# StefanHeng/Symbolic-Music-Generation

Hardware: AMD Instinct MI355X
Metric: train tokens/sec (TransfoXL seq2048 bf16), whole job (higher is better)
Workload: dtype bf16; 1 GPU; TransfoXL 12L/768d H12 dh64 F3072 T=2048 M=2048 V=1190 cutoffs=[] (SURVEY C3, mode R: fresh zero mems); per_gpu_batch=64, global_batch=64, seq_len=2048, mem_len=2048, parallelism=dp1

## Files before the change

include/musicxl.h:

```cpp
#ifndef MUSICXL_H
#define MUSICXL_H

#ifdef __cplusplus
extern "C" {
#endif

#define MXL_ABI_VERSION 2

int mxl_abi_version(void);
const char* mxl_error_string(int code);

#define MXL_GEMM_OUT_F32        0x01
#define MXL_GEMM_OUT_F32_ATOMIC 0x02
#define MXL_GEMM_BIAS           0x04
#define MXL_GEMM_RELU           0x08
#define MXL_GEMM_DROPOUT        0x10
#define MXL_GEMM_RELU_BWD       0x20
#define MXL_GEMM_ADD_AUX        0x40
int mxl_set_reserved_cus(int k);
int mxl_gemm_last_nt_kernel(void);

#define MXL_GEMM_SAVE_RELU_MASK 0x100
#define MXL_GEMM_RELU_BWD_BITS  0x200
size_t mxl_gemm_relu_mask_bytes(int M, int N);
int mxl_gemm_bf16(const void* A, const void* B, void* C, int M, int N, int K, int lda, int ldb, int ldc,
                  int transA, int transB, int flags, float alpha, const float* bias,
                  const void* aux, int ldaux, int ksplits,
                  float drop_p, unsigned long long seed, unsigned site, void* stream);

int mxl_gemm_bf16_colsum(const void* A, const void* B, void* C, int M, int N, int K, int lda, int ldb, int ldc,
                         int transA, int transB, int flags, float alpha, const float* bias, const void* aux, int ldaux,
                         float drop_p, unsigned long long seed, unsigned site, float* colsum, void* stream);

int mxl_gemm_bf16_headdot(const void* A, const void* B, void* C, int M, int N, int K, int lda, int ldb, int ldc, const void* O, int ldo,
                          int T, float* delta, void* stream);

int mxl_gemm_bf16_batched(const void* A, const void* B, void* C, int M, int N, int K, int lda, int ldb, int ldc,
                          int transA, int transB, int flags, float alpha, int ksplits, int batch, int bdiv,
                          long long sA1, long long sA2, long long sB1, long long sB2, long long sC1, long long sC2,
                          void* stream);

int mxl_gemm_skinny_bf16(const void* A, const void* W, void* C, int M, int N, int K, int lda, int ldw, int ldc, int flags,
                         const float* bias, void* stream);
int mxl_gemm_skinny_partial(const void* A, const void* W, float* slabs, int M, int N, int K, int lda, int ldw, int KS,
                            void* stream);
int mxl_ln_residual_fwd_partial(const float* slabs, int KS, long long slab_stride, const float* bias, const void* res,
                                const float* gamma, const float* beta, void* y, int N, int d, float eps, void* stream);
int mxl_decode_qkv(const void* x, const void* Wqkv, void* qkv, void* kcache, void* vcache, const int* t_dev,
                   const float* r_r_bias, void* qr_out, int B, int d, int dh, int Mring, void* stream);

int mxl_relattn_fwd(const void* q, const void* k, const void* v, const void* rd, const float* r_w_bias,
                    const float* r_r_bias, void* out, float* lse, int B, int T, int H, int dh, int M, int Kc,
                    long long q_bs, int q_rs, long long kv_bs, int kv_rs, int rd_rs, long long o_bs, int o_rs,
                    float scale, void* stream);

int mxl_relattn_bwd(const void* q, const void* k, const void* v, const void* rd, const float* r_w_bias,
                    const float* r_r_bias, const void* out, const void* dout, const float* lse, float* delta,
                    void* dq, void* dk, void* dv, void* dg, float* d_r_w_bias, float* d_r_r_bias , int B, int T,
                    int H, int dh, int M, int Kc, long long q_bs, int q_rs, long long kv_bs, int kv_rs, int rd_rs,
                    long long o_bs, int o_rs, long long dq_bs, int dq_rs, long long dkv_bs, int dkv_rs,
                    float scale, void* stream);

int mxl_relattn_drd(const void* dg, const void* qr, float* d_rd, int B, int T, int H, int dh, int M, long long qr_bs,
                    int qr_rs, int drd_ld, const void* rd, int rd_rs, float* d_r_r_bias, float* d_r_w_bias_fix, void* stream);

int mxl_relattn_bwd_sparse_dg(const void* q, const void* k, const void* v, const void* rd, const float* r_w_bias,
                              const float* r_r_bias, const void* out, const void* dout, const float* lse, float* delta, void* dq,
                              void* dk, void* dv, void* dg, float* d_r_w_bias, int B, int T, int H, int dh, int M, int Kc,
                              long long q_bs, int q_rs, long long kv_bs, int kv_rs, int rd_rs, long long o_bs, int o_rs,
                              long long dq_bs, int dq_rs, long long dkv_bs, int dkv_rs, float scale, void* stream);
int mxl_relattn_fwd_phantom(const void* q, const void* k, const void* v, const void* rd, const float* r_w_bias,
                            const float* r_r_bias, void* out, float* lse, void* oph, float* mph, int B, int T, int H,
                            int dh, int M, int Kc, long long q_bs, int q_rs, long long kv_bs, int kv_rs, int rd_rs,
                            long long o_bs, int o_rs, float scale, void* stream);
int mxl_relattn_bwd_sparse_dg_oph(const void* q, const void* k, const void* v, const void* rd, const float* r_w_bias,
                                  const float* r_r_bias, const void* out, const void* dout, const float* lse,
                                  float* delta, void* dq, void* dk, void* dv, void* dg, float* d_r_w_bias,
                                  const void* oph, const float* mph, int B, int T, int H, int dh, int M, int Kc,
                                  long long q_bs, int q_rs, long long kv_bs, int kv_rs, int rd_rs, long long o_bs, int o_rs,
                                  long long dq_bs, int dq_rs, long long dkv_bs, int dkv_rs, float scale, void* stream);
int mxl_relattn_drd_recompute(const void* dg, const void* qr, float* d_rd, int B, int T, int H, int dh, int M, long long qr_bs,
                              int qr_rs, int drd_ld, const void* rd, int rd_rs, float* d_r_r_bias, float* d_r_w_bias_fix,
                              const float* lse, const float* delta, float scale, int Kc, void* stream);

size_t mxl_relattn_bwd_fused_ws_bytes(int B, int T, int H, int dh, int M);
int mxl_relattn_bwd_fused(const void* q, const void* k, const void* v, const void* rd, const float* r_w_bias,
                          const float* r_r_bias, const void* out, const void* dout, const float* lse, float* delta,
                          void* dq, void* dk, void* dv, float* d_rd, int drd_ld, float* d_r_w_bias, float* d_r_r_bias,
                          const void* oph, const float* mph, void* ws, int B, int T, int H, int dh, int M, int Kc,
                          long long q_bs, int q_rs, long long kv_bs, int kv_rs, int rd_rs, long long o_bs, int o_rs,
                          long long dq_bs, int dq_rs, long long dkv_bs, int dkv_rs, float scale, int defer_finish, void* stream);
int mxl_relattn_dq_finish(const void* ws, const void* oph, const float* mph, const float* lse, const float* delta, void* dq,
                          float* d_r_r_bias, int B, int T, int H, int dh, int M, int Kc, long long o_bs, int o_rs, long long dq_bs,
                          int dq_rs, float scale, void* stream);
int mxl_relattn_fwd_phantom2(const void* q, const void* k, const void* v, const void* rd, const float* r_w_bias,
                             const float* r_r_bias, void* out, float* lse, void* oph, float* mph, int oph_all, void* ph_ws, int B,
                             int T, int H, int dh, int M, int Kc, long long q_bs, int q_rs, long long kv_bs, int kv_rs, int rd_rs,
                             long long o_bs, int o_rs, float scale, void* stream);
size_t mxl_relattn_drd_phantom_ws_bytes(int B, int T, int H);
int mxl_relattn_drd_phantom_prep(const void* q, long long q_bs, int q_rs, const float* r_r_bias, const float* lse, void* ws, int B, int T,
                                 int H, int dh, float scale, void* stream);
int mxl_relattn_drd_phantom(const void* ws, const float* delta, float* d_rd, int B, int T, int H, int dh, int M, int drd_ld,
                            const void* rd, int rd_rs, int Kc, void* stream);

int mxl_sinusoid_table(void* out, int M, int d, int clamp_len, float drop_p, unsigned long long seed, unsigned site,
                       void* stream);
int mxl_embed_fwd(const void* ids, const void* E, void* out, int N, int d, int V, float scale, float drop_p,
                  unsigned long long seed, unsigned site, void* stream);
int mxl_embed_bwd(const void* ids, const void* dout, const void* dout2, float* dE, int N, int d, int V, float scale,
                  float drop_p, unsigned long long seed, unsigned site, void* stream);
int mxl_dropout_bf16(const void* x, void* y, long long n, float drop_p, unsigned long long seed, unsigned site,
                     void* stream);
int mxl_ln_residual_fwd(const void* x, const void* res, const float* gamma, const float* beta, void* y, void* z,
                        float* mean, float* rstd, int N, int d, float eps, float drop_p, unsigned long long seed,
                        unsigned site, void* stream);
int mxl_ln_residual_bwd(const void* dy, const void* dy2, const void* z, const float* mean, const float* rstd,
                        const float* gamma, void* dres, void* dx, float* dgamma, float* dbeta, int N, int d,
                        float drop_p, unsigned long long seed, unsigned site, void* stream);
int mxl_ln_residual_bwd_colsum(const void* dy, const void* dy2, const void* z, const float* mean, const float* rstd,
                               const float* gamma, void* dres, void* dx, float* dgamma, float* dbeta, float* dxsum, int N,
                               int d, float drop_p, unsigned long long seed, unsigned site, void* stream);
int mxl_ln_residual_bwd_add(const void* dy, const void* dy2, const void* z, const float* mean, const float* rstd,
                            const float* gamma, const void* dadd, void* dres, float* dgamma, float* dbeta, int N, int d,
                            void* stream);
int mxl_ln_residual_bwd_add_drop(const void* dy, const void* dy2, const void* z, const float* mean, const float* rstd,
                                 const float* gamma, const void* dadd, void* dres, void* dx, float* dxsum, float* dgamma,
                                 float* dbeta, int N, int d, float drop_p, unsigned long long seed, unsigned site, void* stream);
int mxl_add_rowbias_bf16(const void* x, long long x_bs, int x_rs, const float* bias, void* out, int B, int T, int n,
                         void* stream);
int mxl_colsum_bf16(const void* X, float* out, int M, int N, int ld, void* stream);
int mxl_dropout_colsum_bf16(const void* X, void* Y, float* out, int M, int N, float drop_p, unsigned long long seed,
                            unsigned site, void* stream);
int mxl_center_columns_bf16(const void* X, void* Y, int M, int N, void* stream);
int mxl_mem_update(const void* mem, const void* hid, void* out, int B, int M, int T, int d, void* stream);

int mxl_label_guard(void* labels_row0, int T, long long eos, void* stream);
int mxl_adaptive_nll_fwd(const float* logits, int ldl, const void* labels, float* nll, float* lse, float* acc2, int B,
                         int T, int V, int ncl, const int* cutoffs_host, void* stream);
int mxl_adaptive_nll_bwd(const float* logits, int ldl, const void* labels, const float* nll, const float* lse,
                         const float* acc2, void* dlogits, int ldd, int B, int T, int V, int ncl,
                         const int* cutoffs_host, float grad_scale, void* stream);
int mxl_adaptive_nll_bwd_split(const float* logits, int ldl, const void* labels, const float* nll, const float* lse,
                               const float* acc2, void* dlogits_hi, void* dlogits_lo, int ldd, int B, int T, int V, int ncl,
                               const int* cutoffs_host, float grad_scale, void* stream);
int mxl_adaptive_logprob(const float* logits, int ldl, float* out, int ldo, int N, int V, int ncl,
                         const int* cutoffs_host, void* stream);

int mxl_cluster_bucket(const void* labels, int B, int T, int V, int ncl, const int* cutoffs_host, int* perm, int* counts,
                       int* tgt_head, int* tgt_tail, void* stream);
int mxl_gather_rows_bf16(const void* src, int ld_src, const int* idx, void* dst, int n, int d, void* stream);
int mxl_scatter_add_rows_bf16(const void* src, const int* idx, void* dst, int ld_dst, int n, int d, void* stream);
int mxl_rows_lse_pick(const float* logits, long long ld, int ncols, int n_rows, const int* rows_idx, int row0, const int* tgt,
                      float* lse_out, float* pick_out, void* stream);
int mxl_bucket_nll_finish(const float* head_lse, const float* head_pick, const float* tail_lse, const float* tail_pick,
                          const int* tgt_head, const int* tgt_tail, float* nll, float* nll_tok, float* acc2, int B, int T,
                          void* stream);
int mxl_rows_softmax_grad(const float* logits, long long ld, int ncols, int n_rows, const int* rows_idx, int row0, const int* tgt,
                          const float* lse, const float* nll_tok, const float* acc2, float grad_scale, void* out_hi, void* out_lo,
                          int ldo, void* stream);

int mxl_sumsq_f32(const float* x, long long n, float* out_accum, void* stream);
int mxl_adamw_step(float* p, const float* g, float* m, float* v, void* w16, long long n, long long n_decay, float lr,
                   float beta1, float beta2, float eps, float weight_decay, int step, const float* sumsq,
                   float max_norm, float grad_scale, void* stream);
int mxl_cast_f32_bf16(const float* x, void* y, long long n, void* stream);
int mxl_cast_bf16_f32(const void* x, float* y, long long n, void* stream);
int mxl_transpose_bf16(const void* src, void* dst, int rows, int cols, int ld_src, int ld_dst, int batch,
                       long long src_bstride, long long dst_bstride, void* stream);

int mxl_decode_embed(const void* ids, int ld_ids, const int* t_dev, const void* E, void* out, int B, int d, int V,
                     float scale, void* stream);
int mxl_kv_append(const void* qkv, void* kcache, void* vcache, const int* t_dev, int B, int M, int d, int dh,
                  const float* r_r_bias, void* qr_out, void* stream);
int mxl_kv_fill(const void* qkv, void* kcache, void* vcache, int B, int T, int M, int d, int dh, void* stream);
int mxl_kv_zero_pad(void* qkv, const int* n_pad, int B, int T, int d, void* stream);
int mxl_decode_bd(const void* qr, const void* rd, float* bd, int B, int H, int dh, int M, int ld_qr, int ld_rd, void* stream);
int mxl_relattn_decode(const void* qkv, const void* kcache, const void* vcache, const float* bd, const float* r_w_bias,
                       void* out, const int* t_dev, int B, int H, int dh, int M, float scale, void* stream);
size_t mxl_relattn_decode_split_ws_bytes(int B, int H, int dh, int pieces);
int mxl_relattn_decode_split(const void* qkv, const void* kcache, const void* vcache, const float* bd, const float* r_w_bias,
                             void* out, const int* t_dev, int B, int H, int dh, int M, float scale, int pieces, float* ws,
// ... 239 lines not shown
```

symbolic_music_generation_amd/csrc/relattn_bwd_fused.hip:

```cpp
#include <cstdlib>
#include <type_traits>
#include "common.h"
#include "musicxl_internal.h"

namespace {

typedef __attribute__((ext_vector_type(8))) __bf16 mfma_bf16x8;
typedef __attribute__((address_space(3))) bf16x4 lds_bf16x4;
typedef _Float16 f16x4 __attribute__((ext_vector_type(4)));
typedef float f32x4v __attribute__((ext_vector_type(4)));

#ifndef FUSED_PF
#define FUSED_PF 3
#endif
#ifndef FUSED_VF_RELOAD
#define FUSED_VF_RELOAD 0
#endif
#ifndef FUSED_PARK
#define FUSED_PARK 0
#endif
#ifndef FUSED_SB
#define FUSED_SB 1
#endif
#define UNIT_FENCE() do { if (FUSED_SB) __builtin_amdgcn_sched_barrier(0); } while (0)
#ifndef FUSED_DVDK_LATE
#define FUSED_DVDK_LATE 1
#endif
#ifndef FUSED_PRIO
#define FUSED_PRIO 3
#endif
#define PRIO_UP() do { if (FUSED_PRIO & 1) __builtin_amdgcn_s_setprio(1); } while (0)
#define PRIO_DOWN() do { if (FUSED_PRIO & 1) __builtin_amdgcn_s_setprio(0); } while (0)
#define PRIO_UP_B(bit_) do { if (FUSED_PRIO & (bit_)) __builtin_amdgcn_s_setprio(1); } while (0)
#define PRIO_DOWN_B(bit_) do { if (FUSED_PRIO & (bit_)) __builtin_amdgcn_s_setprio(0); } while (0)
#ifndef FUSED_OWNER_LD_EARLY
#define FUSED_OWNER_LD_EARLY 1
#endif
#ifndef FUSED_TRF_EARLY
#define FUSED_TRF_EARLY 1
#endif
constexpr float LOG2E = 1.4426950408889634f;
constexpr int KBLK = 256;
constexpr int QT = 32;
constexpr int ROWB = 128;
constexpr int K_BYTES = KBLK * ROWB;
constexpr int RING_BLKS = 10;
constexpr int RBLK_BYTES = 32 * ROWB;
constexpr int RING_BYTES = RING_BLKS * RBLK_BYTES;
constexpr int QIMG = QT * ROWB;
constexpr int QSET = 3 * QIMG + 3 * QT * 4;
constexpr int GP = 584;
constexpr int G_BYTES = QT * GP;
constexpr int X_BYTES = KBLK * 64;
constexpr int YP = 608;
constexpr int Y_BYTES = QT * YP;
constexpr int BIAS_BYTES = 2 * 64 * 4;
constexpr int PARK_BYTES = FUSED_PARK ? 32 * 64 * 4 : 0;
constexpr int SMEM = K_BYTES + RING_BYTES + 2 * QSET + G_BYTES + X_BYTES + Y_BYTES + BIAS_BYTES + PARK_BYTES;
constexpr int RING_OFF = 10240;

#ifdef MXL_STAMP
__device__ unsigned long long g_fused_stamps[16];
#define STAMP_DECL unsigned long long st_last, st_acc[16] = {0ull, 0ull, 0ull, 0ull, 0ull, 0ull, 0ull, 0ull, 0ull, 0ull, 0ull, 0ull, 0ull, 0ull, 0ull, 0ull}; \
    { __builtin_amdgcn_sched_barrier(0); asm volatile("s_memtime %0\n\ts_waitcnt lgkmcnt(0)" : "=s"(st_last) :: "memory"); __builtin_amdgcn_sched_barrier(0); }
#define STAMP(i) { unsigned long long t_; __builtin_amdgcn_sched_barrier(0); asm volatile("s_memtime %0\n\ts_waitcnt lgkmcnt(0)" : "=s"(t_) :: "memory"); \
    __builtin_amdgcn_sched_barrier(0); st_acc[i] += t_ - st_last; st_last = t_; }
#define STAMP_FLUSH if ((threadIdx.x & 63) == 0) { for (int i_ = 0; i_ < 16; i_++) atomicAdd(&g_fused_stamps[i_], st_acc[i_]); }
#else
#define STAMP_DECL
#define STAMP(i)
#define STAMP_FLUSH
#endif

#ifndef MXL_SLAB_BF16
#define MXL_SLAB_BF16 1
#endif
#if MXL_SLAB_BF16
typedef bf16_t slab_t;
#else
typedef float slab_t;
#endif

struct FusedP {
    const bf16_t *q, *k, *v, *rd, *dout;
    const float *rwb, *rrb, *lse, *delta;
    bf16_t *dk, *dv;
    slab_t* slab;
    bf16_t* dq;
    const bf16_t* oph;
    const float* mph;
    long long dq_bs;
    int dq_rs;
    float* drd;
    float *d_rwb, *d_rrb;
    int B, T, H, M, Kc;
    long long q_bs, kv_bs, o_bs, dkv_bs, slab_stride;
    int q_rs, kv_rs, rd_rs, o_rs, dkv_rs, drd_ld;
    float scale, scale_log2e;
};

__device__ __forceinline__ int qswz(int row) { return (((row >> 1) & 1) << 2) | (((row >> 2) & 1) << 1) | ((row >> 3) & 1); }
__device__ __forceinline__ int qoff(int row, int ch) { return row * ROWB + ((ch ^ qswz(row)) << 4); }
__device__ __forceinline__ int qeoff(int row, int e) { return qoff(row, e >> 3) + ((e & 7) << 1); }
__device__ __forceinline__ int sswz(int row) { return (((row >> 3) & 1) << 2) | (((row >> 1) & 1) << 1) | ((row >> 2) & 1); }
__device__ __forceinline__ int soff(int row, int ch) { return row * ROWB + ((ch ^ sswz(row)) << 4); }

__device__ __forceinline__ void lds_barrier() {
    asm volatile("s_waitcnt lgkmcnt(0)" ::: "memory");
    __builtin_amdgcn_s_barrier();
    asm volatile("" ::: "memory");
}

__device__ __forceinline__ uint32_t lds_addr(const void* p) {
    return (uint32_t)(uintptr_t)(__attribute__((address_space(3))) const char*)(const char*)p;
}

__device__ __forceinline__ void gskew_wait() { asm volatile("s_waitcnt lgkmcnt(0)" ::: "memory"); }
__device__ __forceinline__ void gskew_read16(uint32_t base, uint32_t (&u)[16]) {
    static_assert(GP == 584, "offsets below are pat(j) * (GP + 2)");
    asm volatile(
        "ds_read_u16 %0, %16\n\t"               "ds_read_u16 %1, %16 offset:586\n\t"    "ds_read_u16 %2, %16 offset:1172\n\t"
        "ds_read_u16 %3, %16 offset:1758\n\t"   "ds_read_u16 %4, %16 offset:4688\n\t"   "ds_read_u16 %5, %16 offset:5274\n\t"
        "ds_read_u16 %6, %16 offset:5860\n\t"   "ds_read_u16 %7, %16 offset:6446\n\t"   "ds_read_u16 %8, %16 offset:9376\n\t"
        "ds_read_u16 %9, %16 offset:9962\n\t"   "ds_read_u16 %10, %16 offset:10548\n\t" "ds_read_u16 %11, %16 offset:11134\n\t"
        "ds_read_u16 %12, %16 offset:14064\n\t" "ds_read_u16 %13, %16 offset:14650\n\t" "ds_read_u16 %14, %16 offset:15236\n\t"
        "ds_read_u16 %15, %16 offset:15822"
        : "=&v"(u[0]), "=&v"(u[1]), "=&v"(u[2]), "=&v"(u[3]), "=&v"(u[4]), "=&v"(u[5]), "=&v"(u[6]), "=&v"(u[7]),
          "=&v"(u[8]), "=&v"(u[9]), "=&v"(u[10]), "=&v"(u[11]), "=&v"(u[12]), "=&v"(u[13]), "=&v"(u[14]), "=&v"(u[15])
        : "v"(base)
        : "memory");
}
__device__ __forceinline__ void yskew_write16(uint32_t base, const uint32_t (&w)[8]) {
    static_assert(YP == 608, "offsets below are pat(j) * (YP + 2)");
    asm volatile(
        "ds_write_b16 %8, %0\n\t"               "ds_write_b16_d16_hi %8, %0 offset:610\n\t"
        "ds_write_b16 %8, %1 offset:1220\n\t"   "ds_write_b16_d16_hi %8, %1 offset:1830\n\t"
        "ds_write_b16 %8, %2 offset:4880\n\t"   "ds_write_b16_d16_hi %8, %2 offset:5490\n\t"
        "ds_write_b16 %8, %3 offset:6100\n\t"   "ds_write_b16_d16_hi %8, %3 offset:6710\n\t"
        "ds_write_b16 %8, %4 offset:9760\n\t"   "ds_write_b16_d16_hi %8, %4 offset:10370\n\t"
        "ds_write_b16 %8, %5 offset:10980\n\t"   "ds_write_b16_d16_hi %8, %5 offset:11590\n\t"
        "ds_write_b16 %8, %6 offset:14640\n\t"   "ds_write_b16_d16_hi %8, %6 offset:15250\n\t"
        "ds_write_b16 %8, %7 offset:15860\n\t"   "ds_write_b16_d16_hi %8, %7 offset:16470"
        :
        : "v"(w[0]), "v"(w[1]), "v"(w[2]), "v"(w[3]), "v"(w[4]), "v"(w[5]), "v"(w[6]), "v"(w[7]), "v"(base)
        : "memory");
}
__device__ __forceinline__ float add_f16(float s, uint32_t h16) {
    float r;
    asm("v_fma_mix_f32 %0, %1, 1.0, %2 op_sel_hi:[0,0,1]" : "=v"(r) : "v"(s), "v"(h16));
    return r;
}
__device__ __forceinline__ bf16x8 tr_pair(const char* lo_p, const char* hi_p) {
    const bf16x4 lo = __builtin_amdgcn_ds_read_tr16_b64_v4i16((lds_bf16x4*)lo_p);
    const bf16x4 hi = __builtin_amdgcn_ds_read_tr16_b64_v4i16((lds_bf16x4*)hi_p);
    return bf16x8{lo[0], lo[1], lo[2], lo[3], hi[0], hi[1], hi[2], hi[3]};
}
__device__ __forceinline__ f32x16 mfma32(bf16x8 a, bf16x8 b, f32x16 c) {
    return __builtin_amdgcn_mfma_f32_32x32x16_bf16(__builtin_bit_cast(mfma_bf16x8, a), __builtin_bit_cast(mfma_bf16x8, b), c, 0, 0, 0);
}
__device__ __forceinline__ f32x4 mfma16(bf16x8 a, bf16x8 b, f32x4 c) {
    return __builtin_amdgcn_mfma_f32_16x16x32_bf16(__builtin_bit_cast(mfma_bf16x8, a), __builtin_bit_cast(mfma_bf16x8, b), c, 0, 0, 0);
}

constexpr int VM_PER_TILE_BLOCK = 6;
constexpr int VM_PER_TILE_OWNER = 10;

__global__ __launch_bounds__(256) void fused_delta_kernel(const bf16_t* o, const bf16_t* dout, float* delta, int B, int T, int H,
                                                          long long o_bs, int o_rs) {
    const int row = blockIdx.x * 4 + (threadIdx.x >> 6);
    if (row >= B * T) return;
    const int lane = threadIdx.x & 63;
    const int b = row / T, i = row % T;
    const bf16_t* op = o + (size_t)b * o_bs + (size_t)i * o_rs;
    const bf16_t* dp = dout + (size_t)b * o_bs + (size_t)i * o_rs;
    const int chunks = H * 8;
    for (int c0 = 0; c0 < chunks; c0 += 64) {
        const int c = c0 + lane;
        float s = 0.f;
        if (c < chunks) {
            const bf16x8 a = *reinterpret_cast<const bf16x8*>(op + c * 8);
            const bf16x8 d = *reinterpret_cast<const bf16x8*>(dp + c * 8);
#pragma unroll
            for (int j = 0; j < 8; j++) s += bf2f((bf16_t)a[j]) * bf2f((bf16_t)d[j]);
        }
        s += __shfl_xor(s, 1, 64); s += __shfl_xor(s, 2, 64); s += __shfl_xor(s, 4, 64);
        if (c < chunks && (lane & 7) == 0) delta[((size_t)b * H + (c >> 3)) * T + i] = s;
    }
}

template <bool OWNER>
__global__ __launch_bounds__(512, 1) void relattn_bwd_fused_kernel(FusedP p) {
    constexpr int NT = 512;
    constexpr int VM_PER_TILE = OWNER ? VM_PER_TILE_OWNER : VM_PER_TILE_BLOCK;
    extern __shared__ __attribute__((aligned(16))) char smem[];
    char* sK = smem;
    char* sR = sK + K_BYTES;
    char* sQ = sR + RING_BYTES;
    char* sG = sQ + 2 * QSET;
    char* sX = sG + G_BYTES;
    char* sY = sX + X_BYTES;
    float* sBias = reinterpret_cast<float*>(sY + Y_BYTES);
    float* sPark = sBias + BIAS_BYTES / 4;

    STAMP_DECL
    const int tid = threadIdx.x;
    const int w = __builtin_amdgcn_readfirstlane(tid >> 6);
    const int l = tid & 63, r = l & 31, hh = l >> 5;
    int bx_, h, b;
    xcd_block(bx_, h, b);
    const int h64 = __builtin_amdgcn_readfirstlane(h * 64);
    const int T = p.T, M = p.M;
    const int p0 = T - p.Kc;
    const int nkb = (p.Kc + KBLK - 1) / KBLK;
    const int kloc0 = 32 * w + r;
    const int MB = M >> 5;

    const bf16_t* qbase = p.q + (size_t)b * p.q_bs + (size_t)h * 64;
    const bf16_t* dobase = p.dout + (size_t)b * p.o_bs + (size_t)h * 64;
    const bf16_t* rbase = p.rd + (size_t)h * 64;
    const bf16_t* kbase = p.k + (size_t)b * p.kv_bs + (size_t)h * 64;
    const bf16_t* vbase = p.v + (size_t)b * p.kv_bs + (size_t)h * 64;

    const int eq = w >> 1, ih0 = w & 1;
    const int g16 = l >> 4;
    int rowq, rows, tkb, xw, yt0, qb0, xa0, xa1, ka0, ka1, yq0, krow;
    uint32_t gRb, yWb;
    auto lane_consts = [&](const int l) {
    const int r = l & 31, hh = l >> 5, kloc0 = 32 * w + r;
    const int gq = l >> 4, q4 = (l & 15) >> 2, pp = l & 3;
    rowq = qoff(r, hh);
    rows = r * ROWB + ((hh ^ sswz(r)) << 4);
    tkb = qeoff(4 * hh + q4, 16 * (gq & 1) + 4 * pp);
    gRb = lds_addr(sG) + 4 * hh * (GP + 2) + (256 - kloc0) * 2;
    yWb = lds_addr(sY) + 4 * hh * (YP + 2) + (256 - kloc0) * 2;
    const int xf = (kloc0 >> 1) & 7;
    xw = kloc0 * 64 + ((((hh ^ (xf & 1)) | (xf & 6))) << 3);
    yt0 = (4 * (l >> 4) + ((l & 15) >> 2)) * YP + (16 * (w & 1) + 4 * pp) * 2;
    qb0 = qeoff(4 * (l >> 4) + ((l & 15) >> 2), 16 * (w >> 1) + 4 * pp);
    const int g16 = l >> 4, q16 = (l & 15) >> 2;
    xa0 = ((8 * g16 + q16) * 64 + ((pp ^ ((4 * g16 + (q16 >> 1)) & 7)) << 3)) ^ (ih0 << 5);
    xa1 = ((8 * g16 + q16 + 4) * 64 + ((pp ^ ((4 * g16 + 2 + (q16 >> 1)) & 7)) << 3)) ^ (ih0 << 5);
    const int kch = 2 * eq + (pp >> 1);
    const int ksw = ((g16 & 1) << 2) | (((q16 >> 1) & 1) << 1);
    ka0 = (8 * g16 + q16) * ROWB + ((kch ^ ksw) << 4) + ((pp & 1) << 3);
    ka1 = (8 * g16 + q16 + 4) * ROWB + ((kch ^ (ksw | 1)) << 4) + ((pp & 1) << 3);
    yq0 = (16 * ih0 + (l & 15)) * YP + 16 * g16;
    krow = kloc0 * ROWB + ((hh ^ sswz(kloc0)) << 4);
    };
    if (!OWNER) lane_consts(l);

    if (tid < 128) sBias[tid] = (tid < 64) ? p.rwb[h64 + tid] : p.rrb[h64 + tid - 64];

    const bool st_q = w < 4;
    const __amdgpu_buffer_rsrc_t rs_q = __builtin_amdgcn_make_buffer_rsrc((void*)qbase, 0, -1, 0x00020000);
    const __amdgpu_buffer_rsrc_t rs_2 = __builtin_amdgcn_make_buffer_rsrc((void*)(st_q ? rbase : dobase), 0, -1, 0x00020000);
    const __amdgpu_buffer_rsrc_t rs_lse = __builtin_amdgcn_make_buffer_rsrc((void*)(p.lse + ((size_t)b * p.H + h) * T), 0, -1, 0x00020000);
    const __amdgpu_buffer_rsrc_t rs_dl = __builtin_amdgcn_make_buffer_rsrc((void*)(p.delta + ((size_t)b * p.H + h) * T), 0, -1, 0x00020000);
    const bool has_ph = OWNER && p.oph != nullptr;
    const __amdgpu_buffer_rsrc_t rs_mph = __builtin_amdgcn_make_buffer_rsrc(
        (void*)(has_ph ? p.mph + ((size_t)b * p.H + h) * T : p.lse), 0, has_ph ? T * 4 : 0, 0x00020000);
    u32x4 tq = {0u, 0u, 0u, 0u}, t2 = {0u, 0u, 0u, 0u};
    float tl = 0.f, tdl = 0.f, tm = 0.f;
#define STG_IDS int tid_o = tid; asm volatile("" : "+v"(tid_o)); const int srow_ = (tid_o & 255) >> 3, sch_ = tid_o & 7;
    auto load_stage = [&](int it, int nblk) {
        STG_IDS
        const int I = it * QT;
        tq = __builtin_bit_cast(u32x4, __builtin_amdgcn_raw_buffer_load_b128(rs_q, (srow_ * p.q_rs + sch_ * 8) * 2, I * p.q_rs * 2, 0));
        int d = 32 * nblk + srow_;
        d = d < 0 ? 0 : (d > M - 1 ? M - 1 : d);
        const int vo2 = st_q ? (d * p.rd_rs + sch_ * 8) * 2 : (srow_ * p.o_rs + sch_ * 8) * 2;
        const int so2 = st_q ? 0 : I * p.o_rs * 2;
        t2 = __builtin_bit_cast(u32x4, __builtin_amdgcn_raw_buffer_load_b128(rs_2, vo2, so2, 0));
        tl = __builtin_bit_cast(float, __builtin_amdgcn_raw_buffer_load_b32(rs_lse, (tid & 31) * 4, I * 4, 0));
        tdl = __builtin_bit_cast(float, __builtin_amdgcn_raw_buffer_load_b32(rs_dl, (tid & 31) * 4, I * 4, 0));
        if (OWNER) tm = __builtin_bit_cast(float, __builtin_amdgcn_raw_buffer_load_b32(rs_mph, (tid & 31) * 4, I * 4, 0));
    };
    auto store_stage = [&](int buf, int slot) {
        STG_IDS
        char* sQw = sQ + buf * QSET;
        char* sQr = sQw + QIMG;
        char* sDO = sQr + QIMG;
        float* sLse = reinterpret_cast<float*>(sDO + QIMG);
        {
            const bf16_t* src = reinterpret_cast<const bf16_t*>(&tq);
            const float* bb = sBias + (st_q ? 0 : 64) + sch_ * 8;
            const f32x4 b0 = *reinterpret_cast<const f32x4*>(bb), b1 = *reinterpret_cast<const f32x4*>(bb + 4);
            u32x4 wq;
            bf16_t* dq_ = reinterpret_cast<bf16_t*>(&wq);
#pragma unroll
            for (int j = 0; j < 8; j++) dq_[j] = f2bf((bf2f(src[j]) + (j < 4 ? b0[j & 3] : b1[j & 3])) * p.scale_log2e);
            *reinterpret_cast<u32x4*>((st_q ? sQw : sQr) + qoff(srow_, sch_)) = wq;
        }
        if (st_q) {
            *reinterpret_cast<u32x4*>(sR + slot * RBLK_BYTES + soff(srow_, sch_)) = t2;
        } else {
            const bf16_t* src = reinterpret_cast<const bf16_t*>(&t2);
            u32x4 wd;
            bf16_t* dd = reinterpret_cast<bf16_t*>(&wd);
#pragma unroll
            for (int j = 0; j < 8; j++) dd[j] = f2bf(bf2f(src[j]) * p.scale);
            *reinterpret_cast<u32x4*>(sDO + qoff(srow_, sch_)) = wd;
        }
        if (tid < 32) {
            sLse[tid] = -tl * LOG2E; sLse[QT + tid] = -p.scale * tdl;
            if (OWNER) sLse[2 * QT + tid] = tm;
        }
    };
    auto slot_add = [&](int s, int k) { const int x = s + k; return x >= RING_BLKS ? x - RING_BLKS : x; };
    auto gblock = [&](int j, int s0, const bf16x8 (&bq)[4]) {
        f32x16 g;
#pragma unroll
        for (int t = 0; t < 16; t++) g[t] = 0.f;
        const char* rb = sR + slot_add(s0, j) * RBLK_BYTES;
        bf16x8 a[4];
#pragma unroll
        for (int ks = 0; ks < 4; ks++) a[ks] = *reinterpret_cast<const bf16x8*>(rb + (rows ^ (ks << 5)));
#pragma unroll
        for (int ks = 0; ks < 4; ks++) g = mfma32(a[ks], bq[ks], g);
        char* gw = sG + r * GP + (32 * j + 4 * hh) * 2;
#pragma unroll
        for (int grp = 0; grp < 4; grp++) {
            const f32x4v v4 = {g[4 * grp], g[4 * grp + 1], g[4 * grp + 2], g[4 * grp + 3]};
            *reinterpret_cast<f16x4*>(gw + 16 * grp) = __builtin_convertvector(v4, f16x4);
        }
    };

    f32x16 ak[2], av[2];
    f32x4 racc[9];
    float cw = 0.f, cr = 0.f;

    const int ld4 = p.drd_ld * 4;
    const __amdgpu_buffer_rsrc_t rs_drd = __builtin_amdgcn_make_buffer_rsrc((void*)(p.drd + h64), 0, (int)((32 * MB - 1) * ld4 + 256), 0x00020000);
    constexpr int DRD_OOB = 0x7ffff000;
    auto drd_park = [&](const f32x4& leave) {
#pragma unroll
        for (int t = 0; t < 4; t++) sPark[(16 * (w & 1) + 4 * (l >> 4) + t) * 64 + 16 * (w >> 1) + (l & 15)] = leave[t];
    };
    auto drd_add = [&](const f32x4& leave, int nL) {
        const bool ok = nL >= 0 && nL < MB;
        const float f = 1.f / p.scale_log2e;
        const int so = (ok ? 32 * nL : 0) + 16 * (w & 1);
        const int vo = ok ? 4 * (l >> 4) * ld4 + (16 * (w >> 1) + (l & 15)) * 4 : DRD_OOB;
#pragma unroll
        for (int t = 0; t < 4; t++)
#ifndef MXL_ABL_NO_ATOMICS
            __builtin_amdgcn_raw_ptr_buffer_atomic_fadd_f32(leave[t] * f, rs_drd, vo, (so + t) * ld4, 0);
#else
            asm volatile("" :: "v"(leave[t]));
#endif
    };
    float pk[4];
    auto park_read = [&]() {
#pragma unroll
        for (int i = 0; i < 4; i++) pk[i] = sPark[(4 * w + i) * 64 + l];
    };
    auto park_add = [&](int nL) {
        const bool ok = nL >= 0 && nL < MB;
        const int so = ok ? 32 * nL * ld4 : 0;
        const float f = 1.f / p.scale_log2e;
#pragma unroll
        for (int i = 0; i < 4; i++)
#ifndef MXL_ABL_NO_ATOMICS
            __builtin_amdgcn_raw_ptr_buffer_atomic_fadd_f32(pk[i] * f, rs_drd, ok ? l * 4 : DRD_OOB, so + (4 * w + i) * ld4, 0);
#else
            asm volatile("" :: "v"(pk[i]));
#endif
    };
    auto drd_flush_direct = [&](int nfirst, const int l) {
#ifndef MXL_ABL_NO_ATOMICS
        const float f = 1.f / p.scale_log2e;
        const int vo = 4 * (l >> 4) * ld4 + (16 * (w >> 1) + (l & 15)) * 4;
#pragma unroll
        for (int v = 0; v < 8; v++) {
            const int nb = nfirst + v;
            if (nb >= 0 && nb < MB) {
#pragma unroll
                for (int t = 0; t < 4; t++)
                    __builtin_amdgcn_raw_ptr_buffer_atomic_fadd_f32(racc[v][t] * f, rs_drd, vo, (32 * nb + 16 * (w & 1) + t) * ld4, 0);
            }
        }
#endif
    };
    const __amdgpu_buffer_rsrc_t rs_sc = __builtin_amdgcn_make_buffer_rsrc(
        (void*)((char*)p.slab + (OWNER ? ((size_t)b * p.H + h) * (size_t)(T >> 5) * 8192 : 0)), 0, OWNER ? (T >> 5) * 8192 : 0, 0x00020000);
    const __amdgpu_buffer_rsrc_t rs_dq = __builtin_amdgcn_make_buffer_rsrc(
        (void*)(OWNER ? p.dq + (size_t)b * p.dq_bs + (size_t)h * 64 + 16 * eq : (bf16_t*)p.slab), 0, OWNER ? T * p.dq_rs * 2 : 0, 0x00020000);
    const __amdgpu_buffer_rsrc_t rs_oph = __builtin_amdgcn_make_buffer_rsrc(
        (void*)(has_ph ? p.oph + (size_t)b * p.o_bs + (size_t)h * 64 + 16 * eq : p.q), 0, has_ph ? T * p.o_rs * 2 : 0, 0x00020000);
    auto owner_loads = [&](int it, bool first, bool last, f32x4& part, uint32_t (&ophw)[2]) {
        part = __builtin_bit_cast(f32x4, __builtin_amdgcn_raw_buffer_load_b128(rs_sc, first ? DRD_OOB : l * 16, it * 8192 + w * 1024, 0));
        const int vo = last ? (4 * g16 + ((l & 1) ? 2 : 0)) * p.o_rs * 2 + ((l & 15) >> 1) * 4 : DRD_OOB;
#pragma unroll
        for (int u = 0; u < 2; u++)
            ophw[u] = (uint32_t)__builtin_amdgcn_raw_buffer_load_b32(rs_oph, vo, (it * QT + 16 * ih0 + u) * p.o_rs * 2, 0);
    };

#pragma unroll 1
    do {
    const int P0 = p0 + KBLK * bx_;
    const int Pw = P0 + 32 * w;
    __syncthreads();
    int tp = tid;
    if (OWNER) asm volatile("" : "+v"(tp));
#pragma unroll
    for (int n = 0; n < 2048 / NT; n++) {
        const int c = tp + n * NT;
        const int row = c >> 3, ch = c & 7;
        const int srow = KBLK * bx_ + row;
        u32x4 val = {0u, 0u, 0u, 0u};
        if (srow < p.Kc) val = *reinterpret_cast<const u32x4*>(kbase + (size_t)srow * p.kv_rs + ch * 8);
        *reinterpret_cast<u32x4*>(sK + soff(row, ch)) = val;
    }
    for (int i = tp; i < Y_BYTES / 16; i += NT) reinterpret_cast<u32x4*>(sY)[i] = u32x4{0u, 0u, 0u, 0u};
    bf16x8 vf[4];
    const bool kok = Pw + r < T;
    {
        const size_t srow = (size_t)(kok ? Pw + r - p0 : 0);
        const bf16_t* vp = vbase + srow * p.kv_rs;
#pragma unroll
        for (int ks = 0; ks < 4; ks++) {
            const bf16x8 vv = *reinterpret_cast<const bf16x8*>(vp + 16 * ks + 8 * hh);
#pragma unroll
            for (int j = 0; j < 8; j++) vf[ks][j] = kok ? vv[j] : (short)0;
        }
    }

    const int i_lo = max(P0, 0), i_hi = min(P0 + KBLK - 1 + M - 1, T - 1);
    const int it_lo = i_lo >> 5, it_hi = i_hi >> 5;

    int rs0;
    {
        const int n0 = (it_lo * QT - P0 - KBLK) >> 5;
        rs0 = (n0 + RING_OFF) % RING_BLKS;
        load_stage(it_lo, n0 + 8);
        store_stage(0, slot_add(rs0, 8));
        constexpr int NPR = (9 * 256 + NT - 1) / NT;
        u32x4 pr_[NPR];
#pragma unroll
        for (int n = 0; n < NPR; n++) {
            const int c = tp + n * NT;
            int d = 32 * n0 + (c >> 3);
            d = d < 0 ? 0 : (d > M - 1 ? M - 1 : d);
            pr_[n] = (c < 9 * 256) ? *reinterpret_cast<const u32x4*>(rbase + (size_t)d * p.rd_rs + (c & 7) * 8) : u32x4{0u, 0u, 0u, 0u};
        }
#pragma unroll
        for (int n = 0; n < NPR; n++) {
            const int c = tp + n * NT;
            if (c < 9 * 256) {
                const int slot = slot_add(rs0, c >> 8);
                *reinterpret_cast<u32x4*>(sR + slot * RBLK_BYTES + soff((c >> 3) & 31, c & 7)) = pr_[n];
            }
        }
    }
    __syncthreads();
    if (OWNER) {
        int l_ = l;
        asm volatile("" : "+v"(l_));
        lane_consts(l_);
    }
    {
        bf16x8 bq[4];
#pragma unroll
        for (int ks = 0; ks < 4; ks++) bq[ks] = *reinterpret_cast<const bf16x8*>(sQ + QIMG + (rowq ^ (ks << 5)));
        gblock(w, rs0, bq);
        if (w == 0) gblock(8, rs0, bq);
    }
    load_stage(min(it_lo + 1, it_hi), ((it_lo * QT - P0 - KBLK) >> 5) + 9);
    __syncthreads();

#pragma unroll
    for (int e = 0; e < 2; e++)
#pragma unroll
        for (int j = 0; j < 16; j++) { ak[e][j] = 0.f; av[e][j] = 0.f; }
#pragma unroll
    for (int v = 0; v < 9; v++) racc[v] = f32x4{0.f, 0.f, 0.f, 0.f};

    if (FUSED_PARK) {
        for (int i = tid; i < PARK_BYTES / 4; i += NT) sPark[i] = 0.f;
        __syncthreads();
    }
#pragma unroll
    for (int i = 0; i < VM_PER_TILE; i++)
        __builtin_amdgcn_raw_ptr_buffer_atomic_fadd_f32(0.f, rs_drd, DRD_OOB, i * ld4, 0);

    int cur = 0;
    STAMP(15)
#pragma unroll 1
    for (int it = it_lo; it <= it_hi; it++) {
        const int I = it * QT;
        const bool more = it < it_hi;
        asm volatile("" : "+v"(rowq), "+v"(rows), "+v"(tkb), "+v"(xw), "+v"(yt0), "+v"(qb0), "+v"(xa0), "+v"(xa1), "+v"(ka0), "+v"(ka1), "+v"(yq0), "+v"(krow));
        const char* sQw = sQ + cur * QSET;
        const char* sQr = sQw + QIMG;
        const char* sDO = sQr + QIMG;
        const float* sLse = reinterpret_cast<const float*>(sDO + QIMG);
        const int n0 = (I - P0 - KBLK) >> 5;
#ifndef MXL_ABL_NO_STAGING
#ifdef MXL_STAMP
        asm volatile("s_waitcnt vmcnt(6)" ::: "memory");
        STAMP(14)
#endif
        store_stage(cur ^ 1, slot_add(rs0, 9));
#ifdef MXL_ABL_HOT_LOADS
        load_stage(it_lo, n0 + 10);
#else
        load_stage(min(it + 2, it_hi), n0 + 10);
#endif
#endif
        if (FUSED_PARK) park_read();
        STAMP(0)

        const int dmin_w = I - Pw - 31, dmax_w = I + 31 - Pw;
        const bool active = (dmax_w >= 0) && (dmin_w <= M - 1) && (Pw < T);
        const bool full = (dmin_w >= 0) && (dmax_w <= M - 1) && (Pw + 31 < T);
        uint32_t dsw[8], prw[8];
        bf16x8 tdo_[2][2], tqw_[2][2];
        auto dvdk = [&]() {
#ifndef MXL_ABL_NO_DVDK
#pragma unroll
            for (int st = 0; st < 2; st++) {
                const u32x4 pw = {prw[4 * st], prw[4 * st + 1], prw[4 * st + 2], prw[4 * st + 3]};
                const u32x4 dw = {dsw[4 * st], dsw[4 * st + 1], dsw[4 * st + 2], dsw[4 * st + 3]};
#pragma unroll
                for (int e = 0; e < 2; e++) {
                    av[e] = mfma32(tdo_[st][e], __builtin_bit_cast(bf16x8, pw), av[e]);
                    ak[e] = mfma32(tqw_[st][e], __builtin_bit_cast(bf16x8, dw), ak[e]);
                }
            }
#endif
        };
        auto tr_frags = [&]() {
#pragma unroll
            for (int st = 0; st < 2; st++)
#pragma unroll
                for (int e = 0; e < 2; e++) {
                    const int lo = 2048 * st + (tkb ^ (e << 6)), hi = 2048 * st + 1024 + (tkb ^ 16 ^ (e << 6));
                    tdo_[st][e] = tr_pair(sDO + lo, sDO + hi);
                    tqw_[st][e] = tr_pair(sQw + lo, sQw + hi);
                }
        };
        if (active) {
            bf16x8 aq[4], ad[4], kfl[4];
            f32x16 s, dp;
#pragma unroll
            for (int grp = 0; grp < 4; grp++) {
                const f32x4 cl = *reinterpret_cast<const f32x4*>(sLse + 8 * grp + 4 * hh);
#pragma unroll
                for (int t = 0; t < 4; t++) s[4 * grp + t] = cl[t];
            }
#pragma unroll
            for (int ks = 0; ks < 4; ks++) {
                aq[ks] = *reinterpret_cast<const bf16x8*>(sQw + (rowq ^ (ks << 5)));
                kfl[ks] = *reinterpret_cast<const bf16x8*>(sK + (krow ^ (ks << 5)));
            }
            __builtin_amdgcn_sched_barrier(0);
#pragma unroll
            for (int grp = 0; grp < 4; grp++) {
                const f32x4 cd = *reinterpret_cast<const f32x4*>(sLse + QT + 8 * grp + 4 * hh);
#pragma unroll
                for (int t = 0; t < 4; t++) dp[4 * grp + t] = cd[t];
            }
#pragma unroll
            for (int ks = 0; ks < 4; ks++) ad[ks] = *reinterpret_cast<const bf16x8*>(sDO + (rowq ^ (ks << 5)));
            PRIO_UP();
#pragma unroll
            for (int ks = 0; ks < 4; ks++) s = mfma32(aq[ks], kfl[ks], s);
            __builtin_amdgcn_sched_barrier(0);
#if FUSED_VF_RELOAD
            bf16x8 vfl[4];
            {
                const bf16_t* vp = vbase + (size_t)(kok ? Pw + r - p0 : 0) * p.kv_rs;
#pragma unroll
                for (int ks = 0; ks < 4; ks++) vfl[ks] = *reinterpret_cast<const bf16x8*>(vp + 16 * ks + 8 * hh);
            }
#pragma unroll
            for (int ks = 0; ks < 4; ks++) dp = mfma32(ad[ks], vfl[ks], dp);
#else
#pragma unroll
            for (int ks = 0; ks < 4; ks++) dp = mfma32(ad[ks], vf[ks], dp);
#endif
            PRIO_DOWN();
            uint32_t bdu[16];
            gskew_read16(gRb, bdu);
            STAMP(1)
            gskew_wait();
            STAMP(2)
            f32x16 pr;
            const bool fl = __builtin_amdgcn_readfirstlane((int)full) != 0;
            if (fl) {
#pragma unroll
                for (int j = 0; j < 16; j++) {
                    const float pv = __builtin_amdgcn_exp2f(add_f16(s[j], bdu[j]));
                    pr[j] = pv;
                    s[j] = pv * dp[j];
                }
            } else {
                const int pk = Pw + r;
#pragma unroll
                for (int j = 0; j < 16; j++) {
                    const int ii = (j & 3) + 8 * (j >> 2) + 4 * hh;
                    const int d = I + ii - pk;
                    const bool valid = (d >= 0) && (d <= M - 1) && kok;
                    const float x = add_f16(s[j], bdu[j]);
                    const float pv = __builtin_amdgcn_exp2f(valid ? x : -1.0e30f);
                    pr[j] = pv;
                    s[j] = pv * (valid ? dp[j] : 0.f);
                }
            }
#pragma unroll
            for (int m = 0; m < 8; m++) { dsw[m] = pack2bf(s[2 * m], s[2 * m + 1]); prw[m] = pack2bf(pr[2 * m], pr[2 * m + 1]); }
            if (FUSED_TRF_EARLY || !FUSED_DVDK_LATE) tr_frags();
#pragma unroll
            for (int grp = 0; grp < 4; grp++)
                *reinterpret_cast<u32x2*>(sX + (xw ^ (grp << 4))) = u32x2{dsw[2 * grp], dsw[2 * grp + 1]};
            yskew_write16(yWb, dsw);
            if (!FUSED_DVDK_LATE) dvdk();
        } else {
            const uint32_t z[8] = {0u, 0u, 0u, 0u, 0u, 0u, 0u, 0u};
#pragma unroll
            for (int grp = 0; grp < 4; grp++) *reinterpret_cast<u32x2*>(sX + (xw ^ (grp << 4))) = u32x2{0u, 0u};
            yskew_write16(yWb, z);
            if (FUSED_DVDK_LATE) {
#pragma unroll
                for (int m = 0; m < 8; m++) asm volatile("" : "=v"(dsw[m]), "=v"(prw[m]));
#pragma unroll
                for (int st = 0; st < 2; st++)
#pragma unroll
                    for (int e = 0; e < 2; e++) asm volatile("" : "=v"(tdo_[st][e]), "=v"(tqw_[st][e]));
            }
        }
        if (FUSED_PARK) park_add(n0 - 1);
        bool v_first = false, v_last = false;
        f32x4 part = {0.f, 0.f, 0.f, 0.f};
        uint32_t ophw[2] = {0u, 0u};
        if (OWNER) {
            const int x = I - M - 254 - p0;
            const int kb_lo = x <= 0 ? 0 : (x + 255) >> 8;
            const int kb_hi = min(nkb - 1, (I + 31 - p0) >> 8);
            v_first = bx_ == kb_lo;
            v_last = bx_ == kb_hi;
#if FUSED_OWNER_LD_EARLY
            owner_loads(it, v_first, v_last, part, ophw);
#endif
        }
        STAMP(3)
        lds_barrier();
        STAMP(4)

        {
            bf16x8 ua[26], ub[17], qrb;
            int sl = rs0;
            auto rd_unit = [&](int n) {
                if (n < 8) {
                    ub[n] = tr_pair(sK + n * 4096 + ka0, sK + n * 4096 + ka1);
                    ua[n] = tr_pair(sX + n * 2048 + xa0, sX + n * 2048 + xa1);
                } else if (n < 17) {
                    const char* rb = sR + sl * RBLK_BYTES;
                    ub[n] = tr_pair(rb + ka0, rb + ka1);
                    ua[n] = *reinterpret_cast<const bf16x8*>(sY + yq0 + (n - 8) * 64);
                    sl = (sl == RING_BLKS - 1) ? 0 : sl + 1;
                } else {
                    if (n == 17) qrb = tr_pair(sQr + qb0, sQr + qb0 + 2048);
                    ua[n] = tr_pair(sY + yt0 + (n - 17) * 64, sY + yt0 + 16 * YP + (n - 17) * 64);
                }
            };
            if (FUSED_DVDK_LATE && !FUSED_TRF_EARLY && active) tr_frags();
#pragma unroll
            for (int n = 0; n < FUSED_PF; n++) rd_unit(n);
            UNIT_FENCE();
            PRIO_UP();
            if (FUSED_DVDK_LATE && active) dvdk();
            PRIO_DOWN();
#if !FUSED_OWNER_LD_EARLY
            if (OWNER) owner_loads(it, v_first, v_last, part, ophw);
#endif
            UNIT_FENCE();
            STAMP(5)
            f32x4 aw4[2], ar4[2];
#pragma unroll
            for (int c = 0; c < 2; c++) { aw4[c] = f32x4{0.f, 0.f, 0.f, 0.f}; ar4[c] = f32x4{0.f, 0.f, 0.f, 0.f}; }
            f32x4 leave;
            PRIO_UP_B(2);
#pragma unroll
            for (int n = 0; n < 26; n++) {
                if (n < 8) aw4[n & 1] = mfma16(ua[n], ub[n], aw4[n & 1]);
                else if (n < 17) ar4[n & 1] = mfma16(ua[n], ub[n], ar4[n & 1]);
                else if (n == 17) leave = mfma16(ua[n], qrb, racc[0]);
                else racc[n - 18] = mfma16(ua[n], qrb, racc[n - 17]);
                if (n + FUSED_PF < 26) rd_unit(n + FUSED_PF);
                UNIT_FENCE();
            }
            PRIO_DOWN_B(2);
            racc[8] = f32x4{0.f, 0.f, 0.f, 0.f};
            STAMP(6)
            const char* sQrN = sQ + (cur ^ 1) * QSET + QIMG;
            const int rs1 = slot_add(rs0, 1);
            bf16x8 gq_[4], ga[4];
            {
                const char* rb = sR + slot_add(rs1, w) * RBLK_BYTES;
#pragma unroll
                for (int ks = 0; ks < 4; ks++) {
                    gq_[ks] = *reinterpret_cast<const bf16x8*>(sQrN + (rowq ^ (ks << 5)));
                    ga[ks] = *reinterpret_cast<const bf16x8*>(rb + (rows ^ (ks << 5)));
                }
            }
            UNIT_FENCE();
            if (OWNER) {
#pragma unroll
                for (int t = 0; t < 4; t++) { aw4[0][t] += aw4[1][t]; ar4[0][t] += ar4[1][t]; }
                const bool odd = (l & 1) != 0;
                float v[4], nb[4];
#pragma unroll
                for (int t = 0; t < 4; t++) v[t] = (aw4[0][t] + ar4[0][t]) + part[t];
                __builtin_amdgcn_raw_buffer_store_b128(u32x4{__builtin_bit_cast(uint32_t, v[0]), __builtin_bit_cast(uint32_t, v[1]),
                                                             __builtin_bit_cast(uint32_t, v[2]), __builtin_bit_cast(uint32_t, v[3])},
                                                       rs_sc, v_last ? DRD_OOB : l * 16, it * 8192 + w * 1024, 0);
#pragma unroll
                for (int t = 0; t < 4; t++)
                    nb[t] = __builtin_bit_cast(float, __builtin_amdgcn_mov_dpp(__builtin_bit_cast(int, v[t]), 0xB1, 0xf, 0xf, true));
                const int rowl = 16 * ih0 + 4 * g16 + (odd ? 2 : 0);
                const int vo = v_last ? (4 * g16 + (odd ? 2 : 0)) * p.dq_rs * 2 + ((l & 15) >> 1) * 4 : DRD_OOB;
                float slo = 0.f, shi = 0.f;
#pragma unroll
                for (int u = 0; u < 2; u++) {
                    float lo = odd ? nb[2 + u] : v[u], hi = odd ? v[2 + u] : nb[u];
                    const float f = sLse[QT + rowl + u] * __builtin_amdgcn_exp2f(fminf(sLse[2 * QT + rowl + u] + sLse[rowl + u], 126.f));
                    const float plo = f * __builtin_bit_cast(float, ophw[u] << 16), phi = f * __builtin_bit_cast(float, ophw[u] & 0xffff0000u);
                    if (has_ph) { lo += plo; hi += phi; slo += plo; shi += phi; }
                    __builtin_amdgcn_raw_buffer_store_b32((int)pack2bf(lo, hi), rs_dq, vo, (I + 16 * ih0 + u) * p.dq_rs * 2, 0);
                }
                cw += (aw4[0][0] + aw4[0][1]) + (aw4[0][2] + aw4[0][3]);
                cr += (ar4[0][0] + ar4[0][1]) + (ar4[0][2] + ar4[0][3]);
                const float want = odd ? slo : shi;
                const float got = __builtin_bit_cast(float, __builtin_amdgcn_mov_dpp(__builtin_bit_cast(int, want), 0xB1, 0xf, 0xf, true));
                if (has_ph && v_last) cr += (odd ? shi : slo) + got;
            } else {
#pragma unroll
                for (int t = 0; t < 4; t++) { aw4[0][t] += aw4[1][t]; ar4[0][t] += ar4[1][t]; }
                const int x = I - M - 254 - p0;
                const int kb_lo = x <= 0 ? 0 : (x + 255) >> 8;
                const int rowb = p.H * 64 * (int)sizeof(slab_t);
                slab_t* tile = p.slab + (size_t)(bx_ - kb_lo) * p.slab_stride + ((size_t)b * T + I + 16 * ih0) * (size_t)(p.H * 64) + h * 64 + 16 * eq;
                const __amdgpu_buffer_rsrc_t rs_sl = __builtin_amdgcn_make_buffer_rsrc((void*)tile, 0, -1, 0x00020000);
#if MXL_SLAB_BF16
                const bool odd = (l & 1) != 0;
                const int vo = (4 * g16 + (odd ? 2 : 0)) * rowb + ((l & 15) >> 1) * 4;
                float v[4], nb[4];
#pragma unroll
                for (int t = 0; t < 4; t++) {
                    v[t] = aw4[0][t] + ar4[0][t];
                    nb[t] = __builtin_bit_cast(float, __builtin_amdgcn_mov_dpp(__builtin_bit_cast(int, v[t]), 0xB1, 0xf, 0xf, true));
                }
#pragma unroll
                for (int u = 0; u < 2; u++) {
                    const float lo = odd ? nb[2 + u] : v[u], hi = odd ? v[2 + u] : nb[u];
                    __builtin_amdgcn_raw_buffer_store_b32((int)pack2bf(lo, hi), rs_sl, vo, u * rowb, 0);
                }
#else
                const int vo = 4 * g16 * rowb + (l & 15) * 4;
#pragma unroll
                for (int t = 0; t < 4; t++)
                    __builtin_amdgcn_raw_buffer_store_b32(__builtin_bit_cast(int, aw4[0][t] + ar4[0][t]), rs_sl, vo, t * rowb, 0);
#endif
                cw += (aw4[0][0] + aw4[0][1]) + (aw4[0][2] + aw4[0][3]);
                cr += (ar4[0][0] + ar4[0][1]) + (ar4[0][2] + ar4[0][3]);
            }
            STAMP(7)
            if (FUSED_PARK) drd_park(leave); else drd_add(leave, n0);
            STAMP(8)
            if (more) {
                f32x16 g;
#pragma unroll
                for (int t = 0; t < 16; t++) g[t] = 0.f;
                PRIO_UP_B(4);
#pragma unroll
                for (int ks = 0; ks < 4; ks++) g = mfma32(ga[ks], gq_[ks], g);
                PRIO_DOWN_B(4);
                char* gw = sG + r * GP + (32 * w + 4 * hh) * 2;
#pragma unroll
                for (int grp = 0; grp < 4; grp++) {
                    const f32x4v v4 = {g[4 * grp], g[4 * grp + 1], g[4 * grp + 2], g[4 * grp + 3]};
                    *reinterpret_cast<f16x4*>(gw + 16 * grp) = __builtin_convertvector(v4, f16x4);
                }
                if (w == ((n0 + 4) & 7)) {
                    const char* rb = sR + slot_add(rs1, 8) * RBLK_BYTES;
#pragma unroll
                    for (int ks = 0; ks < 4; ks++) ga[ks] = *reinterpret_cast<const bf16x8*>(rb + (rows ^ (ks << 5)));
                    UNIT_FENCE();
                    f32x16 g8;
#pragma unroll
                    for (int t = 0; t < 16; t++) g8[t] = 0.f;
#pragma unroll
                    for (int ks = 0; ks < 4; ks++) g8 = mfma32(ga[ks], gq_[ks], g8);
                    char* gw8 = sG + r * GP + (32 * 8 + 4 * hh) * 2;
#pragma unroll
                    for (int grp = 0; grp < 4; grp++) {
                        const f32x4v v4 = {g8[4 * grp], g8[4 * grp + 1], g8[4 * grp + 2], g8[4 * grp + 3]};
                        *reinterpret_cast<f16x4*>(gw8 + 16 * grp) = __builtin_convertvector(v4, f16x4);
                    }
                }
            }
            STAMP(9)
            STAMP(10)
        }
        lds_barrier();
        STAMP(12)
        cur ^= 1;
        rs0 = (rs0 == RING_BLKS - 1) ? 0 : rs0 + 1;
    }
    {
        const int n0_end = ((it_hi + 1) * QT - P0 - KBLK) >> 5;
        if (FUSED_PARK && it_lo <= it_hi) { park_read(); park_add(n0_end - 1); }
    }
    int le = l;
    if (OWNER) asm volatile("" : "+v"(le));
    drd_flush_direct(((it_hi + 1) * QT - P0 - KBLK) >> 5, le);
    STAMP(13)

    if (kok) {
        const int r = le & 31, hh = le >> 5;
        const float fk = 1.f / p.scale_log2e, fv = 1.f / p.scale;
        const size_t srow = (size_t)(Pw + r - p0);
        bf16_t* dkp = p.dk + (size_t)b * p.dkv_bs + srow * p.dkv_rs + (size_t)h * 64;
        bf16_t* dvp = p.dv + (size_t)b * p.dkv_bs + srow * p.dkv_rs + (size_t)h * 64;
#pragma unroll
        for (int e = 0; e < 2; e++) {
#pragma unroll
            for (int grp = 0; grp < 4; grp++) {
                const int e0 = 32 * e + 8 * grp + 4 * hh;
                const u32x2 wk = {pack2bf(ak[e][4 * grp] * fk, ak[e][4 * grp + 1] * fk), pack2bf(ak[e][4 * grp + 2] * fk, ak[e][4 * grp + 3] * fk)};
                const u32x2 wv = {pack2bf(av[e][4 * grp] * fv, av[e][4 * grp + 1] * fv), pack2bf(av[e][4 * grp + 2] * fv, av[e][4 * grp + 3] * fv)};
                *reinterpret_cast<u32x2*>(dkp + e0) = wk;
                *reinterpret_cast<u32x2*>(dvp + e0) = wv;
            }
        }
    }
    } while (OWNER && ++bx_ < nkb);
    STAMP_FLUSH

    {
        float a = cw, c = cr;
        a += __shfl_xor(a, 16, 64); a += __shfl_xor(a, 32, 64);
        c += __shfl_xor(c, 16, 64); c += __shfl_xor(c, 32, 64);
        if (l < 16) {
            atomicAdd(p.d_rwb + h * 64 + 16 * eq + l, a);
            atomicAdd(p.d_rrb + h * 64 + 16 * eq + l, c);
        }
    }
}

struct FinP {
    const slab_t* slab; const bf16_t* oph; const float *mph, *lse, *delta;
    bf16_t* dq; float* d_rrb;
    int B, T, H, M, Kc;
    long long slab_stride, o_bs, dq_bs; int o_rs, dq_rs;
    float scale;
};
#ifndef FIN_K_
#define FIN_K_ 1
#endif
constexpr int FIN_K = FIN_K_;
constexpr int FIN_ROWS = 16;
__global__ __launch_bounds__(256) void relattn_dq_finish_kernel(FinP p) {
    __shared__ float s_red[256 * 8];
    const int d = p.H * 64, nch = d >> 3;
    const int per_b = p.T / FIN_ROWS;
    const int p0 = p.T - p.Kc;
    const int nkb = (p.Kc + KBLK - 1) / KBLK;
    const bool colsum = p.oph != nullptr && p.d_rrb != nullptr;
    const slab_t* __restrict__ slab = p.slab;
    const int t = threadIdx.x;
    for (int cb = 0; cb < nch; cb += 256) {
        const int cw = min(256, nch - cb), kr = 256 / cw;
        const int c = cb + t % cw, rsub = t / cw;
        const bool act = rsub < kr;
        float cs[8];
#pragma unroll
        for (int j = 0; j < 8; j++) cs[j] = 0.f;
        for (int rg = blockIdx.x; rg < p.B * per_b; rg += gridDim.x) {
            const int b = rg / per_b, i0 = (rg % per_b) * FIN_ROWS;
            const int I = i0 & ~31;
            const int x = I - p.M - 254 - p0;
            const int kb_lo = x <= 0 ? 0 : (x + 255) >> 8;
            const int kb_hi = min(nkb - 1, (I + 31 - p0) >> 8);
            const int nsl = kb_hi - kb_lo + 1;
            for (int rbase = 0; rbase < FIN_ROWS; rbase += FIN_K * kr) {
                float acc[FIN_K][8];
                int i_[FIN_K];
                bool ok[FIN_K];
#pragma unroll
                for (int k = 0; k < FIN_K; k++) {
// ... 9 lines not shown
                    bf16x8 a[FIN_K];
#pragma unroll
                    for (int k = 0; k < FIN_K; k++)
                        a[k] = *reinterpret_cast<const bf16x8*>(slab + (size_t)s * p.slab_stride + ((size_t)b * p.T + i_[k]) * (size_t)d + c * 8);
#pragma unroll
                    for (int k = 0; k < FIN_K; k++)
#pragma unroll
                        for (int j = 0; j < 8; j++) acc[k][j] += bf2f((bf16_t)a[k][j]);
#else
                    f32x4 a[FIN_K][2];
#pragma unroll
                    for (int k = 0; k < FIN_K; k++) {
                        const float* sp = slab + (size_t)s * p.slab_stride + ((size_t)b * p.T + i_[k]) * (size_t)d + c * 8;
                        a[k][0] = *reinterpret_cast<const f32x4*>(sp); a[k][1] = *reinterpret_cast<const f32x4*>(sp + 4);
                    }
#pragma unroll
                    for (int k = 0; k < FIN_K; k++)
#pragma unroll
                        for (int j = 0; j < 4; j++) { acc[k][j] += a[k][0][j]; acc[k][4 + j] += a[k][1][j]; }
#endif
                }
#pragma unroll
                for (int k = 0; k < FIN_K; k++) {
                    if (!ok[k]) continue;
                    const int i = i_[k];
                    if (p.oph) {
                        const size_t sidx = ((size_t)b * p.H + (c >> 3)) * p.T + i;
                        const float f = -p.scale * p.delta[sidx] * __builtin_amdgcn_exp2f(fminf(p.mph[sidx] - p.lse[sidx] * LOG2E, 126.f));
                        const bf16x8 o = *reinterpret_cast<const bf16x8*>(p.oph + (size_t)b * p.o_bs + (size_t)i * p.o_rs + c * 8);
#pragma unroll
                        for (int j = 0; j < 8; j++) {
                            const float v = f * bf2f((bf16_t)o[j]);
                            acc[k][j] += v;
                            cs[j] += v;
                        }
                    }
                    const u32x4 wq = {pack2bf(acc[k][0], acc[k][1]), pack2bf(acc[k][2], acc[k][3]), pack2bf(acc[k][4], acc[k][5]),
                                      pack2bf(acc[k][6], acc[k][7])};
                    *reinterpret_cast<u32x4*>(p.dq + (size_t)b * p.dq_bs + (size_t)i * p.dq_rs + c * 8) = wq;
                }
            }
        }
        if (colsum) {
            __syncthreads();
            if (act) {
#pragma unroll
                for (int j = 0; j < 8; j++) s_red[(rsub * 8 + j) * cw + (c - cb)] = cs[j];
            }
            __syncthreads();
            for (int a = t; a < cw * 8; a += blockDim.x) {
                float v = 0.f;
                for (int q = 0; q < kr; q++) v += s_red[(q * 8 + (a & 7)) * cw + (a >> 3)];
                atomicAdd(p.d_rrb + cb * 8 + a, v);
            }
        }
    }
}

}

#ifdef MXL_STAMP
extern "C" int mxl_debug_fused_stamps(unsigned long long* host_out16) {
    hipError_t e = hipMemcpyFromSymbol(host_out16, HIP_SYMBOL(g_fused_stamps), sizeof(unsigned long long) * 16);
    if (e != hipSuccess) return (int)e;
    unsigned long long z[16] = {0};
    e = hipMemcpyToSymbol(HIP_SYMBOL(g_fused_stamps), z, sizeof(z));
    return (int)e;
}
#endif

#ifndef FUSED_OWNER_MIN_FILL
#define FUSED_OWNER_MIN_FILL 0.9
#endif
static bool fused_owner_fills(int B, int H, int cus) {
    const long long wgs = (long long)B * H, rounds = (wgs + cus - 1) / cus;
    return (double)wgs >= FUSED_OWNER_MIN_FILL * (double)(rounds * cus);
}

extern "C" size_t mxl_relattn_bwd_fused_ws_bytes(int B, int T, int H, int dh, int M) {
    if (B <= 0 || T <= 0 || H <= 0 || dh != 64 || M <= 0) return 0;
    return (size_t)((M + KBLK - 1) / KBLK + 1) * (size_t)B * T * H * 64 * sizeof(slab_t);
}

extern "C" int mxl_relattn_bwd_fused(const void* q, const void* k, const void* v, const void* rd, const float* r_w_bias,
                                     const float* r_r_bias, const void* out, const void* dout, const float* lse, float* delta,
                                     void* dq, void* dk, void* dv, float* d_rd, int drd_ld, float* d_r_w_bias, float* d_r_r_bias,
                                     const void* oph, const float* mph, void* ws, int B, int T, int H, int dh, int M, int Kc,
                                     long long q_bs, int q_rs, long long kv_bs, int kv_rs, int rd_rs, long long o_bs, int o_rs,
                                     long long dq_bs, int dq_rs, long long dkv_bs, int dkv_rs, float scale, int defer_finish,
                                     void* stream) {
    MXL_CHECK_ARG(q && k && v && rd && r_w_bias && r_r_bias && out && dout && lse && delta && dq && dk && dv && d_rd && d_r_w_bias &&
                  d_r_r_bias && ws);
    if (dh != 64) return MXL_EUNSUPPORTED;
    MXL_CHECK_ARG(B > 0 && T > 0 && H > 0 && M > 0 && Kc >= T && Kc <= M + T && drd_ld >= H * 64);
    if ((T % 32) != 0 || (M % 32) != 0 || (Kc % 32) != 0) return MXL_EUNSUPPORTED;
    MXL_CHECK_ARG(Kc == M + T || (oph && mph));
    MXL_CHECK_ARG((q_rs % 8) == 0 && (kv_rs % 8) == 0 && (rd_rs % 8) == 0 && (o_rs % 8) == 0 && (dq_rs % 8) == 0 && (dkv_rs % 4) == 0);
    MXL_CHECK_ARG((q_bs % 8) == 0 && (kv_bs % 8) == 0 && (o_bs % 8) == 0 && (dq_bs % 8) == 0 && (dkv_bs % 4) == 0);
    MXL_CHECK_ARG(((uintptr_t)q % 16) == 0 && ((uintptr_t)k % 16) == 0 && ((uintptr_t)v % 16) == 0 && ((uintptr_t)rd % 16) == 0 &&
                  ((uintptr_t)out % 16) == 0 && ((uintptr_t)dout % 16) == 0 && ((uintptr_t)dq % 16) == 0 && ((uintptr_t)ws % 16) == 0 &&
                  (oph == nullptr || ((uintptr_t)oph % 16) == 0));
    hipStream_t s = (hipStream_t)stream;
    static bool attr_set = false;
    if (!attr_set) {
        hipError_t e = hipFuncSetAttribute(reinterpret_cast<const void*>(&relattn_bwd_fused_kernel<false>), hipFuncAttributeMaxDynamicSharedMemorySize, SMEM);
        if (e == hipSuccess)
            e = hipFuncSetAttribute(reinterpret_cast<const void*>(&relattn_bwd_fused_kernel<true>), hipFuncAttributeMaxDynamicSharedMemorySize, SMEM);
        if (e != hipSuccess) return (int)e;
        attr_set = true;
    }
    const bool delta_ready = (defer_finish & 2) != 0;
    MXL_CHECK_ARG((defer_finish & 12) != 12);
    const bool owner = (defer_finish & 1) ? false : (defer_finish & 4) ? true : (defer_finish & 8) ? false
                                                                               : fused_owner_fills(B, H, mxl_usable_cus());
    defer_finish &= 1;
    if (!delta_ready) {
        mxl_kt::Scope kt(MXL_KT_RELATTN_DELTA, s);
        hipLaunchKernelGGL(fused_delta_kernel, dim3((B * T + 3) / 4), dim3(256), 0, s, (const bf16_t*)out, (const bf16_t*)dout, delta, B, T,
                           H, o_bs, o_rs);
    }
    FusedP p;
    p.q = (const bf16_t*)q; p.k = (const bf16_t*)k; p.v = (const bf16_t*)v; p.rd = (const bf16_t*)rd; p.dout = (const bf16_t*)dout;
    p.rwb = r_w_bias; p.rrb = r_r_bias; p.lse = lse; p.delta = delta;
    p.dk = (bf16_t*)dk; p.dv = (bf16_t*)dv; p.slab = (slab_t*)ws; p.drd = d_rd; p.d_rwb = d_r_w_bias; p.d_rrb = d_r_r_bias;
    p.B = B; p.T = T; p.H = H; p.M = M; p.Kc = Kc;
    p.q_bs = q_bs; p.kv_bs = kv_bs; p.o_bs = o_bs; p.dkv_bs = dkv_bs; p.slab_stride = (long long)B * T * H * 64;
    p.q_rs = q_rs; p.kv_rs = kv_rs; p.rd_rs = rd_rs; p.o_rs = o_rs; p.dkv_rs = dkv_rs; p.drd_ld = drd_ld;
    p.scale = scale; p.scale_log2e = scale * LOG2E;
    p.dq = (bf16_t*)dq; p.dq_bs = dq_bs; p.dq_rs = dq_rs;
    p.oph = (Kc < M + T) ? (const bf16_t*)oph : nullptr; p.mph = mph;
    {
        mxl_kt::Scope kt(MXL_KT_RELATTN_FUSED, s);
        if (owner) hipLaunchKernelGGL(relattn_bwd_fused_kernel<true>, dim3(1, H, B), dim3(512), SMEM, s, p);
        else hipLaunchKernelGGL(relattn_bwd_fused_kernel<false>, dim3((Kc + KBLK - 1) / KBLK, H, B), dim3(512), SMEM, s, p);
    }
    MXL_LAUNCH_CHECK();
    if (defer_finish || owner) return MXL_OK;
    return mxl_relattn_dq_finish(ws, oph, mph, lse, delta, dq, d_r_r_bias, B, T, H, dh, M, Kc, o_bs, o_rs, dq_bs, dq_rs, scale, stream);
}

extern "C" int mxl_relattn_dq_finish(const void* ws, const void* oph, const float* mph, const float* lse, const float* delta, void* dq,
                                     float* d_r_r_bias, int B, int T, int H, int dh, int M, int Kc, long long o_bs, int o_rs,
                                     long long dq_bs, int dq_rs, float scale, void* stream) {
    MXL_CHECK_ARG(ws && lse && delta && dq && B > 0 && T > 0 && H > 0 && M > 0 && Kc >= T && Kc <= M + T);
    if (dh != 64 || (T % 32) != 0 || (M % 32) != 0 || (Kc % 32) != 0) return MXL_EUNSUPPORTED;
    MXL_CHECK_ARG(Kc == M + T || (oph && mph));
    MXL_CHECK_ARG((o_rs % 8) == 0 && (o_bs % 8) == 0 && (dq_rs % 8) == 0 && (dq_bs % 8) == 0 && ((uintptr_t)dq % 16) == 0 &&
                  ((uintptr_t)ws % 16) == 0 && (oph == nullptr || ((uintptr_t)oph % 16) == 0));
    hipStream_t s = (hipStream_t)stream;
    FinP f;
    f.slab = (const slab_t*)ws; f.oph = (Kc < M + T) ? (const bf16_t*)oph : nullptr; f.mph = mph; f.lse = lse; f.delta = delta;
    f.dq = (bf16_t*)dq; f.d_rrb = d_r_r_bias;
    f.B = B; f.T = T; f.H = H; f.M = M; f.Kc = Kc;
    f.slab_stride = (long long)B * T * H * 64; f.o_bs = o_bs; f.dq_bs = dq_bs; f.o_rs = o_rs; f.dq_rs = dq_rs; f.scale = scale;
    {
        mxl_kt::Scope kt(MXL_KT_RELATTN_DQFIN, s);
        const long long rgs = (long long)B * (T / FIN_ROWS);
        const int nch = H * 8, cw = nch < 256 ? nch : 256, busy = (256 / cw) * cw, nthr = (busy + 63) / 64 * 64;
        static const int per_cu = getenv("MXL_DQFIN_WG_PER_CU") ? atoi(getenv("MXL_DQFIN_WG_PER_CU")) : 2048 / nthr;
        const long long want = 256ll * per_cu;
        hipLaunchKernelGGL(relattn_dq_finish_kernel, dim3((unsigned)(rgs < want ? rgs : want)), dim3(nthr), 0, s, f);
    }
    MXL_LAUNCH_CHECK();
    return MXL_OK;
}
```

symbolic_music_generation_amd/csrc/relattn_fwd.hip:

```cpp
#include <type_traits>
#include "common.h"
#include "musicxl_internal.h"

namespace {

typedef __attribute__((ext_vector_type(8))) __bf16 mfma_bf16x8;
typedef __attribute__((address_space(3))) bf16x4 lds_bf16x4;

struct RelAttnP {
    const bf16_t *q, *k, *v, *rd;
    const float *rwb, *rrb;
    bf16_t* out;
    float* lse;
    int B, T, H, M, Kc;
    long long q_bs, kv_bs, o_bs;
    int q_rs, kv_rs, rd_rs, o_rs;
    float scale_log2e;
    bf16_t* oph;
    float* mph;
    int oph_all;
    char* ph_rec;
};

constexpr int QB = 128;
constexpr int KT = 64;
constexpr int GS = 100;
constexpr float NEG_BIG = -1.0e30f;

__device__ __forceinline__ int floordiv(int a, int b) { return (a >= 0) ? a / b : -((-a + b - 1) / b); }

template <int DH> struct Geo {
    static constexpr int KS = DH / 16;
    static constexpr int EB = (DH + 31) / 32;
    static constexpr int VW = EB * 32;
    static constexpr int ROWB = DH * 2;
    static constexpr int VROWB = VW * 2;
    static constexpr int CH = DH / 8;
    static constexpr int VCH = VW / 8;
    static constexpr int K_BYTES = KT * ROWB;
    static constexpr int V_BYTES = KT * VROWB;
    static constexpr int R_BYTES = 256 * ROWB;
    static constexpr int G_BYTES = 4 * 32 * GS * 2;
    static constexpr int SMEM = K_BYTES + V_BYTES + R_BYTES + G_BYTES;
    static constexpr int NLD_K = (KT * CH + 255) / 256;
    static constexpr int NLD_V = (KT * CH + 255) / 256;
    __device__ static __forceinline__ int koff(int row, int ch) {
        if (DH == 64) return row * ROWB + ((ch ^ ((row >> 1) & 7)) << 4);
        return row * ROWB + (ch << 4);
    }
    __device__ static __forceinline__ int eoff(int row, int e) { return koff(row, e >> 3) + ((e & 7) << 1); }
    __device__ static __forceinline__ int voff(int row, int byte) {
        if (DH == 64) return row * VROWB + (byte ^ (((row >> 1) & 1) << 6));
        return row * VROWB + byte;
    }
};

typedef _Float16 f16x4 __attribute__((ext_vector_type(4)));
typedef float f32x4v __attribute__((ext_vector_type(4)));


#define MXL_SKEW_READS                                                                                                        \
        "ds_read_u16 %0, %16 offset:54\n\t"  "ds_read_u16 %1, %16 offset:52\n\t"  "ds_read_u16 %2, %16 offset:50\n\t"           \
        "ds_read_u16 %3, %16 offset:48\n\t"  "ds_read_u16 %4, %16 offset:38\n\t"  "ds_read_u16 %5, %16 offset:36\n\t"           \
        "ds_read_u16 %6, %16 offset:34\n\t"  "ds_read_u16 %7, %16 offset:32\n\t"  "ds_read_u16 %8, %16 offset:22\n\t"           \
        "ds_read_u16 %9, %16 offset:20\n\t"  "ds_read_u16 %10, %16 offset:18\n\t" "ds_read_u16 %11, %16 offset:16\n\t"          \
        "ds_read_u16 %12, %16 offset:6\n\t"  "ds_read_u16 %13, %16 offset:4\n\t"  "ds_read_u16 %14, %16 offset:2\n\t"           \
        "ds_read_u16 %15, %16\n\t"
#define MXL_SKEW_OPERANDS                                                                                                     \
        : "=&v"(u[0]), "=&v"(u[1]), "=&v"(u[2]), "=&v"(u[3]), "=&v"(u[4]), "=&v"(u[5]), "=&v"(u[6]), "=&v"(u[7]),               \
          "=&v"(u[8]), "=&v"(u[9]), "=&v"(u[10]), "=&v"(u[11]), "=&v"(u[12]), "=&v"(u[13]), "=&v"(u[14]), "=&v"(u[15])          \
        : "v"(base)                                                                                                           \
        : "memory"
__device__ __forceinline__ void skew_issue16(uint32_t base, uint32_t (&u)[16]) {
    asm volatile(MXL_SKEW_READS "s_nop 0" MXL_SKEW_OPERANDS);
}
__device__ __forceinline__ void skew_issue16_w15(uint32_t base, uint32_t (&u)[16]) {
    asm volatile(MXL_SKEW_READS "s_waitcnt lgkmcnt(15)" MXL_SKEW_OPERANDS);
}
__device__ __forceinline__ void lgkm_wait0() { asm volatile("s_waitcnt lgkmcnt(0)" ::: "memory"); }

__device__ __forceinline__ float add_f16v(float s, uint32_t h16) {
    float r;
    asm volatile("v_fma_mix_f32 %0, %1, 1.0, %2 op_sel_hi:[0,0,1]" : "=v"(r) : "v"(s), "v"(h16));
    return r;
}

__device__ __forceinline__ float max3(float a, float b, float c) {
    float r;
    asm("v_max3_f32 %0, %1, %2, %3" : "=v"(r) : "v"(a), "v"(b), "v"(c));
    return r;
}

#ifdef MXL_STAMP
__device__ unsigned long long g_fwd_stamps[16];
#define STAMP_DECL unsigned long long st_last, st_acc[16] = {0ull, 0ull, 0ull, 0ull, 0ull, 0ull, 0ull, 0ull, 0ull, 0ull, 0ull, 0ull, 0ull, 0ull, 0ull, 0ull}; \
    { __builtin_amdgcn_sched_barrier(0); asm volatile("s_memtime %0\n\ts_waitcnt lgkmcnt(0)" : "=s"(st_last) :: "memory"); __builtin_amdgcn_sched_barrier(0); }
#define STAMP(i) { unsigned long long t_; __builtin_amdgcn_sched_barrier(0); asm volatile("s_memtime %0\n\ts_waitcnt lgkmcnt(0)" : "=s"(t_) :: "memory"); \
    __builtin_amdgcn_sched_barrier(0); st_acc[i] += t_ - st_last; st_last = t_; }
#define STAMP_FLUSH if ((threadIdx.x & 63) == 0) { for (int i_ = 0; i_ < 16; i_++) atomicAdd(&g_fwd_stamps[i_], st_acc[i_]); }
#else
#define STAMP_DECL
#define STAMP(i)
#define STAMP_FLUSH
#endif

#ifndef FWD_PRIO
#define FWD_PRIO 6
#endif
#define FPRIO_UP(bit_) do { if (FWD_PRIO & (bit_)) __builtin_amdgcn_s_setprio(1); } while (0)
#define FPRIO_DOWN(bit_) do { if (FWD_PRIO & (bit_)) __builtin_amdgcn_s_setprio(0); } while (0)
constexpr float RESCALE_THRESH = 8.0f;
constexpr float FAST_SUM_MAX = 8192.0f;

template <int DH>
__global__ __launch_bounds__(256, 2) void relattn_fwd_kernel(RelAttnP p) {
    using G = Geo<DH>;
    constexpr int KS = G::KS, EB = G::EB;
    extern __shared__ __attribute__((aligned(16))) char smem[];
    char* sK = smem;
    char* sV = sK + G::K_BYTES;
    char* sR = sV + G::V_BYTES;
    _Float16* sG = reinterpret_cast<_Float16*>(sR + G::R_BYTES);

    STAMP_DECL
    const int tid = threadIdx.x;
    const int wid = __builtin_amdgcn_readfirstlane(tid >> 6);
    const int l = tid & 63, r = l & 31, hh = l >> 5;
    int bx_, h, b;
    xcd_block(bx_, h, b);
    const int i0 = (gridDim.x - 1 - bx_) * QB;
    const int iw0 = i0 + 32 * wid;
    const int T = p.T, M = p.M;
    const int p0 = T - p.Kc;
    _Float16* gW = sG + wid * 32 * GS + r * GS + 4 * hh;
    const _Float16* gR = sG + wid * 32 * GS + r * GS + r + 64 - 4 * hh;
    const uint32_t gRb = (uint32_t)(uintptr_t)(__attribute__((address_space(3))) const char*)(const char*)(gR - 27);
    f16x4 carry[4];
    int rfr[KS];
#pragma unroll
    for (int ks = 0; ks < KS; ks++)
        rfr[ks] = r * G::ROWB + ((DH == 64) ? (((2 * ks + hh) ^ ((r >> 1) & 7)) << 4) : ((2 * ks + hh) << 4));

    const bf16_t* kbase = p.k + (size_t)b * p.kv_bs + (size_t)h * DH;
    const bf16_t* vbase = p.v + (size_t)b * p.kv_bs + (size_t)h * DH;
    const bf16_t* rbase = p.rd + (size_t)h * DH;

    bf16x8 qw[KS], qr[KS];
    {
        const int i = iw0 + r;
        const bool ok = i < T;
        const bf16_t* qp = p.q + (size_t)b * p.q_bs + (size_t)(ok ? i : 0) * p.q_rs + (size_t)h * DH;
#pragma unroll
        for (int ks = 0; ks < KS; ks++) {
            const int e0 = 16 * ks + 8 * hh;
            bf16x8 qv = *reinterpret_cast<const bf16x8*>(qp + e0);
#pragma unroll
            for (int j = 0; j < 8; j++) {
                const float qf = ok ? bf2f((bf16_t)qv[j]) : 0.f;
                qw[ks][j] = (short)f2bf((qf + p.rwb[h * DH + e0 + j]) * p.scale_log2e);
                qr[ks][j] = (short)f2bf((qf + p.rrb[h * DH + e0 + j]) * p.scale_log2e);
            }
        }
    }

    if (p.ph_rec && iw0 < T) {
        char* rec = p.ph_rec + (((size_t)b * p.H + h) * (size_t)(T >> 5) + (iw0 >> 5)) * 4352;
        const int sw = (((r >> 1) & 1) << 2) | (((r >> 2) & 1) << 1) | ((r >> 3) & 1);
#pragma unroll
        for (int ks = 0; ks < KS; ks++) *reinterpret_cast<bf16x8*>(rec + r * 128 + (((2 * ks + hh) ^ sw) << 4)) = qr[ks];
    }

    const int p_lo = i0 - M + 1;
    const int p_hi = min(i0 + QB - 1, T - 1);
    const int kt_lo = floordiv(p_lo, KT), kt_hi = floordiv(p_hi, KT);

    typedef u32x4 stage_t[G::NLD_K];
    stage_t rk, rv, rr[2];
    const unsigned kv_bytes = (unsigned)(((long long)(p.Kc - 1) * p.kv_rs + DH) * 2);
    const unsigned rd_bytes = (unsigned)(((long long)(M - 1) * p.rd_rs + DH) * 2);
    const __amdgpu_buffer_rsrc_t rs_k = __builtin_amdgcn_make_buffer_rsrc((void*)kbase, 0, (int)kv_bytes, 0x00020000);
    const __amdgpu_buffer_rsrc_t rs_v = __builtin_amdgcn_make_buffer_rsrc((void*)vbase, 0, (int)kv_bytes, 0x00020000);
    const __amdgpu_buffer_rsrc_t rs_r = __builtin_amdgcn_make_buffer_rsrc((void*)rbase, 0, (int)rd_bytes, 0x00020000);
    constexpr bool STG_ALL = (KT * G::CH) % 256 == 0;
    int kvo[G::NLD_K], rdo[G::NLD_K], kst[G::NLD_K], vst[G::NLD_K];
#pragma unroll
    for (int n = 0; n < G::NLD_K; n++) {
        const int c = tid + n * 256;
        const int row = c / G::CH, ch = c % G::CH;
        kvo[n] = ((row - p0) * p.kv_rs + ch * 8) * 2;
        rdo[n] = (row * p.rd_rs + ch * 8) * 2;
        kst[n] = G::koff(row & (KT - 1), ch);
        vst[n] = G::voff(row & (KT - 1), ch * 16);
    }
    auto load_kv = [&](stage_t& dk, stage_t& dv, int P) __attribute__((always_inline)) {
        const int so = P * p.kv_rs * 2;
#pragma unroll
        for (int n = 0; n < G::NLD_K; n++) {
// ... 166 lines not shown
                    const int dblk = db + 32 * gb;
                    if (p.oph && on[gb] && (p.oph_all || (dblk & ~255) > iw0 + 31 - pz)) {
                        const int gq = l >> 4, li = l & 15, q4 = li >> 2, pp = li & 3;
                        const char* rbb = rb + gb * 32 * G::ROWB;
#pragma unroll
                        for (int st = 0; st < 2; st++) {
                            const u32x4 pw = {pack2bf(g[gb][8 * st], g[gb][8 * st + 1]), pack2bf(g[gb][8 * st + 2], g[gb][8 * st + 3]),
                                              pack2bf(g[gb][8 * st + 4], g[gb][8 * st + 5]), pack2bf(g[gb][8 * st + 6], g[gb][8 * st + 7])};
                            const bf16x8 pf = __builtin_bit_cast(bf16x8, pw);
#pragma unroll
                            for (int e = 0; e < EB; e++) {
                                const int dist = dblk + 16 * st + 4 * hh + q4;
                                const int ecol = 32 * e + 16 * (gq & 1) + 4 * pp;
                                bf16x8 a = {0, 0, 0, 0, 0, 0, 0, 0};
                                if (DH == 64) {
                                    const char* a0 = rbb + tk0 + 16 * st * G::ROWB;
                                    const bf16x4 lo = __builtin_amdgcn_ds_read_tr16_b64_v4i16((lds_bf16x4*)(a0 + 64 * e));
                                    const bf16x4 hi = __builtin_amdgcn_ds_read_tr16_b64_v4i16((lds_bf16x4*)(a0 + 8 * G::ROWB + 64 * (1 - e)));
                                    a = bf16x8{lo[0], lo[1], lo[2], lo[3], hi[0], hi[1], hi[2], hi[3]};
                                } else if (ecol < DH) {
                                    const bf16x4 lo = __builtin_amdgcn_ds_read_tr16_b64_v4i16((lds_bf16x4*)(sR + G::eoff(dist & 255, ecol)));
                                    const bf16x4 hi = __builtin_amdgcn_ds_read_tr16_b64_v4i16((lds_bf16x4*)(sR + G::eoff((dist + 8) & 255, ecol)));
                                    a = bf16x8{lo[0], lo[1], lo[2], lo[3], hi[0], hi[1], hi[2], hi[3]};
                                }
                                o[e] = __builtin_amdgcn_mfma_f32_32x32x16_bf16(__builtin_bit_cast(mfma_bf16x8, a),
                                                                               __builtin_bit_cast(mfma_bf16x8, pf), o[e], 0, 0, 0);
                            }
                        }
                    }
                }
                FPRIO_DOWN(4);
            }
            STAMP(13)
            __syncthreads();
            STAMP(14)
        };
#pragma unroll 1
        for (int db = db0; db <= M - 1; db += 128) {
            chunk(std::integral_constant<int, 0>{}, db);
            if (db + 64 > M - 1) break;
            chunk(std::integral_constant<int, 1>{}, db + 64);
        }
    }

    if (p.oph) {
        const int qi = iw0 + r;
        if (qi < T) {
            bf16_t* op = p.oph + (size_t)b * p.o_bs + (size_t)qi * p.o_rs + (size_t)h * DH;
#pragma unroll
            for (int e = 0; e < EB; e++) {
#pragma unroll
                for (int grp = 0; grp < 4; grp++) {
                    const int e0 = 32 * e + 8 * grp + 4 * hh;
                    if (e0 < DH) {
                        u32x2 w = {pack2bf(o[e][4 * grp], o[e][4 * grp + 1]), pack2bf(o[e][4 * grp + 2], o[e][4 * grp + 3])};
                        *reinterpret_cast<u32x2*>(op + e0) = w;
                    }
                }
            }
            if (hh == 0) p.mph[((size_t)b * p.H + h) * T + qi] = (m_run == NEG_BIG) ? 0.f : m_run;
        }
#pragma unroll
        for (int e = 0; e < EB; e++)
#pragma unroll
            for (int j = 0; j < 16; j++) o[e][j] = 0.f;
    }

    {
        const int P0 = kt_start * KT;
        const int dbase = i0 - P0 - 64;
        stage_t w2;
        load_kv(rk, rv, P0);
        load_r(rr[0], dbase);
        load_r(rr[1], dbase + 64);
        load_r(w2, dbase + 128);
        store_kv(rk, rv);
        store_r(rr[0], dbase);
        store_r(rr[1], dbase + 64);
        store_r(w2, dbase + 128);
    }
    __syncthreads();

    bool have_ring = false;
    auto rescale_o = [&](float alpha) __attribute__((always_inline)) {
#pragma unroll
        for (int e = 0; e < EB; e++)
#pragma unroll
            for (int j = 0; j < 16; j++) o[e][j] *= alpha;
    };

#pragma unroll 1
    for (int kt = kt_start; kt <= kt_hi; kt++) {
        const int P = kt * KT;
        STAMP(15)
        load_kv(rk, rv, P + KT);
        load_r(rr[0], i0 - (P + KT) - 64);
        STAMP(0)
        const int dmin_w = iw0 - P - (KT - 1), dmax_w = iw0 + 31 - P;
        const bool active = (dmax_w >= 0) && (dmin_w <= M - 1) && (iw0 < T);
        if (active) {
            const char* cK = sK;
            const char* cV = sV;
            const int dlo = iw0 - P - 64;
            auto gblock = [&](int gb, f16x4 (&dst)[4]) __attribute__((always_inline)) {
                f32x16 g;
#pragma unroll
                for (int j = 0; j < 16; j++) g[j] = 0.f;
                const char* rb = sR + ((dlo + 32 * gb) & 255) * G::ROWB;
#pragma unroll
                for (int ks = 0; ks < KS; ks++) {
                    const bf16x8 a = *reinterpret_cast<const bf16x8*>(rb + rfr[ks]);
                    g = __builtin_amdgcn_mfma_f32_32x32x16_bf16(__builtin_bit_cast(mfma_bf16x8, a),
                                                                __builtin_bit_cast(mfma_bf16x8, qr[ks]), g, 0, 0, 0);
                }
#pragma unroll
                for (int grp = 0; grp < 4; grp++) {
                    const f32x4v v4 = {g[4 * grp], g[4 * grp + 1], g[4 * grp + 2], g[4 * grp + 3]};
                    dst[grp] = __builtin_convertvector(v4, f16x4);
                }
            };
            f16x4 b0[4], b1[4];
            if (!have_ring) gblock(2, carry);
            {
                bf16x8 ra[2][KS];
#pragma unroll
                for (int gb = 0; gb < 2; gb++) {
                    const char* rb = sR + ((dlo + 32 * gb) & 255) * G::ROWB;
#pragma unroll
                    for (int ks = 0; ks < KS; ks++) ra[gb][ks] = *reinterpret_cast<const bf16x8*>(rb + rfr[ks]);
                }
                __builtin_amdgcn_sched_barrier(0);
                f32x16 g0, g1;
#pragma unroll
                for (int j = 0; j < 16; j++) { g0[j] = 0.f; g1[j] = 0.f; }
                FPRIO_UP(1);
#pragma unroll
                for (int ks = 0; ks < KS; ks++) {
                    g0 = __builtin_amdgcn_mfma_f32_32x32x16_bf16(__builtin_bit_cast(mfma_bf16x8, ra[0][ks]),
                                                                 __builtin_bit_cast(mfma_bf16x8, qr[ks]), g0, 0, 0, 0);
                    g1 = __builtin_amdgcn_mfma_f32_32x32x16_bf16(__builtin_bit_cast(mfma_bf16x8, ra[1][ks]),
                                                                 __builtin_bit_cast(mfma_bf16x8, qr[ks]), g1, 0, 0, 0);
                }
                FPRIO_DOWN(1);
                STAMP(1)
#pragma unroll
                for (int grp = 0; grp < 4; grp++) {
                    const f32x4v v0 = {g0[4 * grp], g0[4 * grp + 1], g0[4 * grp + 2], g0[4 * grp + 3]};
                    const f32x4v v1 = {g1[4 * grp], g1[4 * grp + 1], g1[4 * grp + 2], g1[4 * grp + 3]};
                    b0[grp] = __builtin_convertvector(v0, f16x4);
                    b1[grp] = __builtin_convertvector(v1, f16x4);
                }
            }
#pragma unroll
            for (int grp = 0; grp < 4; grp++) {
                *reinterpret_cast<f16x4*>(gW + 8 * grp) = b0[grp];
                *reinterpret_cast<f16x4*>(gW + 32 + 8 * grp) = b1[grp];
                *reinterpret_cast<f16x4*>(gW + 64 + 8 * grp) = carry[grp];
                carry[grp] = b0[grp];
            }
            have_ring = true;
            STAMP(2)
            const bool full = (dmin_w >= 0) && (dmax_w <= M - 1) && (iw0 + 31 < T);
            const int qi = iw0 + r;
            f32x16 s[2];
            auto tile_scores = [&](auto masked) __attribute__((always_inline)) {
                constexpr bool MASKED = decltype(masked)::value;
                {
                    bf16x8 ka[2][KS];
#pragma unroll
                    for (int kb = 0; kb < 2; kb++)
#pragma unroll
                        for (int ks = 0; ks < KS; ks++)
                            ka[kb][ks] = *reinterpret_cast<const bf16x8*>(cK + G::koff(32 * kb + r, 2 * ks + hh));
                    __builtin_amdgcn_sched_barrier(0);
                    s[0] = cinit; s[1] = cinit;
                    FPRIO_UP(1);
#pragma unroll
                    for (int ks = 0; ks < KS; ks++) {
#pragma unroll
                        for (int kb = 0; kb < 2; kb++)
                            s[kb] = __builtin_amdgcn_mfma_f32_32x32x16_bf16(__builtin_bit_cast(mfma_bf16x8, ka[kb][ks]),
                                                                            __builtin_bit_cast(mfma_bf16x8, qw[ks]), s[kb], 0, 0, 0);
                    }
                    FPRIO_DOWN(1);
                    __builtin_amdgcn_sched_barrier(0);
                }
                STAMP(3)
                uint32_t u0[16], u1[16];
                skew_issue16(gRb, u0);
                skew_issue16_w15(gRb - 64, u1);
#pragma unroll
                for (int kb = 0; kb < 2; kb++) {
                    if (kb == 1) lgkm_wait0();
#pragma unroll
                    for (int j = 0; j < 16; j++) {
                        float val = add_f16v(s[kb][j], kb == 0 ? u0[j] : u1[j]);
                        if (MASKED) {
                            const int d = qi - P - (32 * kb + (j & 3) + 8 * (j >> 2) + 4 * hh);
                            const bool valid = (d >= 0) && (d <= M - 1) && (qi < T);
                            val = valid ? val : NEG_BIG;
                        }
                        s[kb][j] = val;
                    }
                }
            };
            auto scores = [&]() __attribute__((always_inline)) { if (full) tile_scores(std::false_type{}); else tile_scores(std::true_type{}); };
            const bool attempt = all_set;
            bool precise = !attempt, bad = false;
            float rs = 0.f;
            if (attempt) {
                scores();
                STAMP(4)
                rs = exp_sum(s);
                bad = !(rs <= FAST_SUM_MAX);
                precise = __any(bad);
            }
            if (precise) {
                scores();
                rebase(s, rescale_o, attempt, rs);
                rs = exp_sum(s);
            }
            l_run += rs;
            STAMP(5)
            FPRIO_UP(2);
#pragma unroll
            for (int kb = 0; kb < 2; kb++) {
#pragma unroll
                for (int st = 0; st < 2; st++) {
                    const u32x4 pw = {pack2bf(s[kb][8 * st], s[kb][8 * st + 1]), pack2bf(s[kb][8 * st + 2], s[kb][8 * st + 3]),
                                      pack2bf(s[kb][8 * st + 4], s[kb][8 * st + 5]), pack2bf(s[kb][8 * st + 6], s[kb][8 * st + 7])};
                    const bf16x8 pf = __builtin_bit_cast(bf16x8, pw);
                    const int gq = l >> 4, li = l & 15, q4 = li >> 2, pp = li & 3;
#pragma unroll
                    for (int e = 0; e < EB; e++) {
                        const int key = 32 * kb + 16 * st + 4 * hh + q4;
                        const int byte = (32 * e + 16 * (gq & 1) + 4 * pp) * 2;
                        const lds_bf16x4* a0 = (const lds_bf16x4*)(cV + G::voff(key, byte));
                        const lds_bf16x4* a1 = (const lds_bf16x4*)(cV + G::voff(key + 8, byte));
                        const bf16x4 lo = __builtin_amdgcn_ds_read_tr16_b64_v4i16((lds_bf16x4*)a0);
                        const bf16x4 hi = __builtin_amdgcn_ds_read_tr16_b64_v4i16((lds_bf16x4*)a1);
                        const bf16x8 a = {lo[0], lo[1], lo[2], lo[3], hi[0], hi[1], hi[2], hi[3]};
                        o[e] = __builtin_amdgcn_mfma_f32_32x32x16_bf16(__builtin_bit_cast(mfma_bf16x8, a),
                                                                       __builtin_bit_cast(mfma_bf16x8, pf), o[e], 0, 0, 0);
                    }
                }
            }
            FPRIO_DOWN(2);
        }
        STAMP(6)
        __syncthreads();
        STAMP(7)
        store_kv(rk, rv);
        store_r(rr[0], i0 - (P + KT) - 64);
        STAMP(8)
        __syncthreads();
        STAMP(9)
    }
    STAMP(15)

    const float l_tot = l_run + __shfl_xor(l_run, 32, 64);
    const float inv = l_tot > 0.f ? 1.f / l_tot : 0.f;
    const int qi = iw0 + r;
    if (qi < T) {
        bf16_t* op = p.out + (size_t)b * p.o_bs + (size_t)qi * p.o_rs + (size_t)h * DH;
#pragma unroll
        for (int e = 0; e < EB; e++) {
#pragma unroll
            for (int grp = 0; grp < 4; grp++) {
                const int e0 = 32 * e + 8 * grp + 4 * hh;
                if (e0 < DH) {
                    u32x2 w = {pack2bf(o[e][4 * grp] * inv, o[e][4 * grp + 1] * inv),
                               pack2bf(o[e][4 * grp + 2] * inv, o[e][4 * grp + 3] * inv)};
                    *reinterpret_cast<u32x2*>(op + e0) = w;
                }
            }
        }
        const float lse2 = m_run + __builtin_amdgcn_logf(l_tot);
        if (hh == 0 && p.lse) p.lse[((size_t)b * p.H + h) * T + qi] = lse2 * 0.6931471805599453f;
        if (hh == 0 && p.ph_rec)
            reinterpret_cast<float*>(p.ph_rec + (((size_t)b * p.H + h) * (size_t)(T >> 5) + (iw0 >> 5)) * 4352 + 4096)[r] = -lse2;
    }
    STAMP(15)
    STAMP_FLUSH
}

template <int DH>
int launch_fwd(const RelAttnP& p, hipStream_t s) {
    using G = Geo<DH>;
    static bool attr_set = false;
    if (!attr_set) {
        hipError_t e = hipFuncSetAttribute(reinterpret_cast<const void*>(&relattn_fwd_kernel<DH>),
                                           hipFuncAttributeMaxDynamicSharedMemorySize, G::SMEM);
        if (e != hipSuccess) return (int)e;
        attr_set = true;
    }
    dim3 grid((p.T + QB - 1) / QB, p.H, p.B);
    {
        mxl_kt::Scope kt(MXL_KT_RELATTN_FWD, s);
        hipLaunchKernelGGL((relattn_fwd_kernel<DH>), grid, dim3(256), G::SMEM, s, p);
    }
    MXL_LAUNCH_CHECK();
    return MXL_OK;
}

}

#ifdef MXL_STAMP
extern "C" int mxl_debug_fwd_stamps(unsigned long long* host_out16) {
    hipError_t e = hipMemcpyFromSymbol(host_out16, HIP_SYMBOL(g_fwd_stamps), sizeof(unsigned long long) * 16);
    if (e != hipSuccess) return (int)e;
    unsigned long long z[16] = {0};
    e = hipMemcpyToSymbol(HIP_SYMBOL(g_fwd_stamps), z, sizeof(z));
    return (int)e;
}
#endif

static int relattn_fwd_launch(const void* q, const void* k, const void* v, const void* rd, const float* r_w_bias,
                              const float* r_r_bias, void* out, float* lse, int B, int T, int H, int dh, int M, int Kc,
                              long long q_bs, int q_rs, long long kv_bs, int kv_rs, int rd_rs, long long o_bs, int o_rs,
                              float scale, void* oph, float* mph, void* stream, int oph_all = 0, void* ph_ws = nullptr) {
    MXL_CHECK_ARG(q && k && v && rd && r_w_bias && r_r_bias && out);
    if (oph_all) MXL_CHECK_ARG(oph && ((T - Kc) % 64) == 0);
    if (ph_ws) MXL_CHECK_ARG(oph_all && dh == 64 && ((uintptr_t)ph_ws % 16) == 0);
    if (oph) MXL_CHECK_ARG(mph && (M % (oph_all ? 32 : 256)) == 0 && (T % 32) == 0 && ((uintptr_t)oph % 8) == 0);
    MXL_CHECK_ARG(B > 0 && T > 0 && H > 0 && M > 0 && Kc >= T && Kc <= M + T);
    MXL_CHECK_ARG((q_rs % 8) == 0 && (kv_rs % 8) == 0 && (rd_rs % 8) == 0 && (o_rs % 4) == 0);
    MXL_CHECK_ARG((q_bs % 8) == 0 && (kv_bs % 8) == 0 && (o_bs % 4) == 0);
    MXL_CHECK_ARG((long long)Kc * kv_rs * 2 < (1ll << 31) && (long long)M * rd_rs * 2 < (1ll << 31));
    MXL_CHECK_ARG(((uintptr_t)q % 16) == 0 && ((uintptr_t)k % 16) == 0 && ((uintptr_t)v % 16) == 0 &&
                  ((uintptr_t)rd % 16) == 0 && ((uintptr_t)out % 8) == 0);
    RelAttnP p;
    p.q = (const bf16_t*)q; p.k = (const bf16_t*)k; p.v = (const bf16_t*)v; p.rd = (const bf16_t*)rd;
    p.rwb = r_w_bias; p.rrb = r_r_bias; p.out = (bf16_t*)out; p.lse = lse;
    p.B = B; p.T = T; p.H = H; p.M = M; p.Kc = Kc;
    p.q_bs = q_bs; p.kv_bs = kv_bs; p.o_bs = o_bs; p.q_rs = q_rs; p.kv_rs = kv_rs; p.rd_rs = rd_rs; p.o_rs = o_rs;
    p.scale_log2e = scale * 1.4426950408889634f;
    p.oph = (bf16_t*)oph; p.mph = mph; p.oph_all = oph_all ? 1 : 0; p.ph_rec = (char*)ph_ws;
    hipStream_t s = (hipStream_t)stream;
    switch (dh) {
        case 16: return launch_fwd<16>(p, s);
        case 32: return launch_fwd<32>(p, s);
        case 64: return launch_fwd<64>(p, s);
        default: return MXL_EUNSUPPORTED;
    }
}

extern "C" int mxl_relattn_fwd(const void* q, const void* k, const void* v, const void* rd, const float* r_w_bias,
                               const float* r_r_bias, void* out, float* lse, int B, int T, int H, int dh, int M, int Kc,
                               long long q_bs, int q_rs, long long kv_bs, int kv_rs, int rd_rs, long long o_bs, int o_rs,
                               float scale, void* stream) {
    return relattn_fwd_launch(q, k, v, rd, r_w_bias, r_r_bias, out, lse, B, T, H, dh, M, Kc, q_bs, q_rs, kv_bs, kv_rs, rd_rs, o_bs,
                              o_rs, scale, nullptr, nullptr, stream);
}

extern "C" int mxl_relattn_fwd_phantom(const void* q, const void* k, const void* v, const void* rd, const float* r_w_bias,
                                       const float* r_r_bias, void* out, float* lse, void* oph, float* mph, int B, int T, int H,
                                       int dh, int M, int Kc, long long q_bs, int q_rs, long long kv_bs, int kv_rs, int rd_rs,
                                       long long o_bs, int o_rs, float scale, void* stream) {
    MXL_CHECK_ARG(oph && mph);
    return relattn_fwd_launch(q, k, v, rd, r_w_bias, r_r_bias, out, lse, B, T, H, dh, M, Kc, q_bs, q_rs, kv_bs, kv_rs, rd_rs, o_bs,
                              o_rs, scale, oph, mph, stream);
}

extern "C" int mxl_relattn_fwd_phantom2(const void* q, const void* k, const void* v, const void* rd, const float* r_w_bias,
                                        const float* r_r_bias, void* out, float* lse, void* oph, float* mph, int oph_all, void* ph_ws,
                                        int B, int T, int H, int dh, int M, int Kc, long long q_bs, int q_rs, long long kv_bs, int kv_rs,
                                        int rd_rs, long long o_bs, int o_rs, float scale, void* stream) {
    MXL_CHECK_ARG(oph && mph);
    return relattn_fwd_launch(q, k, v, rd, r_w_bias, r_r_bias, out, lse, B, T, H, dh, M, Kc, q_bs, q_rs, kv_bs, kv_rs, rd_rs, o_bs,
                              o_rs, scale, oph, mph, stream, oph_all, ph_ws);
}
```

symbolic_music_generation_amd/ops.py:

```python
import ctypes as C
import math
import os
from typing import Optional, Sequence

import torch

from ._lib import lib, check, MusicXLError

GEMM_OUT_F32 = 0x01
GEMM_OUT_F32_ATOMIC = 0x02
GEMM_BIAS = 0x04
GEMM_RELU = 0x08
GEMM_DROPOUT = 0x10
GEMM_RELU_BWD = 0x20
GEMM_ADD_AUX = 0x40
GEMM_SAVE_RELU_MASK = 0x100
GEMM_RELU_BWD_BITS = 0x200


def mix_seed(base_seed: int, step: int) -> int:
    import torch.distributed as dist
    rank = dist.get_rank() if (dist.is_available() and dist.is_initialized()) else 0
    x = (base_seed * 0x9E3779B97F4A7C15 + rank * 0xD1B54A32D192ED03 + step * 0x2545F4914F6CDD1D) & 0xFFFFFFFFFFFFFFFF
    x ^= x >> 32
# ... 544 lines not shown
        check(lib().mxl_ln_residual_bwd_colsum(_p(dy), _p(dy2), _p(z), _p(mean), _p(rstd), _p(gamma), _p(dres), _p(dx),
                                               _p(dgamma), _p(dbeta), _p(dxsum), N, d, float(drop_p), seed, site, _stream()),
              'mxl_ln_residual_bwd_colsum')
        return
    check(lib().mxl_ln_residual_bwd(_p(dy), _p(dy2), _p(z), _p(mean), _p(rstd), _p(gamma), _p(dres), _p(dx),
                                    _p(dgamma), _p(dbeta), N, d, float(drop_p), seed, site, _stream()),
          'mxl_ln_residual_bwd')
    if dxsum is not None:
        colsum(dx, dxsum, N, d)


def ln_bwd_add(dy, dy2, z, mean, rstd, gamma, dadd, dres, dgamma, dbeta):
    d = z.shape[-1]
    N = z.numel() // d
    check(lib().mxl_ln_residual_bwd_add(_p(dy), _p(dy2), _p(z), _p(mean), _p(rstd), _p(gamma), _p(dadd), _p(dres), _p(dgamma),
                                        _p(dbeta), N, d, _stream()), 'mxl_ln_residual_bwd_add')


def ln_bwd_add_drop(dy, dy2, z, mean, rstd, gamma, dadd, dres, dx, dxsum, dgamma, dbeta, p: float, seed: int, site: int):
    d = z.shape[-1]
    N = z.numel() // d
    check(lib().mxl_ln_residual_bwd_add_drop(_p(dy), _p(dy2), _p(z), _p(mean), _p(rstd), _p(gamma), _p(dadd), _p(dres), _p(dx),
                                             _p(dxsum), _p(dgamma), _p(dbeta), N, d, float(p), seed, site, _stream()),
          'mxl_ln_residual_bwd_add_drop')


def dropout_colsum(x: torch.Tensor, y: torch.Tensor, out: torch.Tensor, M: int, N: int, p: float, seed: int, site: int):
    check(lib().mxl_dropout_colsum_bf16(_p(x), _p(y), _p(out), M, N, float(p), seed, site, _stream()), 'mxl_dropout_colsum_bf16')


def colsum(x: torch.Tensor, out: torch.Tensor, M: int, N: int, ld: Optional[int] = None):
    check(lib().mxl_colsum_bf16(_p(x), _p(out), M, N, ld if ld is not None else x.stride(-2), _stream()), 'mxl_colsum_bf16')
    return out


def mem_update(mem, hid, out):
    B, M, d = mem.shape
    T = hid.shape[1]
    check(lib().mxl_mem_update(_p(mem), _p(hid), _p(out), B, M, T, d, _stream()), 'mxl_mem_update')
    return out


def phantom_sum_applies(*, T, dh, M, Kc) -> bool:
    return (dh == 64 and T % 32 == 0 and M % 256 == 0 and Kc < M + T and os.environ.get('MXL_NO_DQ8') != '1'
            and os.environ.get('MXL_DG_RECOMPUTE', '1') != '0' and os.environ.get('MXL_NO_OPH') != '1')


def set_reserved_cus(k: int) -> None:
    global _RESERVED_CUS
    check(lib().mxl_set_reserved_cus(int(k)), 'mxl_set_reserved_cus')
    _RESERVED_CUS = int(k)


_RESERVED_CUS = 0
_N_CUS = {}
FUSED_OWNER_MIN_FILL = 0.9


def fused_dq_owner_mode(B, H, cus, reserved=0, env=None) -> bool:
    ov = (env or {}).get('MXL_FUSED_OWNER')
    if ov in ('0', '1'):
        return ov == '1'
    usable = max(int(cus) - int(reserved), 8)
    wgs = int(B) * int(H)
    rounds = (wgs + usable - 1) // usable
    return wgs >= FUSED_OWNER_MIN_FILL * rounds * usable


def _n_cus(device) -> int:
    key = str(device)
    if key not in _N_CUS:
        _N_CUS[key] = int(torch.cuda.get_device_properties(device).multi_processor_count)
    return _N_CUS[key]


def fused_bwd_applies(*, T, dh, M, Kc, B=None, H=None) -> bool:
    ok = (dh == 64 and T % 32 == 0 and M % 32 == 0 and M <= 8192 and Kc % 32 == 0 and (T - Kc) % 64 == 0
          and os.environ.get('MXL_NO_FUSED_BWD') != '1')
    if ok and B is not None and H is not None and Kc < M + T:
        ok = H * (T // 32) * 4352 < 2 ** 31 and B * H * T * 4 < 2 ** 31
    return ok


def relattn_fwd(q, k, v, rd, r_w_bias, r_r_bias, out, lse, *, B, T, H, dh, M, Kc, q_bs, q_rs, kv_bs, kv_rs, rd_rs,
                o_bs, o_rs, scale=None, oph=None, mph=None, oph_all=False, ph_buf=None):
    scale = scale if scale is not None else 1.0 / math.sqrt(dh)
    if oph is not None and oph_all:
        check(lib().mxl_relattn_fwd_phantom2(_p(q), _p(k), _p(v), _p(rd), _p(r_w_bias), _p(r_r_bias), _p(out), _p(lse), _p(oph),
                                             _p(mph), 1, _p(ph_buf), B, T, H, dh, M, Kc, q_bs, q_rs, kv_bs, kv_rs, rd_rs, o_bs, o_rs,
                                             float(scale), _stream()), 'mxl_relattn_fwd_phantom2')
        return out
    if oph is not None:
        check(lib().mxl_relattn_fwd_phantom(_p(q), _p(k), _p(v), _p(rd), _p(r_w_bias), _p(r_r_bias), _p(out), _p(lse), _p(oph),
                                            _p(mph), B, T, H, dh, M, Kc, q_bs, q_rs, kv_bs, kv_rs, rd_rs, o_bs, o_rs, float(scale),
                                            _stream()), 'mxl_relattn_fwd_phantom')
        return out
    check(lib().mxl_relattn_fwd(_p(q), _p(k), _p(v), _p(rd), _p(r_w_bias), _p(r_r_bias), _p(out), _p(lse), B, T, H, dh,
                                M, Kc, q_bs, q_rs, kv_bs, kv_rs, rd_rs, o_bs, o_rs, float(scale), _stream()),
          'mxl_relattn_fwd')
    return out


def label_guard(labels: torch.Tensor, eos: int):
    _req(labels, torch.int64, 'labels')
    check(lib().mxl_label_guard(_p(labels), labels.shape[1], int(eos), _stream()), 'mxl_label_guard')


def adaptive_nll_fwd(logits, labels, nll, lse, acc2, B, T, V, cutoffs=()):
    n, arr = _cut(cutoffs)
    check(lib().mxl_adaptive_nll_fwd(_p(logits), logits.stride(0), _p(labels), _p(nll), _p(lse), _p(acc2), B, T, V, n,
                                     C.cast(arr, C.c_void_p) if arr is not None else None, _stream()),
          'mxl_adaptive_nll_fwd')


def adaptive_nll_bwd(logits, labels, nll, lse, acc2, dlogits, B, T, V, cutoffs=(), grad_scale=1.0, dlogits_lo=None):
    n, arr = _cut(cutoffs)
    if dlogits_lo is not None:
        assert dlogits_lo.shape == dlogits.shape and dlogits_lo.stride(0) == dlogits.stride(0)
        check(lib().mxl_adaptive_nll_bwd_split(_p(logits), logits.stride(0), _p(labels), _p(nll), _p(lse), _p(acc2), _p(dlogits),
                                               _p(dlogits_lo), dlogits.stride(0), B, T, V, n,
                                               C.cast(arr, C.c_void_p) if arr is not None else None, float(grad_scale),
                                               _stream()), 'mxl_adaptive_nll_bwd_split')
        return
    check(lib().mxl_adaptive_nll_bwd(_p(logits), logits.stride(0), _p(labels), _p(nll), _p(lse), _p(acc2), _p(dlogits),
                                     dlogits.stride(0), B, T, V, n,
                                     C.cast(arr, C.c_void_p) if arr is not None else None, float(grad_scale), _stream()),
          'mxl_adaptive_nll_bwd')


def adaptive_logprob(logits, out, N, V, cutoffs=()):
    n, arr = _cut(cutoffs)
    check(lib().mxl_adaptive_logprob(_p(logits), logits.stride(0), _p(out), out.stride(0), N, V, n,
                                     C.cast(arr, C.c_void_p) if arr is not None else None, _stream()),
          'mxl_adaptive_logprob')
    return out


def cluster_bucket(labels, V, cutoffs, perm, counts, tgt_head, tgt_tail):
    B, T = labels.shape
    n, arr = _cut(cutoffs)
    check(lib().mxl_cluster_bucket(_p(labels), B, T, V, n, C.cast(arr, C.c_void_p), _p(perm), _p(counts), _p(tgt_head),
                                   _p(tgt_tail), _stream()), 'mxl_cluster_bucket')


def gather_rows(src, idx, dst, n):
    check(lib().mxl_gather_rows_bf16(_p(src), src.stride(-2), _p(idx), _p(dst), n, src.shape[-1], _stream()), 'mxl_gather_rows_bf16')
    return dst


def scatter_add_rows(src, idx, dst, n):
    check(lib().mxl_scatter_add_rows_bf16(_p(src), _p(idx), _p(dst), dst.stride(-2), n, src.shape[-1], _stream()),
          'mxl_scatter_add_rows_bf16')


def rows_lse_pick(logits, ncols, n_rows, tgt, lse_out, pick_out, rows_idx=None, row0=0):
    check(lib().mxl_rows_lse_pick(_p(logits), logits.stride(0), ncols, n_rows, _p(rows_idx), row0, _p(tgt), _p(lse_out),
                                  _p(pick_out), _stream()), 'mxl_rows_lse_pick')


def bucket_nll_finish(hlse, hpick, tlse, tpick, tgt_head, tgt_tail, nll, nll_tok, acc2, B, T):
    check(lib().mxl_bucket_nll_finish(_p(hlse), _p(hpick), _p(tlse), _p(tpick), _p(tgt_head), _p(tgt_tail), _p(nll), _p(nll_tok),
                                      _p(acc2), B, T, _stream()), 'mxl_bucket_nll_finish')


def rows_softmax_grad(logits, ncols, n_rows, tgt, lse, nll_tok, acc2, grad_scale, out_hi, out_lo=None, rows_idx=None, row0=0):
    check(lib().mxl_rows_softmax_grad(_p(logits), logits.stride(0), ncols, n_rows, _p(rows_idx), row0, _p(tgt), _p(lse), _p(nll_tok),
                                      _p(acc2), float(grad_scale), _p(out_hi), _p(out_lo), out_hi.stride(0), _stream()),
          'mxl_rows_softmax_grad')

# ... 46 lines not shown
def add_rowbias(x, x_bs, x_rs, bias, out, B, T, n):
    check(lib().mxl_add_rowbias_bf16(_p(x), x_bs, x_rs, _p(bias), _p(out), B, T, n, _stream()), 'mxl_add_rowbias_bf16')
    return out


def relattn_bwd(q, k, v, rd, r_w_bias, r_r_bias, out, dout, lse, delta, dq, dk, dv, dg, d_rwb, d_rrb, *, B, T, H, dh, M,
                Kc, q_bs, q_rs, kv_bs, kv_rs, rd_rs, o_bs, o_rs, dq_bs, dq_rs, dkv_bs, dkv_rs, scale=None,
                d_rd: Optional[torch.Tensor] = None, qr_buf: Optional[torch.Tensor] = None, defer_drd: bool = False,
                oph: Optional[torch.Tensor] = None, mph: Optional[torch.Tensor] = None):
    scale = scale if scale is not None else 1.0 / math.sqrt(dh)
    fused_rrb = (d_rd is not None and dg is not None and dh == 64 and T % 32 == 0 and M % 8 == 0 and M >= 8
                 and os.environ.get('MXL_NO_DQ8') != '1')
    Bc = B if dg is None else min(B, dg.shape[0])
    sparse = fused_rrb and M % 256 == 0 and Kc < M + T and os.environ.get('MXL_DG_RECOMPUTE', '1') != '0'
    assert oph is None or sparse, 'oph / mph are for the shapes phantom_sum_applies() accepts, with d_rd / dg given'

    def launch(b0, n):
        sl = slice(b0, b0 + n)
        if sparse and oph is not None:
            check(lib().mxl_relattn_bwd_sparse_dg_oph(_p(q[sl]), _p(k[sl]), _p(v[sl]), _p(rd), _p(r_w_bias), _p(r_r_bias),
                                                      _p(out[sl]), _p(dout[sl]), _p(lse[sl]), _p(delta[sl]), _p(dq[sl]), _p(dk[sl]),
                                                      _p(dv[sl]), _p(dg), _p(d_rwb), _p(oph[sl]), _p(mph[sl]), n, T, H, dh, M, Kc,
                                                      q_bs, q_rs, kv_bs, kv_rs, rd_rs, o_bs, o_rs, dq_bs, dq_rs, dkv_bs, dkv_rs,
                                                      float(scale), _stream()), 'mxl_relattn_bwd_sparse_dg_oph')
            return
        if sparse:
            check(lib().mxl_relattn_bwd_sparse_dg(_p(q[sl]), _p(k[sl]), _p(v[sl]), _p(rd), _p(r_w_bias), _p(r_r_bias), _p(out[sl]),
                                                  _p(dout[sl]), _p(lse[sl]), _p(delta[sl]), _p(dq[sl]), _p(dk[sl]), _p(dv[sl]),
                                                  _p(dg), _p(d_rwb), n, T, H, dh, M, Kc, q_bs, q_rs, kv_bs, kv_rs, rd_rs, o_bs,
                                                  o_rs, dq_bs, dq_rs, dkv_bs, dkv_rs, float(scale), _stream()),
                  'mxl_relattn_bwd_sparse_dg')
            return
        check(lib().mxl_relattn_bwd(_p(q[sl]), _p(k[sl]), _p(v[sl]), _p(rd), _p(r_w_bias), _p(r_r_bias), _p(out[sl]), _p(dout[sl]),
                                    _p(lse[sl]), _p(delta[sl]), _p(dq[sl]), _p(dk[sl]), _p(dv[sl]), _p(dg), _p(d_rwb),
                                    None if fused_rrb else _p(d_rrb), n, T, H, dh, M, Kc, q_bs, q_rs, kv_bs, kv_rs, rd_rs, o_bs,
                                    o_rs, dq_bs, dq_rs, dkv_bs, dkv_rs, float(scale), _stream()), 'mxl_relattn_bwd')

    def drd(b0, n):
        if d_rd is not None:
            relattn_drd(q[b0:b0 + n], r_r_bias, dg, d_rd, qr_buf, B=n, T=T, H=H, dh=dh, M=M, q_bs=q_bs, q_rs=q_rs,
                        rd=rd if fused_rrb else None, rd_rs=rd_rs, d_rrb=d_rrb if fused_rrb else None,
                        d_rwb=d_rwb if fused_rrb else None,
                        recompute=dict(lse=lse[b0:b0 + n], delta=delta[b0:b0 + n], scale=scale, Kc=Kc) if sparse else None)

    if Bc >= B:
        launch(0, B)
        if defer_drd:
            return lambda: drd(0, B)
        drd(0, B)
        return None
    for b0 in range(0, B, Bc):
        n = min(Bc, B - b0)
        launch(b0, n)
        drd(b0, n)
    return (lambda: None) if defer_drd else None


def relattn_bwd_fused_ws_numel(B, T, H, dh, M) -> int:
    return int(lib().mxl_relattn_bwd_fused_ws_bytes(B, T, H, dh, M)) // 4


_PH_WS = {}


def _phantom_ws(B, T, H, device):
    key = (B, T, H, str(device))
    buf = _PH_WS.get(key)
    if buf is None:
        buf = torch.empty(int(lib().mxl_relattn_drd_phantom_ws_bytes(B, T, H)), device=device, dtype=torch.uint8)
        _PH_WS[key] = buf
    return buf


def gemm_headdot(a, b, c, M, N, K, o, T, delta, lda=None, ldb=None, ldc=None, ldo=None):
    rc = lib().mxl_gemm_bf16_headdot(_p(a), _p(b), _p(c), M, N, K, lda or K, ldb or K, ldc or N, _p(o), ldo or N, T, _p(delta), _stream())
    if rc == -2:
        return False
    check(rc, 'mxl_gemm_bf16_headdot')
    return True


def relattn_bwd_fused(q, k, v, rd, r_w_bias, r_r_bias, out, dout, lse, delta, dq, dk, dv, d_rd, d_rwb, d_rrb, ws, qr_buf, *,
                      B, T, H, dh, M, Kc, q_bs, q_rs, kv_bs, kv_rs, rd_rs, o_bs, o_rs, dq_bs, dq_rs, dkv_bs, dkv_rs,
                      scale=None, oph=None, mph=None, defer_drd=False, ph_buf=None, ph_ready=False, delta_ready=False, dq_mode=None):
    scale = scale if scale is not None else 1.0 / math.sqrt(dh)
    d = H * dh
    if dq_mode is None:
        owner = fused_dq_owner_mode(B, H, _n_cus(q.device), _RESERVED_CUS, os.environ)
    else:
        if dq_mode not in ('owner', 'slabs'):
            raise ValueError(f'dq_mode must be None, "owner" or "slabs", not {dq_mode!r}')
        owner = dq_mode == 'owner'
    mode_bits = (2 if delta_ready else 0) | (4 if owner else 8)
    check(lib().mxl_relattn_bwd_fused(_p(q), _p(k), _p(v), _p(rd), _p(r_w_bias), _p(r_r_bias), _p(out), _p(dout), _p(lse), _p(delta),
                                      _p(dq), _p(dk), _p(dv), _p(d_rd), d_rd.stride(0), _p(d_rwb), _p(d_rrb), _p(oph), _p(mph), _p(ws),
                                      B, T, H, dh, M, Kc, q_bs, q_rs, kv_bs, kv_rs, rd_rs, o_bs, o_rs, dq_bs, dq_rs, dkv_bs, dkv_rs,
                                      float(scale), mode_bits, _stream()), 'mxl_relattn_bwd_fused')

    def phantom():
        if Kc < M + T:
            ph = ph_buf if ph_buf is not None else _phantom_ws(B, T, H, q.device)
            if not (ph_ready and ph_buf is not None):
                check(lib().mxl_relattn_drd_phantom_prep(_p(q), q_bs, q_rs, _p(r_r_bias), _p(lse), _p(ph), B, T, H, dh, float(scale),
                                                         _stream()), 'mxl_relattn_drd_phantom_prep')
            check(lib().mxl_relattn_drd_phantom(_p(ph), _p(delta), _p(d_rd), B, T, H, dh, M, d_rd.stride(0), _p(rd), int(rd_rs), Kc,
                                                _stream()), 'mxl_relattn_drd_phantom')
    if defer_drd:
        return phantom
    phantom()
    return None


def relattn_drd(q, r_r_bias, dg, d_rd, qr_buf, *, B, T, H, dh, M, q_bs, q_rs, rd=None, rd_rs=0, d_rrb=None, d_rwb=None,
                recompute=None):
    d = H * dh
    add_rowbias(q, q_bs, q_rs, r_r_bias.reshape(-1), qr_buf, B, T, d)
    if recompute is not None:
        check(lib().mxl_relattn_drd_recompute(_p(dg), _p(qr_buf), _p(d_rd), B, T, H, dh, M, T * d, d, d, _p(rd), int(rd_rs),
                                              _p(d_rrb), _p(d_rwb), _p(recompute['lse']), _p(recompute['delta']),
                                              float(recompute['scale']), int(recompute['Kc']), _stream()),
              'mxl_relattn_drd_recompute')
        return
    rc = lib().mxl_relattn_drd(_p(dg), _p(qr_buf), _p(d_rd), B, T, H, dh, M, T * d, d, d, _p(rd), int(rd_rs), _p(d_rrb),
                               _p(d_rwb), _stream())
    if rc == -2:
        assert d_rrb is None
        gemm_batched(dg, qr_buf, d_rd, M, dh, T, lda=M, ldb=d, ldc=d, trans_a=True, trans_b=True,
                     flags=GEMM_OUT_F32_ATOMIC, batch=B * H, bdiv=H, sA=(H * T * M, T * M), sB=(T * d, dh), sC=(0, dh))
    else:
        check(rc, 'mxl_relattn_drd')


def decode_embed(ids, t_dev, E, out, scale):
    B, d = out.shape
    check(lib().mxl_decode_embed(_p(ids), ids.stride(0), _p(t_dev), _p(E), _p(out), B, d, E.shape[0], float(scale),
                                 _stream()), 'mxl_decode_embed')


def kv_append(qkv, kc, vc, t_dev, rrb=None, qr_out=None):
    B, H, M, dh = kc.shape
    check(lib().mxl_kv_append(_p(qkv), _p(kc), _p(vc), _p(t_dev), B, M, H * dh, dh, _p(rrb), _p(qr_out), _stream()),
          'mxl_kv_append')


def kv_fill(qkv, kc, vc, T):
    B, H, M, dh = kc.shape
    check(lib().mxl_kv_fill(_p(qkv), _p(kc), _p(vc), B, T, M, H * dh, dh, _stream()), 'mxl_kv_fill')


def _req_fp8_rings(kc8, ke, vc8, ve, what):
    for t, dt in ((kc8, torch.uint8), (vc8, torch.uint8), (ke, torch.int8), (ve, torch.int8)):
        _req(t, dt, what)
        if not t.is_contiguous():
            raise MusicXLError(f'{what}: fp8 rings and their exponents must be contiguous')
    if kc8.dim() != 4 or vc8.shape != kc8.shape or ke.shape != kc8.shape[:3] or ve.shape != kc8.shape[:3]:
        raise MusicXLError(f'{what}: expected (B, H, M, dh) byte rings with (B, H, M) exponents')


def kv_append_fp8(qkv, kc8, ke, vc8, ve, t_dev, rrb=None, qr_out=None):
    _req_fp8_rings(kc8, ke, vc8, ve, 'kv_append_fp8')
    B, H, M, dh = kc8.shape
    check(lib().mxl_kv_append_fp8(_p(qkv), _p(kc8), _p(ke), _p(vc8), _p(ve), _p(t_dev), B, M, H * dh, dh, _p(rrb), _p(qr_out),
                                  _stream()), 'mxl_kv_append_fp8')


def kv_fill_fp8(qkv, kc8, ke, vc8, ve, T):
    _req_fp8_rings(kc8, ke, vc8, ve, 'kv_fill_fp8')
    B, H, M, dh = kc8.shape
    check(lib().mxl_kv_fill_fp8(_p(qkv), _p(kc8), _p(ke), _p(vc8), _p(ve), B, T, M, H * dh, dh, _stream()), 'mxl_kv_fill_fp8')


def kv_zero_pad(qkv, n_pad, B, T, d):
    _req(qkv, torch.bfloat16, 'kv_zero_pad qkv')
    _req(n_pad, torch.int32, 'kv_zero_pad n_pad')
    if not qkv.is_contiguous() or qkv.numel() != B * T * 3 * d or n_pad.numel() != B or not n_pad.is_contiguous():
        raise MusicXLError(f'kv_zero_pad: expected a contiguous ({B}, {T}, {3 * d}) qkv buffer and ({B},) n_pad')
    check(lib().mxl_kv_zero_pad(_p(qkv), _p(n_pad), B, T, d, _stream()), 'mxl_kv_zero_pad')


def decode_ring_pieces(B: int, H: int, M: int) -> int:
# ... 391 lines not shown
```

symbolic_music_generation_amd/xl_engine.py:

```python
import math
import os
from collections import OrderedDict
from typing import Dict, List, Optional, Sequence, Tuple

import torch

from . import ops
from ._lib import MusicXLError

F = ops


def _r8(n: int) -> int:
    return (n + 7) // 8 * 8


class ParamLayout:

    def __init__(self, cfg):
        d, Fi, H, dh, V, L = cfg.d_model, cfg.d_inner, cfg.n_head, cfg.d_head, cfg.vocab_size, cfg.n_layer
        ncl = len(cfg.cutoffs)
        self.n_head_rows = V + ncl
        self.head_rows_padded = _r8(V + ncl)
        decay: List[Tuple[str, Tuple[int, ...]]] = [('transformer.word_emb.emb_layers.0.weight', (V, d))]
        if ncl:
            decay.append(('crit.cluster_weight', (ncl, d)))
        if self.head_rows_padded > V + ncl:
            decay.append(('_pad.head_rows', (self.head_rows_padded - V - ncl, d)))
        nodecay: List[Tuple[str, Tuple[int, ...]]] = [('crit.out_layers.0.bias', (V,))]
        if ncl:
            nodecay.append(('crit.cluster_bias', (ncl,)))
        for l in range(L):
            p = f'transformer.layers.{l}.'
            decay += [(p + 'dec_attn.qkv_net.weight', (3 * H * dh, d)), (p + 'dec_attn.r_net.weight', (H * dh, d)),
                      (p + 'dec_attn.o_net.weight', (d, H * dh)), (p + 'pos_ff.CoreNet.0.weight', (Fi, d)),
                      (p + 'pos_ff.CoreNet.3.weight', (d, Fi))]
            nodecay += [(p + 'dec_attn.r_r_bias', (H, dh)), (p + 'dec_attn.r_w_bias', (H, dh)),
                        (p + 'dec_attn.layer_norm.weight', (d,)), (p + 'dec_attn.layer_norm.bias', (d,)),
                        (p + 'pos_ff.CoreNet.0.bias', (Fi,)), (p + 'pos_ff.CoreNet.3.bias', (d,)),
                        (p + 'pos_ff.layer_norm.weight', (d,)), (p + 'pos_ff.layer_norm.bias', (d,))]
        self.entries: "OrderedDict[str, Tuple[int, Tuple[int, ...]]]" = OrderedDict()
        off = 0
        for name, shape in decay:
            self.entries[name] = (off, shape)
            n = math.prod(shape)
            contiguous_next = name in ('transformer.word_emb.emb_layers.0.weight', 'crit.cluster_weight')
            off = off + n if contiguous_next else _r8(off + n)
        off = _r8(off)
        self.n_decay = off
        for name, shape in nodecay:
            self.entries[name] = (off, shape)
            n = math.prod(shape)
            off = off + n if (name == 'crit.out_layers.0.bias' and ncl) else _r8(off + n)
        self.total = _r8(off)

    def view(self, buf: torch.Tensor, name: str) -> torch.Tensor:
        off, shape = self.entries[name]
        return buf[off:off + math.prod(shape)].view(*shape)

    def real_names(self):
        return [n for n in self.entries if not n.startswith('_pad.')]


class _WS:
    pass


class XLEngine:
    SITE_EMB, SITE_POS, SITE_FINAL = 0, 1, 2

    def __init__(self, cfg, device, seed: int = 77):
        if not torch.cuda.is_available():
            raise MusicXLError('XLEngine needs a GPU: the product path has no CPU fallback')
        self.cfg = cfg
        self.dev = torch.device(device)
        assert cfg.d_model % 8 == 0 and cfg.d_inner % 8 == 0 and cfg.n_head * cfg.d_head == cfg.d_model
        assert cfg.d_head in (16, 32, 64), 'HIP attention kernels cover d_head 16/32/64 (all reference presets)'
        assert cfg.mem_len % 8 == 0 and cfg.mem_len > 0
        assert cfg.same_length and cfg.div_val == 1 and cfg.d_embed == cfg.d_model
        self.layout = ParamLayout(cfg)
        n = self.layout.total
        self.P = torch.zeros(n, device=self.dev, dtype=torch.float32)
        self.W = torch.zeros(n, device=self.dev, dtype=torch.bfloat16)
        self.G: Optional[torch.Tensor] = None
        self.m: Optional[torch.Tensor] = None
        self.v: Optional[torch.Tensor] = None
        self.WT: Optional[Dict[str, torch.Tensor]] = None
        self.step_count = 0
        self.rng_step = 0
        self.base_seed = seed
        self._ws: Dict[Tuple, _WS] = {}
        self._sumsq = torch.zeros(1, device=self.dev)
        self.bucketed_head = len(cfg.cutoffs) > 0 and cfg.vocab_size >= 16384
# ... 67 lines not shown
        for name in self.layout.real_names():
            sd[name] = self.p32(name).detach().cpu().clone()
        sd['crit.out_layers.0.weight'] = sd['transformer.word_emb.emb_layers.0.weight']
        return sd

    def load_state_dict(self, sd: Dict[str, torch.Tensor], strict: bool = True):
        missing = []
        for name in self.layout.real_names():
            if name in sd:
                self.p32(name).copy_(sd[name].to(torch.float32).reshape(self.layout.entries[name][1]))
            else:
                missing.append(name)
        if strict and missing:
            raise KeyError(f'missing parameters: {missing[:4]}...')
        self.sync_weights()

    def num_parameters(self) -> int:
        return sum(math.prod(self.layout.entries[n][1]) for n in self.layout.real_names())

    def _workspace(self, B, T, Kc, train) -> _WS:
        key = (B, T, Kc, train)
        ws = self._ws.get(key)
        if ws is not None:
            self._ws[key] = self._ws.pop(key)
            return ws
        same = [k for k in self._ws if k[-1] == train]
        for k in same[:max(0, len(same) - 1)]:
            del self._ws[k]
        c, dev = self.cfg, self.dev
        d, Fi, H, L, M = c.d_model, c.d_inner, c.n_head, c.n_layer, c.mem_len
        N = B * T
        bf = dict(device=dev, dtype=torch.bfloat16)
        f32 = dict(device=dev, dtype=torch.float32)
        ws = _WS()
        keep = L if train else 1
        ws.phi = torch.empty(M, d, **bf)
        ws.h = [torch.empty(N, d, **bf) for _ in range(L + 1)] if train else [torch.empty(N, d, **bf) for _ in range(2)]
        ws.cat = [torch.empty(B, Kc, d, **bf) for _ in range(keep)] if Kc > T else None
        ws.qkv = [torch.empty(B, Kc, 3 * d, **bf) for _ in range(keep)]
        ws.rd = [torch.empty(M, d, **bf) for _ in range(keep)]
        ws.av = [torch.empty(N, d, **bf) for _ in range(keep)]
        ws.lse = [torch.empty(B, H, T, **f32) for _ in range(keep)]
        ws.fused_bwd = train and ops.fused_bwd_applies(T=T, dh=c.d_head, M=M, Kc=Kc, B=B, H=H)
        use_oph = train and ((ws.fused_bwd and Kc < M + T) or ops.phantom_sum_applies(T=T, dh=c.d_head, M=M, Kc=Kc))
        ws.oph = [torch.empty(N, d, **bf) for _ in range(keep)] if use_oph else None
        ws.mph = [torch.empty(B, H, T, **f32) for _ in range(keep)] if use_oph else None
        ws.ph = ([torch.empty(int(ops.lib().mxl_relattn_drd_phantom_ws_bytes(B, T, H)), device=self.dev, dtype=torch.uint8)
                  for _ in range(keep)] if (use_oph and ws.fused_bwd) else None)
        ws.tmp = torch.empty(N, d, **bf)
        ws.h1 = [torch.empty(N, d, **bf) for _ in range(keep)]
        ws.a = [torch.empty(N, Fi, **bf) for _ in range(keep)]
        mb = ops.gemm_relu_mask_bytes(N, Fi) if train else 0
        ws.rmask = [torch.empty(mb, device=self.dev, dtype=torch.uint8) for _ in range(keep)] if mb else None
        if train:
            ws.z1 = [torch.empty(N, d, **bf) for _ in range(L)]
            ws.z2 = [torch.empty(N, d, **bf) for _ in range(L)]
            ws.st1 = [torch.empty(2, N, **f32) for _ in range(L)]
            ws.st2 = [torch.empty(2, N, **f32) for _ in range(L)]
            ws.hid_d = torch.empty(N, d, **bf)
            ws.dA = torch.empty(N, d, **bf)
            ws.dB = torch.empty(N, d, **bf)
            ws.dC = torch.empty(N, d, **bf)
            ws.dD = torch.empty(N, d, **bf)
            ws.dF = torch.empty(N, Fi, **bf)
            ws.dqkv = torch.empty(B, Kc, 3 * d, **bf)
            ws.delta = torch.empty(B, H, T, **f32)
            if ws.fused_bwd:
                ws.dg = None
                ws.dq_slabs = torch.empty(ops.relattn_bwd_fused_ws_numel(B, T, H, c.d_head, M), **f32)
                ws.qr = None
            else:
                ws.dg = torch.empty(B, H, T, M, **bf)
                ws.qr = torch.empty(B, T, d, **bf)
            ws.d_rd = torch.empty(M, d, **f32)
            ws.d_rd16 = torch.empty(M, d, **bf)
            ws.phi_c = torch.empty(M, d, **bf)
            if not self.bucketed_head:
                ws.dlogits = torch.empty(N, self._head_kp(), **bf)
                ws.dlogits_lo = torch.empty(N, self._head_kp(), **bf)
        ws.logits = torch.empty(N, self.layout.head_rows_padded, **f32) if not self.bucketed_head else None
        ws.nll = torch.empty(B, max(T - 1, 1), **f32)
        ws.hlse = torch.empty(N, 2, **f32)
        ws.acc = torch.zeros(2, **f32)
        self._ws[key] = ws
        return ws

    def _site(self, l, k):
        return 8 + 8 * l + k

    def forward(self, input_ids: torch.Tensor, mems: Optional[Sequence[torch.Tensor]] = None,
                labels: Optional[torch.Tensor] = None, train: bool = False, want_logprobs: bool = True, kv_sink=None,
                n_pad: Optional[torch.Tensor] = None):
        c = self.cfg
        B, T = input_ids.shape
        if n_pad is not None and (train or mems is not None):
            raise MusicXLError('n_pad (left-padded prompts) is only supported for an eval forward from zero mems')
        d, H, dh, L, M, Fi = c.d_model, c.n_head, c.d_head, c.n_layer, c.mem_len, c.d_inner
        V, cut = c.vocab_size, tuple(c.cutoffs)
        N = B * T
        has_mem = mems is not None
        Kc = T + (M if has_mem else 0)
        ws = self._workspace(B, T, Kc, train)
        p = float(c.dropout) if train else 0.0
        seed = ops.mix_seed(self.base_seed, self.rng_step)
        ids = input_ids.contiguous()
        ws.ids, ws.B, ws.T, ws.Kc, ws.p, ws.seed, ws.has_mem = ids, B, T, Kc, p, seed, has_mem

        ops.sinusoid_table(M, d, c.clamp_len, self.dev, drop_p=p, seed=seed, site=self.SITE_POS, out=ws.phi)
        E = self.w16('transformer.word_emb.emb_layers.0.weight')
        ops.embed_fwd(ids, E, ws.h[0], math.sqrt(d), drop_p=p, seed=seed, site=self.SITE_EMB)
        new_mems = [] if not train else None
        st = dict(B=B, T=T, H=H, dh=dh, M=M, Kc=Kc, q_bs=Kc * 3 * d, q_rs=3 * d, kv_bs=Kc * 3 * d, kv_rs=3 * d, rd_rs=d,
                  o_bs=T * d, o_rs=d)
        for l in range(L):
            s = l if train else 0
            h_in = ws.h[l] if train else ws.h[l & 1]
            h_out = ws.h[l + 1] if train else ws.h[(l + 1) & 1]
            if has_mem:
                cat = ws.cat[s]
                cat[:, :M].copy_(mems[l])
                cat[:, M:].copy_(h_in.view(B, T, d))
                x_qkv = cat.view(B * Kc, d)
            else:
                x_qkv = h_in
            if new_mems is not None:
                if has_mem:
                    new_mems.append(cat[:, Kc - M:].clone())
                elif T >= M:
                    new_mems.append(h_in.view(B, T, d)[:, T - M:].clone())
                else:
                    nm = torch.zeros(B, M, d, device=self.dev, dtype=torch.bfloat16)
                    nm[:, M - T:].copy_(h_in.view(B, T, d))
                    new_mems.append(nm)
            qkv = ws.qkv[s]
            ops.gemm(x_qkv, self._lw(l, 'dec_attn.qkv_net.weight'), qkv.view(B * Kc, 3 * d), B * Kc, 3 * d, d)
            if n_pad is not None:
                ops.kv_zero_pad(qkv, n_pad, B, T, d)
            if kv_sink is not None:
                kv_sink(l, qkv)
            ops.gemm(ws.phi, self._lw(l, 'dec_attn.r_net.weight'), ws.rd[s], M, d, d)
            ops.relattn_fwd(qkv[:, Kc - T:, :d], qkv[:, :, d:2 * d], qkv[:, :, 2 * d:], ws.rd[s],
                            self._lw(l, 'dec_attn.r_w_bias', self.P), self._lw(l, 'dec_attn.r_r_bias', self.P),
                            ws.av[s], ws.lse[s], oph=ws.oph[s].view(B, T, d) if (train and ws.oph is not None) else None,
                            mph=ws.mph[s] if (train and ws.oph is not None) else None,
                            oph_all=bool(train and getattr(ws, 'fused_bwd', False)),
                            ph_buf=ws.ph[s] if (train and ws.ph is not None) else None, **st)
            ops.gemm(ws.av[s], self._lw(l, 'dec_attn.o_net.weight'), ws.tmp, N, d, d)
            ops.ln_residual_fwd(ws.tmp, h_in, self._lw(l, 'dec_attn.layer_norm.weight', self.P),
                                self._lw(l, 'dec_attn.layer_norm.bias', self.P), ws.h1[s],
                                ws.z1[l] if train else None, ws.st1[l][0] if train else None,
                                ws.st1[l][1] if train else None, eps=c.layer_norm_epsilon, drop_p=p, seed=seed,
                                site=self._site(l, 0))
            fl = F.GEMM_BIAS | F.GEMM_RELU | (F.GEMM_DROPOUT if p > 0 else 0)
            save_bits = train and ws.rmask is not None
            ops.gemm(ws.h1[s], self._lw(l, 'pos_ff.CoreNet.0.weight'), ws.a[s], N, Fi, d,
                     flags=fl | (F.GEMM_SAVE_RELU_MASK if save_bits else 0), aux=ws.rmask[s] if save_bits else None,
                     bias=self._lw(l, 'pos_ff.CoreNet.0.bias', self.P), drop_p=p, seed=seed, site=self._site(l, 1))
            ops.gemm(ws.a[s], self._lw(l, 'pos_ff.CoreNet.3.weight'), ws.tmp, N, d, Fi, flags=F.GEMM_BIAS,
                     bias=self._lw(l, 'pos_ff.CoreNet.3.bias', self.P))
            ops.ln_residual_fwd(ws.tmp, ws.h1[s], self._lw(l, 'pos_ff.layer_norm.weight', self.P),
                                self._lw(l, 'pos_ff.layer_norm.bias', self.P), h_out,
                                ws.z2[l] if train else None, ws.st2[l][0] if train else None,
                                ws.st2[l][1] if train else None, eps=c.layer_norm_epsilon, drop_p=p, seed=seed,
                                site=self._site(l, 2))
        hid = ws.h[L] if train else ws.h[L & 1]
        if p > 0:
            ops.dropout(hid, ws.hid_d, p, seed=seed, site=self.SITE_FINAL)
            hid = ws.hid_d
        ws.hid = hid
        nrow = self.layout.n_head_rows
        head_w = self.W[:self.layout.head_rows_padded * d].view(self.layout.head_rows_padded, d)
        boff = self.layout.entries['crit.out_layers.0.bias'][0]
        head_b = self.P[boff:boff + nrow]
        out = dict(loss=None, losses=None, logprobs=None, mems=new_mems)
        if self.bucketed_head:
            if labels is not None:
                lab = labels.contiguous().clone()
                ops.label_guard(lab, c.eos_token_id)
                ws.labels = lab
                ws.acc.zero_()
                self._bucketed_nll_fwd(ws, hid, lab, B, T)
                out['losses'] = ws.nll
                out['loss'] = ws.acc[0] / ws.acc[1]
            if want_logprobs and (labels is None or not train):
                out['logprobs'] = self._chunked_logprobs(hid, N, head_w, head_b).view(B, T, V)
            self._last = ws
            return out
        ops.gemm(hid, head_w, ws.logits, N, nrow, d, flags=F.GEMM_OUT_F32 | F.GEMM_BIAS, bias=head_b)
        if labels is not None:
            lab = labels.contiguous().clone()
            ops.label_guard(lab, c.eos_token_id)
            ws.labels = lab
            ws.acc.zero_()
            ops.adaptive_nll_fwd(ws.logits, lab, ws.nll, ws.hlse, ws.acc, B, T, V, cut)
            out['losses'] = ws.nll
            out['loss'] = ws.acc[0] / ws.acc[1]
        if want_logprobs and (labels is None or not train):
            lp = torch.empty(N, V, device=self.dev, dtype=torch.float32)
            ops.adaptive_logprob(ws.logits, lp, N, V, cut)
            out['logprobs'] = lp.view(B, T, V)
        self._last = ws
        return out

    HEAD_CHUNK_BYTES = 1 << 30

    def _hb_scratch(self, N):
        c, dev = self.cfg, self.dev
        hb = self._hb
        ncl, c1, d = len(c.cutoffs), c.cutoffs[0], c.d_model
        if hb is None or hb.N != N:
            hb = self._hb = _WS()
            hb.N = N
            i32 = dict(device=dev, dtype=torch.int32)
            f32 = dict(device=dev, dtype=torch.float32)
            hb.perm = torch.empty(ncl + 2, N, **i32)
            hb.counts = torch.zeros(ncl + 2, **i32)
            hb.tgt_head, hb.tgt_tail = torch.empty(N, **i32), torch.empty(N, **i32)
            hb.hlse, hb.hpick, hb.tlse, hb.tpick = (torch.zeros(N, **f32) for _ in range(4))
            hb.nll_tok = torch.empty(N, **f32)
            hb.ldh = _r8(c1 + ncl)
            hb.wp = torch.zeros(hb.ldh, d, device=dev, dtype=torch.bfloat16)
            hb.bp = torch.zeros(hb.ldh, **f32)
        return hb

    def _chunk_rows(self, n, cols):
        ch = max(256, (self.HEAD_CHUNK_BYTES // (4 * max(cols, 1))) // 256 * 256)
        return min(n, ch)

    def _pack_head(self, hb):
# ... 111 lines not shown
            self.G.zero_()

    @staticmethod
    def _ks(m, n, k=0):
        tiles = ((m + 127) // 128) * ((n + 127) // 128)
        if k >= 49152:
            return 12 if tiles <= 48 else max(1, min(24, 1440 // tiles))
        return max(1, min(24, 512 // max(tiles, 1)))

    def backward(self, grad_scale: float = 1.0, layer_done=None):
        ws, c = self._last, self.cfg
        B, T, Kc, p, seed = ws.B, ws.T, ws.Kc, ws.p, ws.seed
        d, H, dh, L, M, Fi = c.d_model, c.n_head, c.d_head, c.n_layer, c.mem_len, c.d_inner
        V, cut = c.vocab_size, tuple(c.cutoffs)
        if self.WT is None:
            self._refresh_wt(allocate=True)
        N = B * T
        G = self.G
        nrow, nrow_p = self.layout.n_head_rows, self.layout.head_rows_padded
        AT = F.GEMM_OUT_F32_ATOMIC
        dscale = 1.0 / (1.0 - p) if p > 0 else 1.0

        def gw(l, suffix):
            return self._lw(l, suffix, G)

        dy, dy2 = ws.dA, None
        if self.bucketed_head:
            self._bucketed_head_bwd(ws, dy, B, T, grad_scale)
        else:
            ops.adaptive_nll_bwd(ws.logits, ws.labels, ws.nll, ws.hlse, ws.acc, ws.dlogits, B, T, V, cut, grad_scale,
                                 dlogits_lo=ws.dlogits_lo)
            head_w = self.W[:nrow_p * d].view(nrow_p, d)
            g_head_w = G[:nrow_p * d].view(nrow_p, d)
            boff = self.layout.entries['crit.out_layers.0.bias'][0]
            for term in (ws.dlogits_lo, ws.dlogits):
                ops.colsum(term, G[boff:boff + nrow], N, nrow)
                ops.gemm(term, ws.hid, g_head_w, nrow_p, d, N, trans_a=True, trans_b=True, flags=AT,
                         ksplits=self._ks(nrow_p, d, N))
            ops.gemm(ws.dlogits_lo, self.WT['head'], dy, N, d, self._head_kp())
            ops.gemm(ws.dlogits, self.WT['head'], dy, N, d, self._head_kp(), flags=F.GEMM_ADD_AUX, aux=dy)
        if p > 0:
            ops.dropout(dy, dy, p, seed=seed, site=self.SITE_FINAL)
        st = dict(B=B, T=T, H=H, dh=dh, M=M, Kc=Kc, q_bs=Kc * 3 * d, q_rs=3 * d, kv_bs=Kc * 3 * d, kv_rs=3 * d, rd_rs=d,
                  o_bs=T * d, o_rs=d)
        ops.center_columns(ws.phi, ws.phi_c)
        for l in reversed(range(L)):
            h_in = ws.h[l]
            ops.ln_residual_bwd(dy, dy2, ws.z2[l], ws.st2[l][0], ws.st2[l][1], self._lw(l, 'pos_ff.layer_norm.weight', self.P),
                                ws.dC, ws.dD, gw(l, 'pos_ff.layer_norm.weight'), gw(l, 'pos_ff.layer_norm.bias'),
                                drop_p=p, seed=seed, site=self._site(l, 2), dxsum=gw(l, 'pos_ff.CoreNet.3.bias'))
            ops.gemm(ws.dD, ws.a[l], gw(l, 'pos_ff.CoreNet.3.weight'), d, Fi, N, trans_a=True, trans_b=True, flags=AT,
                     ksplits=self._ks(d, Fi, N))
            if ws.rmask is not None:
                ops.gemm(ws.dD, self._lwt(l, 'pos_ff.CoreNet.3.weight'), ws.dF, N, Fi, d, flags=F.GEMM_RELU_BWD_BITS,
                         aux=ws.rmask[l], alpha=dscale, colsum=gw(l, 'pos_ff.CoreNet.0.bias'))
            else:
                ops.gemm(ws.dD, self._lwt(l, 'pos_ff.CoreNet.3.weight'), ws.dF, N, Fi, d, flags=F.GEMM_RELU_BWD,
                         aux=ws.a[l], alpha=dscale, colsum=gw(l, 'pos_ff.CoreNet.0.bias'))
            ops.gemm(ws.dF, ws.h1[l], gw(l, 'pos_ff.CoreNet.0.weight'), Fi, d, N, trans_a=True, trans_b=True, flags=AT,
                     ksplits=self._ks(Fi, d, N))
            ops.gemm(ws.dF, self._lwt(l, 'pos_ff.CoreNet.0.weight'), ws.dD, N, d, Fi)
            ops.ln_residual_bwd(ws.dC, ws.dD, ws.z1[l], ws.st1[l][0], ws.st1[l][1],
                                self._lw(l, 'dec_attn.layer_norm.weight', self.P), ws.dA, ws.dB,
                                gw(l, 'dec_attn.layer_norm.weight'), gw(l, 'dec_attn.layer_norm.bias'), drop_p=p,
                                seed=seed, site=self._site(l, 0))
            ops.gemm(ws.dB, ws.av[l], gw(l, 'dec_attn.o_net.weight'), d, d, N, trans_a=True, trans_b=True, flags=AT,
                     ksplits=self._ks(d, d, N))
            delta_ready = False
            if ws.fused_bwd and not os.environ.get('MXL_HEADDOT_OFF'):
                delta_ready = ops.gemm_headdot(ws.dB, self._lwt(l, 'dec_attn.o_net.weight'), ws.dC, N, d, d, ws.av[l], T, ws.delta)
            else:
                ops.gemm(ws.dB, self._lwt(l, 'dec_attn.o_net.weight'), ws.dC, N, d, d)
            qkv, dqkv = ws.qkv[l], ws.dqkv
            ws.d_rd.zero_()
            if ws.fused_bwd:
                ops.relattn_bwd_fused(qkv[:, Kc - T:, :d], qkv[:, :, d:2 * d], qkv[:, :, 2 * d:], ws.rd[l],
                                      self._lw(l, 'dec_attn.r_w_bias', self.P), self._lw(l, 'dec_attn.r_r_bias', self.P), ws.av[l],
                                      ws.dC, ws.lse[l], ws.delta, dqkv[:, Kc - T:, :d], dqkv[:, :, d:2 * d], dqkv[:, :, 2 * d:],
                                      ws.d_rd, gw(l, 'dec_attn.r_w_bias'), gw(l, 'dec_attn.r_r_bias'), ws.dq_slabs, ws.qr,
                                      dq_bs=Kc * 3 * d, dq_rs=3 * d, dkv_bs=Kc * 3 * d, dkv_rs=3 * d,
                                      oph=ws.oph[l].view(B, T, d) if ws.oph is not None else None,
                                      mph=ws.mph[l] if ws.oph is not None else None,
                                      ph_buf=ws.ph[l] if ws.ph is not None else None, ph_ready=ws.ph is not None,
                                      delta_ready=delta_ready, **st)
            else:
                ops.relattn_bwd(qkv[:, Kc - T:, :d], qkv[:, :, d:2 * d], qkv[:, :, 2 * d:], ws.rd[l],
                                self._lw(l, 'dec_attn.r_w_bias', self.P), self._lw(l, 'dec_attn.r_r_bias', self.P), ws.av[l],
                                ws.dC, ws.lse[l], ws.delta, dqkv[:, Kc - T:, :d], dqkv[:, :, d:2 * d], dqkv[:, :, 2 * d:],
                                ws.dg, gw(l, 'dec_attn.r_w_bias'), gw(l, 'dec_attn.r_r_bias'), dq_bs=Kc * 3 * d, dq_rs=3 * d,
                                dkv_bs=Kc * 3 * d, dkv_rs=3 * d, d_rd=ws.d_rd, qr_buf=ws.qr,
                                oph=ws.oph[l].view(B, T, d) if ws.oph is not None else None,
                                mph=ws.mph[l] if ws.oph is not None else None, **st)
            ops.cast_bf16(ws.d_rd, ws.d_rd16)
            ops.gemm(ws.d_rd16, ws.phi_c, gw(l, 'dec_attn.r_net.weight'), d, d, M, trans_a=True, trans_b=True, flags=AT,
                     ksplits=self._ks(d, d))
            if ws.has_mem:
                dqkv[:, :M, :d].zero_()
                x_qkv = ws.cat[l].view(B * Kc, d)
            else:
                x_qkv = h_in
            ops.gemm(dqkv.view(B * Kc, 3 * d), x_qkv, gw(l, 'dec_attn.qkv_net.weight'), 3 * d, d, B * Kc, trans_a=True,
                     trans_b=True, flags=AT, ksplits=self._ks(3 * d, d, B * Kc))
            if ws.has_mem:
                ops.gemm_batched(dqkv[:, M:], self._lw(l, 'dec_attn.qkv_net.weight'), ws.dB, T, d, 3 * d, lda=3 * d,
                                 ldb=d, ldc=d, trans_b=True, batch=B, bdiv=1, sA=(Kc * 3 * d, 0), sB=(0, 0), sC=(T * d, 0))
            else:
                ops.gemm(dqkv.view(N, 3 * d), self._lwt(l, 'dec_attn.qkv_net.weight'), ws.dB, N, d, 3 * d)
            dy, dy2 = ws.dA, ws.dB
            if layer_done is not None:
                layer_done(l)
        E_g = self.layout.view(G, 'transformer.word_emb.emb_layers.0.weight')
        ops.embed_bwd(ws.ids, dy, E_g, math.sqrt(d), drop_p=p, seed=seed, site=self.SITE_EMB, dout2=dy2)

    def optimizer_step(self, lr: float, betas=(0.9, 0.999), eps=1e-8, weight_decay=0.01, max_grad_norm=1.0,
                       grad_scale: float = 1.0):
        if self.m is None:
            self.m = torch.zeros_like(self.P)
            self.v = torch.zeros_like(self.P)
        self.step_count += 1
        self.rng_step += 1
        self._sumsq.zero_()
        if max_grad_norm and max_grad_norm > 0:
            ops.sumsq(self.G, self._sumsq)
        ops.adamw_step(self.P, self.G, self.m, self.v, self.W, self.layout.n_decay, lr, betas[0], betas[1], eps,
                       weight_decay, self.step_count, self._sumsq if max_grad_norm else None, max_grad_norm or 0.0,
                       grad_scale)
        self._refresh_wt()

    def grad_norm(self) -> torch.Tensor:
        return self._sumsq.sqrt()
```

Measured before the change: 928,300 tokens/s.

## Store attention probabilities in forward and reuse them in fused backward

Adds a probability store: the forward attention kernel writes the banded attention probabilities (16-bit, per 32x32 block) plus per-tile reference maxima. The fused backward kernel then loads and rescales those probabilities instead of recomputing QK^T and the relative-position term. This is meant to remove the recompute MFMAs and the positional G-block work in backward. In exchange it adds a large per-layer memory buffer and extra HBM write and read traffic. It is enabled automatically when owner dq mode is selected and half of free memory can hold the buffer.

New measurement: 911,500 tokens/s. -1.8%, worse.

```diff
diff --git a/include/musicxl.h b/include/musicxl.h
--- a/include/musicxl.h
+++ b/include/musicxl.h
@@ -97,6 +97,19 @@
                              const float* r_r_bias, void* out, float* lse, void* oph, float* mph, int oph_all, void* ph_ws, int B,
                              int T, int H, int dh, int M, int Kc, long long q_bs, int q_rs, long long kv_bs, int kv_rs, int rd_rs,
                              long long o_bs, int o_rs, float scale, void* stream);
+size_t mxl_relattn_pstore_bytes(int B, int T, int H, int M, int Kc);
+size_t mxl_relattn_pstore_ref_bytes(int B, int T, int H, int M, int Kc);
+int mxl_relattn_fwd_pstore(const void* q, const void* k, const void* v, const void* rd, const float* r_w_bias,
+                           const float* r_r_bias, void* out, float* lse, void* oph, float* mph, void* ph_ws, void* pst, float* pst_ref,
+                           int B, int T, int H, int dh, int M, int Kc, long long q_bs, int q_rs, long long kv_bs, int kv_rs, int rd_rs,
+                           long long o_bs, int o_rs, float scale, void* stream);
+int mxl_relattn_bwd_fused_pstore(const void* q, const void* k, const void* v, const void* rd, const float* r_w_bias,
+                                 const float* r_r_bias, const void* out, const void* dout, const float* lse, float* delta,
+                                 void* dq, void* dk, void* dv, float* d_rd, int drd_ld, float* d_r_w_bias, float* d_r_r_bias,
+                                 const void* oph, const float* mph, void* ws, const void* pst, const float* pst_ref, int B, int T, int H,
+                                 int dh, int M, int Kc, long long q_bs, int q_rs, long long kv_bs, int kv_rs, int rd_rs, long long o_bs,
+                                 int o_rs, long long dq_bs, int dq_rs, long long dkv_bs, int dkv_rs, float scale, int defer_finish,
+                                 void* stream);
 size_t mxl_relattn_drd_phantom_ws_bytes(int B, int T, int H);
 int mxl_relattn_drd_phantom_prep(const void* q, long long q_bs, int q_rs, const float* r_r_bias, const float* lse, void* ws, int B, int T,
                                  int H, int dh, float scale, void* stream);
diff --git a/symbolic_music_generation_amd/csrc/pstore_layout.h b/symbolic_music_generation_amd/csrc/pstore_layout.h
--- /dev/null
+++ b/symbolic_music_generation_amd/csrc/pstore_layout.h
@@ -0,0 +1,17 @@
+#pragma once
+
+#if defined(__HIPCC__) || defined(__CUDACC__)
+#define PST_HD __host__ __device__ __forceinline__
+#else
+#define PST_HD inline
+#endif
+
+constexpr int PST_BLOCK_BYTES = 2048;
+
+PST_HD int pst_row_lo(int qb, int a, int MB) { return (qb - MB > a) ? qb - MB : a; }
+PST_HD int pst_row_off(int qb, int a, int MB) {
+    const int c = a + MB + 1;
+    const int g = qb < c ? qb : c;
+    return g * (g - 1) / 2 + g * (1 - a) + (qb - g) * (MB + 1);
+}
+PST_HD int pst_tiles64(int Kc) { return (Kc + 63) >> 6; }
diff --git a/symbolic_music_generation_amd/csrc/relattn_bwd_fused.hip b/symbolic_music_generation_amd/csrc/relattn_bwd_fused.hip
--- a/symbolic_music_generation_amd/csrc/relattn_bwd_fused.hip
+++ b/symbolic_music_generation_amd/csrc/relattn_bwd_fused.hip
@@ -2,6 +2,7 @@
 #include <type_traits>
 #include "common.h"
 #include "musicxl_internal.h"
+#include "pstore_layout.h"
 
 namespace {
 
@@ -97,6 +98,8 @@
     long long q_bs, kv_bs, o_bs, dkv_bs, slab_stride;
     int q_rs, kv_rs, rd_rs, o_rs, dkv_rs, drd_ld;
     float scale, scale_log2e;
+    const char* pst;
+    const float* pst_ref;
 };
 
 __device__ __forceinline__ int qswz(int row) { return (((row >> 1) & 1) << 2) | (((row >> 2) & 1) << 1) | ((row >> 3) & 1); }
@@ -188,7 +191,7 @@
     }
 }
 
-template <bool OWNER>
+template <bool OWNER, bool PSTORE>
 __global__ __launch_bounds__(512, 1) void relattn_bwd_fused_kernel(FusedP p) {
     constexpr int NT = 512;
     constexpr int VM_PER_TILE = OWNER ? VM_PER_TILE_OWNER : VM_PER_TILE_BLOCK;
@@ -260,7 +263,15 @@
     const __amdgpu_buffer_rsrc_t rs_mph = __builtin_amdgcn_make_buffer_rsrc(
         (void*)(has_ph ? p.mph + ((size_t)b * p.H + h) * T : p.lse), 0, has_ph ? T * 4 : 0, 0x00020000);
     u32x4 tq = {0u, 0u, 0u, 0u}, t2 = {0u, 0u, 0u, 0u};
-    float tl = 0.f, tdl = 0.f, tm = 0.f;
+    float tl = 0.f, tdl = 0.f, tm = 0.f, tref = 0.f;
+    const int a32 = p0 >> 5, NQ = T >> 5, NKT = pst_tiles64(p.Kc);
+    const int pst_bh_bytes = pst_row_off(NQ, a32, MB) * PST_BLOCK_BYTES;
+    const __amdgpu_buffer_rsrc_t rs_p = __builtin_amdgcn_make_buffer_rsrc(
+        (void*)(PSTORE ? p.pst + ((size_t)b * p.H + h) * (size_t)pst_bh_bytes : (const char*)p.q), 0, PSTORE ? pst_bh_bytes : 0, 0x00020000);
+    const __amdgpu_buffer_rsrc_t rs_ref = __builtin_amdgcn_make_buffer_rsrc(
+        (void*)(PSTORE ? p.pst_ref + ((size_t)b * p.H + h) * (size_t)NQ * NKT * 32 : p.lse), 0, PSTORE ? NQ * NKT * 128 : 0, 0x00020000);
+    float* sFac = reinterpret_cast<float*>(sG);
+    u32x4 pc[2] = {{0u, 0u, 0u, 0u}, {0u, 0u, 0u, 0u}}, pn[2] = {{0u, 0u, 0u, 0u}, {0u, 0u, 0u, 0u}};
 #define STG_IDS int tid_o = tid; asm volatile("" : "+v"(tid_o)); const int srow_ = (tid_o & 255) >> 3, sch_ = tid_o & 7;
     auto load_stage = [&](int it, int nblk) {
         STG_IDS
@@ -274,6 +285,19 @@
         tl = __builtin_bit_cast(float, __builtin_amdgcn_raw_buffer_load_b32(rs_lse, (tid & 31) * 4, I * 4, 0));
         tdl = __builtin_bit_cast(float, __builtin_amdgcn_raw_buffer_load_b32(rs_dl, (tid & 31) * 4, I * 4, 0));
         if (OWNER) tm = __builtin_bit_cast(float, __builtin_amdgcn_raw_buffer_load_b32(rs_mph, (tid & 31) * 4, I * 4, 0));
+        if (PSTORE) tref = __builtin_bit_cast(float, __builtin_amdgcn_raw_buffer_load_b32(rs_ref, (tid & 127) * 4, (it * NKT + 4 * bx_) * 128, 0));
+    };
+    auto load_p = [&](int itn, u32x4 (&dst)[2]) {
+        const int pb = a32 + 8 * bx_ + w, lo = pst_row_lo(itn, a32, MB);
+        const bool vis = pb >= lo && pb <= itn;
+        const int so = vis ? (pst_row_off(itn, a32, MB) + pb - lo) * PST_BLOCK_BYTES : 0;
+        const int vo = vis ? l * 16 : 0x7ffff000;
+#ifdef MXL_ABL_PST_NOLOAD
+        dst[0] = u32x4{0x3c003c00u, 0x3c003c00u, 0x3c003c00u, 0x3c003c00u} + (uint32_t)(so & vo & 1); dst[1] = dst[0];
+#else
+        dst[0] = __builtin_bit_cast(u32x4, __builtin_amdgcn_raw_buffer_load_b128(rs_p, vo, so, 0));
+        dst[1] = __builtin_bit_cast(u32x4, __builtin_amdgcn_raw_buffer_load_b128(rs_p, vo, so + 1024, 0));
+#endif
     };
     auto store_stage = [&](int buf, int slot) {
         STG_IDS
@@ -305,6 +329,7 @@
             sLse[tid] = -tl * LOG2E; sLse[QT + tid] = -p.scale * tdl;
             if (OWNER) sLse[2 * QT + tid] = tm;
         }
+        if (PSTORE && tid < 128) sFac[buf * 128 + tid] = __builtin_amdgcn_exp2f(tref - tl * LOG2E);
     };
     auto slot_add = [&](int s, int k) { const int x = s + k; return x >= RING_BLKS ? x - RING_BLKS : x; };
     auto gblock = [&](int j, int s0, const bf16x8 (&bq)[4]) {
@@ -458,7 +483,7 @@
         asm volatile("" : "+v"(l_));
         lane_consts(l_);
     }
-    {
+    if (!PSTORE) {
         bf16x8 bq[4];
 #pragma unroll
         for (int ks = 0; ks < 4; ks++) bq[ks] = *reinterpret_cast<const bf16x8*>(sQ + QIMG + (rowq ^ (ks << 5)));
@@ -466,6 +491,7 @@
         if (w == 0) gblock(8, rs0, bq);
     }
     load_stage(min(it_lo + 1, it_hi), ((it_lo * QT - P0 - KBLK) >> 5) + 9);
+    if (PSTORE) load_p(it_lo, pc);
     __syncthreads();
 
 #pragma unroll
@@ -507,6 +533,7 @@
         load_stage(min(it + 2, it_hi), n0 + 10);
 #endif
 #endif
+        if (PSTORE) load_p(min(it + 1, it_hi), pn);
         if (FUSED_PARK) park_read();
         STAMP(0)
 
@@ -539,7 +566,57 @@
                     tqw_[st][e] = tr_pair(sQw + lo, sQw + hi);
                 }
         };
-        if (active) {
+        if (PSTORE && active) {
+            bf16x8 ad[4];
+            f32x16 s, dp, pt;
+#pragma unroll
+            for (int grp = 0; grp < 4; grp++) {
+                const f32x4 cd = *reinterpret_cast<const f32x4*>(sLse + QT + 8 * grp + 4 * hh);
+#pragma unroll
+                for (int t = 0; t < 4; t++) { dp[4 * grp + t] = cd[t]; pt[4 * grp + t] = 0.f; }
+            }
+#pragma unroll
+            for (int ks = 0; ks < 4; ks++) ad[ks] = *reinterpret_cast<const bf16x8*>(sDO + (rowq ^ (ks << 5)));
+            f32x4 fc[4];
+#pragma unroll
+            for (int grp = 0; grp < 4; grp++) fc[grp] = *reinterpret_cast<const f32x4*>(sFac + cur * 128 + 32 * (w >> 1) + 8 * grp + 4 * hh);
+#ifdef MXL_ABL_PST_NOTRANS
+#pragma unroll
+            for (int j = 0; j < 16; j++) pt[j] = __builtin_bit_cast(float, pc[j >> 3][j & 3] << 16);
+#endif
+            u32x4 sb[2];
+            {
+                int ls = l;
+                asm volatile("" : "+v"(ls));
+                const int n = ls & 31;
+                const uint32_t selv = ((ls >> 5) == ((n >> 2) & 1)) ? (0x3F80u << (16 * (n & 1))) : 0u;
+                const int selp = (n >> 4) * 4 + ((n >> 3) & 1) * 2 + ((n >> 1) & 1);
+#pragma unroll
+                for (int i = 0; i < 8; i++) sb[i >> 2][i & 3] = (selp == i) ? selv : 0u;
+            }
+            PRIO_UP();
+#ifndef MXL_ABL_PST_NOTRANS
+#pragma unroll
+            for (int st = 0; st < 2; st++) pt = mfma32(__builtin_bit_cast(bf16x8, pc[st]), __builtin_bit_cast(bf16x8, sb[st]), pt);
+#endif
+#pragma unroll
+            for (int ks = 0; ks < 4; ks++) dp = mfma32(ad[ks], vf[ks], dp);
+            PRIO_DOWN();
+#pragma unroll
+            for (int j = 0; j < 16; j++) {
+                const float pv = pt[j] * fc[j >> 2][j & 3];
+                pt[j] = pv;
+                s[j] = pv * dp[j];
+            }
+#pragma unroll
+            for (int m = 0; m < 8; m++) { dsw[m] = pack2bf(s[2 * m], s[2 * m + 1]); prw[m] = pack2bf(pt[2 * m], pt[2 * m + 1]); }
+            if (FUSED_TRF_EARLY || !FUSED_DVDK_LATE) tr_frags();
+#pragma unroll
+            for (int grp = 0; grp < 4; grp++)
+                *reinterpret_cast<u32x2*>(sX + (xw ^ (grp << 4))) = u32x2{dsw[2 * grp], dsw[2 * grp + 1]};
+            yskew_write16(yWb, dsw);
+            if (!FUSED_DVDK_LATE) dvdk();
+        } else if (active) {
             bf16x8 aq[4], ad[4], kfl[4];
             f32x16 s, dp;
 #pragma unroll
@@ -548,11 +625,13 @@
 #pragma unroll
                 for (int t = 0; t < 4; t++) s[4 * grp + t] = cl[t];
             }
+#ifndef MXL_ABL_PSTORE_CEIL
 #pragma unroll
             for (int ks = 0; ks < 4; ks++) {
                 aq[ks] = *reinterpret_cast<const bf16x8*>(sQw + (rowq ^ (ks << 5)));
                 kfl[ks] = *reinterpret_cast<const bf16x8*>(sK + (krow ^ (ks << 5)));
             }
+#endif
             __builtin_amdgcn_sched_barrier(0);
 #pragma unroll
             for (int grp = 0; grp < 4; grp++) {
@@ -563,8 +642,10 @@
 #pragma unroll
             for (int ks = 0; ks < 4; ks++) ad[ks] = *reinterpret_cast<const bf16x8*>(sDO + (rowq ^ (ks << 5)));
             PRIO_UP();
+#ifndef MXL_ABL_PSTORE_CEIL
 #pragma unroll
             for (int ks = 0; ks < 4; ks++) s = mfma32(aq[ks], kfl[ks], s);
+#endif
             __builtin_amdgcn_sched_barrier(0);
 #if FUSED_VF_RELOAD
             bf16x8 vfl[4];
@@ -580,12 +661,21 @@
             for (int ks = 0; ks < 4; ks++) dp = mfma32(ad[ks], vf[ks], dp);
 #endif
             PRIO_DOWN();
+            f32x16 pr;
+#ifdef MXL_ABL_PSTORE_CEIL
+#pragma unroll
+            for (int j = 0; j < 16; j++) {
+                const float pv = s[j] * -0.001f;
+                pr[j] = pv;
+                s[j] = pv * dp[j];
+            }
+            {
+#else
             uint32_t bdu[16];
             gskew_read16(gRb, bdu);
             STAMP(1)
             gskew_wait();
             STAMP(2)
-            f32x16 pr;
             const bool fl = __builtin_amdgcn_readfirstlane((int)full) != 0;
             if (fl) {
 #pragma unroll
@@ -606,6 +696,7 @@
                     pr[j] = pv;
                     s[j] = pv * (valid ? dp[j] : 0.f);
                 }
+#endif
             }
 #pragma unroll
             for (int m = 0; m < 8; m++) { dsw[m] = pack2bf(s[2 * m], s[2 * m + 1]); prw[m] = pack2bf(pr[2 * m], pr[2 * m + 1]); }
@@ -696,7 +787,8 @@
             const char* sQrN = sQ + (cur ^ 1) * QSET + QIMG;
             const int rs1 = slot_add(rs0, 1);
             bf16x8 gq_[4], ga[4];
-            {
+#ifndef MXL_ABL_PSTORE_CEIL
+            if (!PSTORE) {
                 const char* rb = sR + slot_add(rs1, w) * RBLK_BYTES;
 #pragma unroll
                 for (int ks = 0; ks < 4; ks++) {
@@ -704,6 +796,7 @@
                     ga[ks] = *reinterpret_cast<const bf16x8*>(rb + (rows ^ (ks << 5)));
                 }
             }
+#endif
             UNIT_FENCE();
             if (OWNER) {
 #pragma unroll
@@ -768,7 +861,8 @@
             STAMP(7)
             if (FUSED_PARK) drd_park(leave); else drd_add(leave, n0);
             STAMP(8)
-            if (more) {
+#ifndef MXL_ABL_PSTORE_CEIL
+            if (!PSTORE && more) {
                 f32x16 g;
 #pragma unroll
                 for (int t = 0; t < 16; t++) g[t] = 0.f;
@@ -800,6 +894,9 @@
                     }
                 }
             }
+#else
+            (void)sQrN; (void)rs1; (void)gq_; (void)ga;
+#endif
             STAMP(9)
             STAMP(10)
         }
@@ -807,6 +904,7 @@
         STAMP(12)
         cur ^= 1;
         rs0 = (rs0 == RING_BLKS - 1) ? 0 : rs0 + 1;
+        if (PSTORE) { pc[0] = pn[0]; pc[1] = pn[1]; }
     }
     {
         const int n0_end = ((it_hi + 1) * QT - P0 - KBLK) >> 5;
@@ -982,18 +1080,21 @@
     return (size_t)((M + KBLK - 1) / KBLK + 1) * (size_t)B * T * H * 64 * sizeof(slab_t);
 }
 
-extern "C" int mxl_relattn_bwd_fused(const void* q, const void* k, const void* v, const void* rd, const float* r_w_bias,
-                                     const float* r_r_bias, const void* out, const void* dout, const float* lse, float* delta,
-                                     void* dq, void* dk, void* dv, float* d_rd, int drd_ld, float* d_r_w_bias, float* d_r_r_bias,
-                                     const void* oph, const float* mph, void* ws, int B, int T, int H, int dh, int M, int Kc,
-                                     long long q_bs, int q_rs, long long kv_bs, int kv_rs, int rd_rs, long long o_bs, int o_rs,
-                                     long long dq_bs, int dq_rs, long long dkv_bs, int dkv_rs, float scale, int defer_finish,
-                                     void* stream) {
+static int bwd_fused_launch(const void* q, const void* k, const void* v, const void* rd, const float* r_w_bias,
+                            const float* r_r_bias, const void* out, const void* dout, const float* lse, float* delta,
+                            void* dq, void* dk, void* dv, float* d_rd, int drd_ld, float* d_r_w_bias, float* d_r_r_bias,
+                            const void* oph, const float* mph, void* ws, const void* pst, const float* pst_ref, int B, int T, int H, int dh,
+                            int M, int Kc, long long q_bs, int q_rs, long long kv_bs, int kv_rs, int rd_rs, long long o_bs, int o_rs,
+                            long long dq_bs, int dq_rs, long long dkv_bs, int dkv_rs, float scale, int defer_finish, void* stream) {
     MXL_CHECK_ARG(q && k && v && rd && r_w_bias && r_r_bias && out && dout && lse && delta && dq && dk && dv && d_rd && d_r_w_bias &&
                   d_r_r_bias && ws);
     if (dh != 64) return MXL_EUNSUPPORTED;
     MXL_CHECK_ARG(B > 0 && T > 0 && H > 0 && M > 0 && Kc >= T && Kc <= M + T && drd_ld >= H * 64);
     if ((T % 32) != 0 || (M % 32) != 0 || (Kc % 32) != 0) return MXL_EUNSUPPORTED;
+    if (pst) {
+        MXL_CHECK_ARG(pst_ref && ((uintptr_t)pst % 16) == 0);
+        if (mxl_relattn_pstore_bytes(B, T, H, M, Kc) == 0) return MXL_EUNSUPPORTED;
+    }
     MXL_CHECK_ARG(Kc == M + T || (oph && mph));
     MXL_CHECK_ARG((q_rs % 8) == 0 && (kv_rs % 8) == 0 && (rd_rs % 8) == 0 && (o_rs % 8) == 0 && (dq_rs % 8) == 0 && (dkv_rs % 4) == 0);
     MXL_CHECK_ARG((q_bs % 8) == 0 && (kv_bs % 8) == 0 && (o_bs % 8) == 0 && (dq_bs % 8) == 0 && (dkv_bs % 4) == 0);
@@ -1003,10 +1104,12 @@
     hipStream_t s = (hipStream_t)stream;
     static bool attr_set = false;
     if (!attr_set) {
-        hipError_t e = hipFuncSetAttribute(reinterpret_cast<const void*>(&relattn_bwd_fused_kernel<false>), hipFuncAttributeMaxDynamicSharedMemorySize, SMEM);
-        if (e == hipSuccess)
-            e = hipFuncSetAttribute(reinterpret_cast<const void*>(&relattn_bwd_fused_kernel<true>), hipFuncAttributeMaxDynamicSharedMemorySize, SMEM);
-        if (e != hipSuccess) return (int)e;
+        const void* kernels[4] = {reinterpret_cast<const void*>(&relattn_bwd_fused_kernel<false, false>), reinterpret_cast<const void*>(&relattn_bwd_fused_kernel<true, false>),
+                                  reinterpret_cast<const void*>(&relattn_bwd_fused_kernel<false, true>), reinterpret_cast<const void*>(&relattn_bwd_fused_kernel<true, true>)};
+        for (const void* kn : kernels) {
+            const hipError_t e = hipFuncSetAttribute(kn, hipFuncAttributeMaxDynamicSharedMemorySize, SMEM);
+            if (e != hipSuccess) return (int)e;
+        }
         attr_set = true;
     }
     const bool delta_ready = (defer_finish & 2) != 0;
@@ -1029,14 +1132,43 @@
     p.scale = scale; p.scale_log2e = scale * LOG2E;
     p.dq = (bf16_t*)dq; p.dq_bs = dq_bs; p.dq_rs = dq_rs;
     p.oph = (Kc < M + T) ? (const bf16_t*)oph : nullptr; p.mph = mph;
+    p.pst = (const char*)pst; p.pst_ref = pst_ref;
     {
         mxl_kt::Scope kt(MXL_KT_RELATTN_FUSED, s);
-        if (owner) hipLaunchKernelGGL(relattn_bwd_fused_kernel<true>, dim3(1, H, B), dim3(512), SMEM, s, p);
-        else hipLaunchKernelGGL(relattn_bwd_fused_kernel<false>, dim3((Kc + KBLK - 1) / KBLK, H, B), dim3(512), SMEM, s, p);
+        const dim3 grid_o(1, H, B), grid_b((Kc + KBLK - 1) / KBLK, H, B);
+        if (owner && pst) hipLaunchKernelGGL((relattn_bwd_fused_kernel<true, true>), grid_o, dim3(512), SMEM, s, p);
+        else if (owner) hipLaunchKernelGGL((relattn_bwd_fused_kernel<true, false>), grid_o, dim3(512), SMEM, s, p);
+        else if (pst) hipLaunchKernelGGL((relattn_bwd_fused_kernel<false, true>), grid_b, dim3(512), SMEM, s, p);
+        else hipLaunchKernelGGL((relattn_bwd_fused_kernel<false, false>), grid_b, dim3(512), SMEM, s, p);
     }
     MXL_LAUNCH_CHECK();
     if (defer_finish || owner) return MXL_OK;
     return mxl_relattn_dq_finish(ws, oph, mph, lse, delta, dq, d_r_r_bias, B, T, H, dh, M, Kc, o_bs, o_rs, dq_bs, dq_rs, scale, stream);
+}
+
+extern "C" int mxl_relattn_bwd_fused(const void* q, const void* k, const void* v, const void* rd, const float* r_w_bias,
+                                     const float* r_r_bias, const void* out, const void* dout, const float* lse, float* delta,
+                                     void* dq, void* dk, void* dv, float* d_rd, int drd_ld, float* d_r_w_bias, float* d_r_r_bias,
+                                     const void* oph, const float* mph, void* ws, int B, int T, int H, int dh, int M, int Kc,
+                                     long long q_bs, int q_rs, long long kv_bs, int kv_rs, int rd_rs, long long o_bs, int o_rs,
+                                     long long dq_bs, int dq_rs, long long dkv_bs, int dkv_rs, float scale, int defer_finish,
+                                     void* stream) {
+    return bwd_fused_launch(q, k, v, rd, r_w_bias, r_r_bias, out, dout, lse, delta, dq, dk, dv, d_rd, drd_ld, d_r_w_bias, d_r_r_bias, oph,
+                            mph, ws, nullptr, nullptr, B, T, H, dh, M, Kc, q_bs, q_rs, kv_bs, kv_rs, rd_rs, o_bs, o_rs, dq_bs, dq_rs, dkv_bs,
+                            dkv_rs, scale, defer_finish, stream);
+}
+
+extern "C" int mxl_relattn_bwd_fused_pstore(const void* q, const void* k, const void* v, const void* rd, const float* r_w_bias,
+                                            const float* r_r_bias, const void* out, const void* dout, const float* lse, float* delta,
+                                            void* dq, void* dk, void* dv, float* d_rd, int drd_ld, float* d_r_w_bias, float* d_r_r_bias,
+                                            const void* oph, const float* mph, void* ws, const void* pst, const float* pst_ref, int B,
+                                            int T, int H, int dh, int M, int Kc, long long q_bs, int q_rs, long long kv_bs, int kv_rs,
+                                            int rd_rs, long long o_bs, int o_rs, long long dq_bs, int dq_rs, long long dkv_bs, int dkv_rs,
+                                            float scale, int defer_finish, void* stream) {
+    MXL_CHECK_ARG(pst && pst_ref);
+    return bwd_fused_launch(q, k, v, rd, r_w_bias, r_r_bias, out, dout, lse, delta, dq, dk, dv, d_rd, drd_ld, d_r_w_bias, d_r_r_bias, oph,
+                            mph, ws, pst, pst_ref, B, T, H, dh, M, Kc, q_bs, q_rs, kv_bs, kv_rs, rd_rs, o_bs, o_rs, dq_bs, dq_rs, dkv_bs,
+                            dkv_rs, scale, defer_finish, stream);
 }
 
 extern "C" int mxl_relattn_dq_finish(const void* ws, const void* oph, const float* mph, const float* lse, const float* delta, void* dq,
diff --git a/symbolic_music_generation_amd/csrc/relattn_fwd.hip b/symbolic_music_generation_amd/csrc/relattn_fwd.hip
--- a/symbolic_music_generation_amd/csrc/relattn_fwd.hip
+++ b/symbolic_music_generation_amd/csrc/relattn_fwd.hip
@@ -1,6 +1,7 @@
 #include <type_traits>
 #include "common.h"
 #include "musicxl_internal.h"
+#include "pstore_layout.h"
 
 namespace {
 
@@ -20,6 +21,8 @@
     float* mph;
     int oph_all;
     char* ph_rec;
+    char* pst;
+    float* pst_ref;
 };
 
 constexpr int QB = 128;
@@ -112,7 +115,7 @@
 constexpr float RESCALE_THRESH = 8.0f;
 constexpr float FAST_SUM_MAX = 8192.0f;
 
-template <int DH>
+template <int DH, bool PST = false>
 __global__ __launch_bounds__(256, 2) void relattn_fwd_kernel(RelAttnP p) {
     using G = Geo<DH>;
     constexpr int KS = G::KS, EB = G::EB;
@@ -445,6 +448,13 @@
     __syncthreads();
 
     bool have_ring = false;
+    constexpr int PST_OOB = 0x7ffff000;
+    const int pst_bh_bytes = PST ? pst_row_off(T >> 5, p0 >> 5, M >> 5) * PST_BLOCK_BYTES : 0;
+    const int pref_bh_bytes = PST ? (T >> 5) * pst_tiles64(p.Kc) * 128 : 0;
+    const __amdgpu_buffer_rsrc_t rs_pst = __builtin_amdgcn_make_buffer_rsrc(
+        (void*)(PST ? p.pst + ((size_t)b * p.H + h) * (size_t)pst_bh_bytes : (char*)p.out), 0, pst_bh_bytes, 0x00020000);
+    const __amdgpu_buffer_rsrc_t rs_pref = __builtin_amdgcn_make_buffer_rsrc(
+        (void*)(PST ? (char*)p.pst_ref + ((size_t)b * p.H + h) * (size_t)pref_bh_bytes : (char*)p.out), 0, pref_bh_bytes, 0x00020000);
     auto rescale_o = [&](float alpha) __attribute__((always_inline)) {
 #pragma unroll
         for (int e = 0; e < EB; e++)
@@ -461,6 +471,7 @@
         STAMP(0)
         const int dmin_w = iw0 - P - (KT - 1), dmax_w = iw0 + 31 - P;
         const bool active = (dmax_w >= 0) && (dmin_w <= M - 1) && (iw0 < T);
+        u32x4 pws[2][2];
         if (active) {
             const char* cK = sK;
             const char* cV = sV;
@@ -593,6 +604,7 @@
                     const u32x4 pw = {pack2bf(s[kb][8 * st], s[kb][8 * st + 1]), pack2bf(s[kb][8 * st + 2], s[kb][8 * st + 3]),
                                       pack2bf(s[kb][8 * st + 4], s[kb][8 * st + 5]), pack2bf(s[kb][8 * st + 6], s[kb][8 * st + 7])};
                     const bf16x8 pf = __builtin_bit_cast(bf16x8, pw);
+                    if (PST) pws[kb][st] = pw;
                     const int gq = l >> 4, li = l & 15, q4 = li >> 2, pp = li & 3;
 #pragma unroll
                     for (int e = 0; e < EB; e++) {
@@ -609,6 +621,25 @@
                 }
             }
             FPRIO_DOWN(2);
+        } else if (PST) {
+#pragma unroll
+            for (int i = 0; i < 4; i++) asm volatile("" : "=v"(pws[i >> 1][i & 1]));
+        }
+        if (PST) {
+            const int qb = iw0 >> 5, a32 = p0 >> 5, MB = M >> 5, lo = pst_row_lo(qb, a32, MB);
+            bool any = false;
+#pragma unroll
+            for (int kb = 0; kb < 2; kb++) {
+                const int pb = (P >> 5) + kb;
+                const bool vis = active && pb >= lo && pb <= qb;
+                const int so = vis ? (pst_row_off(qb, a32, MB) + pb - lo) * PST_BLOCK_BYTES : 0;
+                any = any || vis;
+#pragma unroll
+                for (int st = 0; st < 2; st++)
+                    __builtin_amdgcn_raw_buffer_store_b128(pws[kb][st], rs_pst, vis ? l * 16 : PST_OOB, so + 1024 * st, 0);
+            }
+            __builtin_amdgcn_raw_buffer_store_b32(__builtin_bit_cast(int, m_run), rs_pref, (hh == 0 && any) ? r * 4 : PST_OOB,
+                                                  any ? ((qb * pst_tiles64(p.Kc)) + ((P - p0) >> 6)) * 128 : 0, 0);
         }
         STAMP(6)
         __syncthreads();
@@ -647,12 +678,12 @@
     STAMP_FLUSH
 }
 
-template <int DH>
+template <int DH, bool PST = false>
 int launch_fwd(const RelAttnP& p, hipStream_t s) {
     using G = Geo<DH>;
     static bool attr_set = false;
     if (!attr_set) {
-        hipError_t e = hipFuncSetAttribute(reinterpret_cast<const void*>(&relattn_fwd_kernel<DH>),
+        hipError_t e = hipFuncSetAttribute(reinterpret_cast<const void*>(&relattn_fwd_kernel<DH, PST>),
                                            hipFuncAttributeMaxDynamicSharedMemorySize, G::SMEM);
         if (e != hipSuccess) return (int)e;
         attr_set = true;
@@ -660,7 +691,7 @@
     dim3 grid((p.T + QB - 1) / QB, p.H, p.B);
     {
         mxl_kt::Scope kt(MXL_KT_RELATTN_FWD, s);
-        hipLaunchKernelGGL((relattn_fwd_kernel<DH>), grid, dim3(256), G::SMEM, s, p);
+        hipLaunchKernelGGL((relattn_fwd_kernel<DH, PST>), grid, dim3(256), G::SMEM, s, p);
     }
     MXL_LAUNCH_CHECK();
     return MXL_OK;
@@ -681,8 +712,13 @@
 static int relattn_fwd_launch(const void* q, const void* k, const void* v, const void* rd, const float* r_w_bias,
                               const float* r_r_bias, void* out, float* lse, int B, int T, int H, int dh, int M, int Kc,
                               long long q_bs, int q_rs, long long kv_bs, int kv_rs, int rd_rs, long long o_bs, int o_rs,
-                              float scale, void* oph, float* mph, void* stream, int oph_all = 0, void* ph_ws = nullptr) {
+                              float scale, void* oph, float* mph, void* stream, int oph_all = 0, void* ph_ws = nullptr,
+                              void* pst = nullptr, float* pst_ref = nullptr) {
     MXL_CHECK_ARG(q && k && v && rd && r_w_bias && r_r_bias && out);
+    if (pst || pst_ref) {
+        MXL_CHECK_ARG(pst && pst_ref && lse && ((uintptr_t)pst % 16) == 0);
+        if (dh != 64 || (T % 32) != 0 || (M % 32) != 0 || (Kc % 32) != 0 || ((T - Kc) % 64) != 0) return MXL_EUNSUPPORTED;
+    }
     if (oph_all) MXL_CHECK_ARG(oph && ((T - Kc) % 64) == 0);
     if (ph_ws) MXL_CHECK_ARG(oph_all && dh == 64 && ((uintptr_t)ph_ws % 16) == 0);
     if (oph) MXL_CHECK_ARG(mph && (M % (oph_all ? 32 : 256)) == 0 && (T % 32) == 0 && ((uintptr_t)oph % 8) == 0);
@@ -699,7 +735,9 @@
     p.q_bs = q_bs; p.kv_bs = kv_bs; p.o_bs = o_bs; p.q_rs = q_rs; p.kv_rs = kv_rs; p.rd_rs = rd_rs; p.o_rs = o_rs;
     p.scale_log2e = scale * 1.4426950408889634f;
     p.oph = (bf16_t*)oph; p.mph = mph; p.oph_all = oph_all ? 1 : 0; p.ph_rec = (char*)ph_ws;
+    p.pst = (char*)pst; p.pst_ref = pst_ref;
     hipStream_t s = (hipStream_t)stream;
+    if (pst) return launch_fwd<64, true>(p, s);
     switch (dh) {
         case 16: return launch_fwd<16>(p, s);
         case 32: return launch_fwd<32>(p, s);
@@ -733,3 +771,27 @@
     return relattn_fwd_launch(q, k, v, rd, r_w_bias, r_r_bias, out, lse, B, T, H, dh, M, Kc, q_bs, q_rs, kv_bs, kv_rs, rd_rs, o_bs,
                               o_rs, scale, oph, mph, stream, oph_all, ph_ws);
 }
+
+static bool pstore_domain(int B, int T, int H, int M, int Kc) {
+    return B > 0 && T > 0 && H > 0 && M > 0 && Kc >= T && Kc <= M + T && (T % 32) == 0 && (M % 32) == 0 && (Kc % 32) == 0 &&
+           ((T - Kc) % 64) == 0 && (long long)(T >> 5) * (M >> 5) < (1ll << 19) && (long long)(T >> 5) * pst_tiles64(Kc) < (1ll << 23);
+}
+extern "C" size_t mxl_relattn_pstore_bytes(int B, int T, int H, int M, int Kc) {
+    if (!pstore_domain(B, T, H, M, Kc)) return 0;
+    return (size_t)B * H * (size_t)pst_row_off(T >> 5, (T - Kc) / 32, M >> 5) * PST_BLOCK_BYTES;
+}
+extern "C" size_t mxl_relattn_pstore_ref_bytes(int B, int T, int H, int M, int Kc) {
+    if (!pstore_domain(B, T, H, M, Kc)) return 0;
+    return (size_t)B * H * (size_t)(T >> 5) * pst_tiles64(Kc) * 32 * sizeof(float);
+}
+
+extern "C" int mxl_relattn_fwd_pstore(const void* q, const void* k, const void* v, const void* rd, const float* r_w_bias,
+                                      const float* r_r_bias, void* out, float* lse, void* oph, float* mph, void* ph_ws, void* pst,
+                                      float* pst_ref, int B, int T, int H, int dh, int M, int Kc, long long q_bs, int q_rs,
+                                      long long kv_bs, int kv_rs, int rd_rs, long long o_bs, int o_rs, float scale, void* stream) {
+    MXL_CHECK_ARG(pst && pst_ref);
+    MXL_CHECK_ARG(Kc == M + T || (oph && mph));
+    if (dh == 64 && !pstore_domain(B, T, H, M, Kc)) return MXL_EUNSUPPORTED;
+    return relattn_fwd_launch(q, k, v, rd, r_w_bias, r_r_bias, out, lse, B, T, H, dh, M, Kc, q_bs, q_rs, kv_bs, kv_rs, rd_rs, o_bs,
+                              o_rs, scale, oph, mph, stream, oph ? 1 : 0, ph_ws, pst, pst_ref);
+}
diff --git a/symbolic_music_generation_amd/ops.py b/symbolic_music_generation_amd/ops.py
--- a/symbolic_music_generation_amd/ops.py
+++ b/symbolic_music_generation_amd/ops.py
@@ -650,9 +650,36 @@
     return ok
 
 
+def pstore_row_lo(qb, a, MB) -> int:
+    return max(a, qb - MB)
+
+
+def pstore_row_off(qb, a, MB) -> int:
+    g = min(qb, a + MB + 1)
+    return g * (g - 1) // 2 + g * (1 - a) + (qb - g) * (MB + 1)
+
+
+def pstore_bytes(B, T, H, M, Kc):
+    return int(lib().mxl_relattn_pstore_bytes(B, T, H, M, Kc)), int(lib().mxl_relattn_pstore_ref_bytes(B, T, H, M, Kc))
+
+
+def pstore_alloc(B, T, H, M, Kc, device):
+    nb, nr = pstore_bytes(B, T, H, M, Kc)
+    if nb == 0:
+        raise ValueError(f'no probability store at T={T} M={M} Kc={Kc}')
+    return torch.empty(nb, device=device, dtype=torch.uint8), torch.empty(nr // 4, device=device, dtype=torch.float32)
+
+
 def relattn_fwd(q, k, v, rd, r_w_bias, r_r_bias, out, lse, *, B, T, H, dh, M, Kc, q_bs, q_rs, kv_bs, kv_rs, rd_rs,
-                o_bs, o_rs, scale=None, oph=None, mph=None, oph_all=False, ph_buf=None):
+                o_bs, o_rs, scale=None, oph=None, mph=None, oph_all=False, ph_buf=None, pst=None, pst_ref=None):
     scale = scale if scale is not None else 1.0 / math.sqrt(dh)
+    if pst is not None or pst_ref is not None:
+        if pst is None or pst_ref is None or (oph is not None and not oph_all):
+            raise ValueError('the probability store needs pst and pst_ref, and oph_all with oph')
+        check(lib().mxl_relattn_fwd_pstore(_p(q), _p(k), _p(v), _p(rd), _p(r_w_bias), _p(r_r_bias), _p(out), _p(lse), _p(oph), _p(mph),
+                                           _p(ph_buf), _p(pst), _p(pst_ref), B, T, H, dh, M, Kc, q_bs, q_rs, kv_bs, kv_rs, rd_rs, o_bs,
+                                           o_rs, float(scale), _stream()), 'mxl_relattn_fwd_pstore')
+        return out
     if oph is not None and oph_all:
         check(lib().mxl_relattn_fwd_phantom2(_p(q), _p(k), _p(v), _p(rd), _p(r_w_bias), _p(r_r_bias), _p(out), _p(lse), _p(oph),
                                              _p(mph), 1, _p(ph_buf), B, T, H, dh, M, Kc, q_bs, q_rs, kv_bs, kv_rs, rd_rs, o_bs, o_rs,
@@ -865,9 +892,12 @@
 
 def relattn_bwd_fused(q, k, v, rd, r_w_bias, r_r_bias, out, dout, lse, delta, dq, dk, dv, d_rd, d_rwb, d_rrb, ws, qr_buf, *,
                       B, T, H, dh, M, Kc, q_bs, q_rs, kv_bs, kv_rs, rd_rs, o_bs, o_rs, dq_bs, dq_rs, dkv_bs, dkv_rs,
-                      scale=None, oph=None, mph=None, defer_drd=False, ph_buf=None, ph_ready=False, delta_ready=False, dq_mode=None):
+                      scale=None, oph=None, mph=None, defer_drd=False, ph_buf=None, ph_ready=False, delta_ready=False, dq_mode=None,
+                      pst=None, pst_ref=None):
     scale = scale if scale is not None else 1.0 / math.sqrt(dh)
     d = H * dh
+    if (pst is None) != (pst_ref is None):
+        raise ValueError('pst and pst_ref go together')
     if dq_mode is None:
         owner = fused_dq_owner_mode(B, H, _n_cus(q.device), _RESERVED_CUS, os.environ)
     else:
@@ -875,10 +905,17 @@
             raise ValueError(f'dq_mode must be None, "owner" or "slabs", not {dq_mode!r}')
         owner = dq_mode == 'owner'
     mode_bits = (2 if delta_ready else 0) | (4 if owner else 8)
-    check(lib().mxl_relattn_bwd_fused(_p(q), _p(k), _p(v), _p(rd), _p(r_w_bias), _p(r_r_bias), _p(out), _p(dout), _p(lse), _p(delta),
-                                      _p(dq), _p(dk), _p(dv), _p(d_rd), d_rd.stride(0), _p(d_rwb), _p(d_rrb), _p(oph), _p(mph), _p(ws),
-                                      B, T, H, dh, M, Kc, q_bs, q_rs, kv_bs, kv_rs, rd_rs, o_bs, o_rs, dq_bs, dq_rs, dkv_bs, dkv_rs,
-                                      float(scale), mode_bits, _stream()), 'mxl_relattn_bwd_fused')
+    if pst is not None:
+        check(lib().mxl_relattn_bwd_fused_pstore(_p(q), _p(k), _p(v), _p(rd), _p(r_w_bias), _p(r_r_bias), _p(out), _p(dout), _p(lse),
+                                                 _p(delta), _p(dq), _p(dk), _p(dv), _p(d_rd), d_rd.stride(0), _p(d_rwb), _p(d_rrb),
+                                                 _p(oph), _p(mph), _p(ws), _p(pst), _p(pst_ref), B, T, H, dh, M, Kc, q_bs, q_rs, kv_bs,
+                                                 kv_rs, rd_rs, o_bs, o_rs, dq_bs, dq_rs, dkv_bs, dkv_rs, float(scale), mode_bits,
+                                                 _stream()), 'mxl_relattn_bwd_fused_pstore')
+    else:
+        check(lib().mxl_relattn_bwd_fused(_p(q), _p(k), _p(v), _p(rd), _p(r_w_bias), _p(r_r_bias), _p(out), _p(dout), _p(lse), _p(delta),
+                                          _p(dq), _p(dk), _p(dv), _p(d_rd), d_rd.stride(0), _p(d_rwb), _p(d_rrb), _p(oph), _p(mph), _p(ws),
+                                          B, T, H, dh, M, Kc, q_bs, q_rs, kv_bs, kv_rs, rd_rs, o_bs, o_rs, dq_bs, dq_rs, dkv_bs, dkv_rs,
+                                          float(scale), mode_bits, _stream()), 'mxl_relattn_bwd_fused')
 
     def phantom():
         if Kc < M + T:
diff --git a/symbolic_music_generation_amd/xl_engine.py b/symbolic_music_generation_amd/xl_engine.py
--- a/symbolic_music_generation_amd/xl_engine.py
+++ b/symbolic_music_generation_amd/xl_engine.py
@@ -9,6 +9,7 @@
 from ._lib import MusicXLError
 
 F = ops
+PSTORE_AUTO = True
 
 
 def _r8(n: int) -> int:
@@ -242,8 +243,20 @@
         ws.nll = torch.empty(B, max(T - 1, 1), **f32)
         ws.hlse = torch.empty(N, 2, **f32)
         ws.acc = torch.zeros(2, **f32)
+        ws.pst = None
+        mode = os.environ.get('MXL_FUSED_PSTORE', 'auto')
+        if mode not in ('0', '1', 'auto'):
+            raise MusicXLError(f'MXL_FUSED_PSTORE must be 0, 1 or auto, not {mode!r}')
+        auto_on = mode == 'auto' and PSTORE_AUTO and ops.fused_dq_owner_mode(B, H, ops._n_cus(dev), ops._RESERVED_CUS, os.environ)
+        if train and ws.fused_bwd and c.d_head == 64 and (mode == '1' or auto_on):
+            nb, nr = ops.pstore_bytes(B, T, H, M, Kc)
+            if nb and L * (nb + nr) <= self._pstore_budget():
+                ws.pst = [ops.pstore_alloc(B, T, H, M, Kc, dev) for _ in range(L)]
         self._ws[key] = ws
         return ws
+
+    def _pstore_budget(self) -> int:
+        return int(torch.cuda.mem_get_info(self.dev)[0]) // 2
 
     def _site(self, l, k):
         return 8 + 8 * l + k
@@ -304,7 +317,9 @@
                             ws.av[s], ws.lse[s], oph=ws.oph[s].view(B, T, d) if (train and ws.oph is not None) else None,
                             mph=ws.mph[s] if (train and ws.oph is not None) else None,
                             oph_all=bool(train and getattr(ws, 'fused_bwd', False)),
-                            ph_buf=ws.ph[s] if (train and ws.ph is not None) else None, **st)
+                            ph_buf=ws.ph[s] if (train and ws.ph is not None) else None,
+                            pst=ws.pst[s][0] if (train and ws.pst is not None) else None,
+                            pst_ref=ws.pst[s][1] if (train and ws.pst is not None) else None, **st)
             ops.gemm(ws.av[s], self._lw(l, 'dec_attn.o_net.weight'), ws.tmp, N, d, d)
             ops.ln_residual_fwd(ws.tmp, h_in, self._lw(l, 'dec_attn.layer_norm.weight', self.P),
                                 self._lw(l, 'dec_attn.layer_norm.bias', self.P), ws.h1[s],
@@ -582,7 +597,8 @@
                                       oph=ws.oph[l].view(B, T, d) if ws.oph is not None else None,
                                       mph=ws.mph[l] if ws.oph is not None else None,
                                       ph_buf=ws.ph[l] if ws.ph is not None else None, ph_ready=ws.ph is not None,
-                                      delta_ready=delta_ready, **st)
+                                      delta_ready=delta_ready, pst=ws.pst[l][0] if ws.pst is not None else None,
+                                      pst_ref=ws.pst[l][1] if ws.pst is not None else None, **st)
             else:
                 ops.relattn_bwd(qkv[:, Kc - T:, :d], qkv[:, :, d:2 * d], qkv[:, :, 2 * d:], ws.rd[l],
                                 self._lw(l, 'dec_attn.r_w_bias', self.P), self._lw(l, 'dec_attn.r_r_bias', self.P), ws.av[l],
```
